# miha-stopar/Plonky3-mobile

Measured on AMD Instinct MI355X. Metric: fib_air proofs/sec, higher is better.
Workload: dtype u32 (BabyBear Montgomery, 31-bit modular)

## Files before the change

include/p3hip.h:

```cpp
#ifndef P3HIP_H
#define P3HIP_H
#include <stddef.h>
#include <stdint.h>

#ifdef __cplusplus
extern "C" {
#endif

#define P3HIP_OK 0
#define P3HIP_ERR_BAD_ARG (-1)
#define P3HIP_ERR_HIP (-2)
#define P3HIP_ERR_BACKEND (-3)
#define P3HIP_ERR_INTERNAL (-4)

#define P3HIP_BACKEND_CPU 0
#define P3HIP_BACKEND_VULKAN 1
#define P3HIP_BACKEND_METAL 2
#define P3HIP_BACKEND_WEBGPU 3
#define P3HIP_BACKEND_HIP 4

int p3hip_set_backend(const char *name);
int p3hip_get_backend(void);
int p3hip_is_available(char *msg, size_t cap);
const char *p3hip_take_last_error(void);

int p3hip_malloc(void **dev_ptr, size_t bytes);
int p3hip_free(void *dev_ptr);
int p3hip_upload(void *dev_dst, const void *host_src, size_t bytes);
int p3hip_download(void *host_dst, const void *dev_src, size_t bytes);
int p3hip_sync(void *stream);
void p3hip_release_thread_context(void);

int p3hip_dft_batch_bb31(const uint32_t *in, uint32_t *out, size_t height, size_t width);
int p3hip_idft_batch_bb31(const uint32_t *in, uint32_t *out, size_t height, size_t width);
int p3hip_coset_dft_batch_bb31(const uint32_t *in, uint32_t *out, size_t height, size_t width,
                               uint32_t shift_monty);
int p3hip_coset_lde_batch_bb31(const uint32_t *in, uint32_t *out, size_t height, size_t width,
                               unsigned added_bits, uint32_t shift_monty, int bit_reversed_out);
const char *p3hip_last_timing_line(void);
int p3hip_dft_batch_bb31_dev(const uint32_t *d_in, uint32_t *d_out, size_t height, size_t width, void *stream);
int p3hip_idft_batch_bb31_dev(const uint32_t *d_in, uint32_t *d_out, size_t height, size_t width, void *stream);
int p3hip_coset_dft_batch_bb31_dev(const uint32_t *d_in, uint32_t *d_out, size_t height, size_t width,
                                   uint32_t shift_monty, void *stream);
int p3hip_coset_lde_batch_bb31_dev(const uint32_t *d_in, uint32_t *d_out, size_t height, size_t width,
                                   unsigned added_bits, uint32_t shift_monty, int bit_reversed_out,
                                   void *stream);
int p3hip_coset_lde_from_coeffs_bb31_dev(const uint32_t *d_coeffs, uint32_t *d_out, size_t height, size_t width,
                                         unsigned added_bits, uint32_t shift_monty, void *stream);
int p3hip_dft_plan_bb31(size_t height, size_t width, uint32_t *stages_per_pass, size_t cap, size_t *n_passes);
int p3hip_bit_reverse_rows_dev(const uint32_t *d_in, uint32_t *d_out, size_t height, size_t width, void *stream);

int p3hip_fib_trace_dev(uint64_t a, uint64_t b, size_t n, uint32_t *d_out, void *stream);

int p3hip_poseidon2_permute_dev(uint32_t *d_states, size_t n, void *stream);
int p3hip_poseidon2_permute(uint32_t *states, size_t n);
int p3hip_poseidon2_permute_variant_dev(uint32_t *d_states, size_t n, int variant, void *stream);
int p3hip_poseidon2_f64_probe_dev(const double *d_in, uint32_t *d_out, size_t n, int mode, void *stream);

typedef struct p3hip_tree p3hip_tree_t;
int p3hip_mmcs_commit_dev(const uint32_t *const *d_mats, const size_t *heights, const size_t *widths,
                          size_t n_mats, uint32_t root_out[8], p3hip_tree_t **tree_out, void *stream);
int p3hip_mmcs_commit_async_dev(const uint32_t *const *d_mats, const size_t *heights, const size_t *widths,
                                size_t n_mats, p3hip_tree_t **tree_out, void *stream);
int p3hip_mmcs_root(const p3hip_tree_t *tree, uint32_t root_out[8], void *stream);
size_t p3hip_mmcs_log_max_height(const p3hip_tree_t *tree);
size_t p3hip_mmcs_num_layers(const p3hip_tree_t *tree);
const uint32_t *p3hip_mmcs_layer_dev(const p3hip_tree_t *tree, size_t layer, size_t *len_out);
int p3hip_mmcs_open_batch(const p3hip_tree_t *tree, size_t index, uint32_t *rows_out, uint32_t *path_out,
                          void *stream);
void p3hip_mmcs_free(p3hip_tree_t *tree);
#define P3HIP_MMCS_ROOT_MISMATCH 1
#define P3HIP_MMCS_WRONG_HEIGHT  2
#define P3HIP_MMCS_NOT_CANONICAL 3
#define P3HIP_MMCS_BAD_INDEX     4
int p3hip_mmcs_verify_batch(int hash, const uint32_t root[8], const size_t *heights, const size_t *widths, size_t n_mats,
                            size_t index, const uint32_t *rows, const uint32_t *path, size_t path_len);
size_t p3hip_mmcs_row_words(const p3hip_tree_t *tree);
int p3hip_mmcs_open_batch_many_dev(const p3hip_tree_t *tree, const uint32_t *d_indices, size_t n,
                                   uint32_t *d_rows , uint32_t *d_paths , void *stream);
int p3hip_mmcs_verify_batch_many_dev(int hash, const uint32_t root[8] ,
                                     const size_t *heights, const size_t *widths, size_t n_mats,
                                     const uint32_t *d_indices, size_t n, const uint32_t *d_rows, const uint32_t *d_paths,
                                     uint32_t *d_status , uint32_t *d_rejected ,
                                     void *stream);
int p3hip_mmcs_verify_batch_many_form_dev(int form, int hash, const uint32_t root[8], const size_t *heights, const size_t *widths,
                                          size_t n_mats, const uint32_t *d_indices, size_t n, const uint32_t *d_rows,
                                          const uint32_t *d_paths, uint32_t *d_status, uint32_t *d_rejected, void *stream);
size_t p3hip_mmcs_verify_coop_max(int hash, int profile);
int p3hip_mmcs_commit(const uint32_t *const *mats, const size_t *heights, const size_t *widths,
                      size_t n_mats, uint32_t root_out[8], p3hip_tree_t **tree_out);

#define P3HIP_HASH_POSEIDON2 0
#define P3HIP_HASH_KECCAK 1
int p3hip_mmcs_commit_hash_dev(int hash, const uint32_t *const *d_mats, const size_t *heights, const size_t *widths,
                               size_t n_mats, uint32_t root_out[8], p3hip_tree_t **tree_out, void *stream);
int p3hip_mmcs_commit_hash(int hash, const uint32_t *const *mats, const size_t *heights, const size_t *widths,
                           size_t n_mats, uint32_t root_out[8], p3hip_tree_t **tree_out);
size_t p3hip_mmcs_layer_words(size_t max_height);
int p3hip_mmcs_commit_into_dev(int hash, const uint32_t *const *d_mats, const size_t *heights, const size_t *widths,
                               size_t n_mats, uint32_t *d_layers, p3hip_tree_t **tree_out, void *stream);
int p3hip_keccak_f_dev(uint64_t *d_states, size_t n, void *stream);

typedef struct {
    uint32_t log_blowup;
    uint32_t log_final_poly_len;
    uint32_t num_queries;
    uint32_t proof_of_work_bits;
} p3hip_fri_params_t;
typedef struct p3hip_fib_prover p3hip_fib_prover_t;
#define P3HIP_PROFILE_THROUGHPUT 1
#define P3HIP_PROFILE_LATENCY 2
int p3hip_set_thread_profile(int profile);
int p3hip_get_thread_profile(void);
int p3hip_fib_prover_create_profile(int profile, int hash, int hiding, uint64_t seed, unsigned log_n, const p3hip_fri_params_t *params,
                                    void *stream, int own_stream, p3hip_fib_prover_t **out);
int p3hip_fib_prover_create(unsigned log_n, const p3hip_fri_params_t *params, void *stream, int own_stream,
                            p3hip_fib_prover_t **out);
int p3hip_fib_prover_prove(p3hip_fib_prover_t *prover, uint64_t a, uint64_t b, const uint8_t **proof_out,
                           size_t *proof_len);
int p3hip_fib_prover_prove_into(p3hip_fib_prover_t *prover, uint64_t a, uint64_t b, uint8_t *out, size_t cap, size_t *proof_len);
int p3hip_fib_prover_enqueue(p3hip_fib_prover_t *prover, uint64_t a, uint64_t b);
int p3hip_fib_prover_finish(p3hip_fib_prover_t *prover, const uint8_t **proof_out, size_t *proof_len);
int p3hip_fib_prover_stage_times(p3hip_fib_prover_t *prover, double out_ms[6], uint64_t *proofs, int reset);
int p3hip_fib_prover_grind_miss_probe(p3hip_fib_prover_t *prover, uint64_t *misses, uint32_t *indices_out, size_t cap,
                                      size_t *n_out);
void p3hip_fib_prover_destroy(p3hip_fib_prover_t *prover);
int p3hip_verify_fib_air(const uint8_t *proof, size_t len, uint64_t a, uint64_t b, uint64_t x, unsigned log_n,
                         const p3hip_fri_params_t *params);

int p3hip_fib_prover_create_hash(int hash, unsigned log_n, const p3hip_fri_params_t *params, void *stream, int own_stream,
                                 p3hip_fib_prover_t **out);
int p3hip_verify_fib_air_hash(int hash, const uint8_t *proof, size_t len, uint64_t a, uint64_t b, uint64_t x,
                              unsigned log_n, const p3hip_fri_params_t *params);

int p3hip_fib_prover_create_hiding(int hash, unsigned log_n, const p3hip_fri_params_t *params, uint64_t seed, void *stream,
                                   int own_stream, p3hip_fib_prover_t **out);
int p3hip_verify_fib_air_hiding(int hash, const uint8_t *proof, size_t len, uint64_t a, uint64_t b, uint64_t x,
                                unsigned log_n, const p3hip_fri_params_t *params);
typedef struct p3hip_rng p3hip_rng_t;
int p3hip_rng_create(uint64_t seed, p3hip_rng_t **out);
int p3hip_rng_fill_field_dev(p3hip_rng_t *rng, uint32_t *d_out, size_t n, void *stream);
int p3hip_rng_state(p3hip_rng_t *rng, uint64_t state_out[4], void *stream);
void p3hip_rng_destroy(p3hip_rng_t *rng);
int p3hip_mmcs_commit_hiding_dev(int hash, const uint32_t *const *d_mats, const size_t *heights, const size_t *widths,
                                 size_t n_mats, p3hip_rng_t *rng, uint32_t root_out[8], p3hip_tree_t **tree_out, void *stream);

typedef struct p3hip_fib_batch p3hip_fib_batch_t;
int p3hip_fib_batch_create(unsigned log_n, const p3hip_fri_params_t *params, unsigned n_provers,
                           p3hip_fib_batch_t **out);
int p3hip_fib_batch_create_hash(int hash, unsigned log_n, const p3hip_fri_params_t *params, unsigned n_provers,
                                p3hip_fib_batch_t **out);
int p3hip_fib_batch_create_hiding(int hash, unsigned log_n, const p3hip_fri_params_t *params, uint64_t seed, unsigned n_provers,
                                  p3hip_fib_batch_t **out);
int p3hip_fib_batch_prove(p3hip_fib_batch_t *batch, size_t n, const uint64_t *a, const uint64_t *b,
                          const uint8_t **proofs_out, size_t *lens_out);
int p3hip_fib_batch_submit(p3hip_fib_batch_t *batch, size_t n, const uint64_t *a, const uint64_t *b, uint64_t *ticket_out);
int p3hip_fib_batch_collect(p3hip_fib_batch_t *batch, uint64_t ticket, const uint8_t **proofs_out, size_t *lens_out);
void p3hip_fib_batch_destroy(p3hip_fib_batch_t *batch);

#define P3HIP_PROVE_CHECK_TRACE 1u
#define P3HIP_TRACE_BAD_FIRST_LEFT 1u
#define P3HIP_TRACE_BAD_FIRST_RIGHT 2u
#define P3HIP_TRACE_BAD_NEXT_LEFT 4u
#define P3HIP_TRACE_BAD_NEXT_RIGHT 8u
#define P3HIP_TRACE_BAD_LAST_RIGHT 16u
#define P3HIP_TRACE_BAD_RANGE 32u
typedef struct {
    int64_t first_bad_row;
    uint32_t mask;
    uint64_t bad_rows;
} p3hip_trace_check_t;
int p3hip_fib_check_trace_dev(const uint32_t *d_trace, size_t n, const uint32_t pis[3], p3hip_trace_check_t *out, void *stream);
int p3hip_fib_prover_prove_trace_dev(p3hip_fib_prover_t *prover, const uint32_t *d_trace, const uint32_t pis[3], unsigned flags,
                                     const uint8_t **proof_out, size_t *proof_len);
int p3hip_fib_prover_prove_trace(p3hip_fib_prover_t *prover, const uint32_t *host_trace, size_t n, const uint32_t pis[3], unsigned flags,
                                 const uint8_t **proof_out, size_t *proof_len);
int p3hip_fib_prover_enqueue_trace_dev(p3hip_fib_prover_t *prover, const uint32_t *d_trace, const uint32_t pis[3]);
int p3hip_fib_batch_prove_traces_dev(p3hip_fib_batch_t *batch, size_t n, const uint32_t *const *d_traces, const uint32_t *pis,
                                     unsigned flags, const uint8_t **proofs_out, size_t *lens_out);

typedef struct p3hip_fib_verifier p3hip_fib_verifier_t;
#define P3HIP_VERIFY_MALFORMED 16
int p3hip_fib_proof_len(int hash, int hiding, unsigned log_n, const p3hip_fri_params_t *params, size_t *len_out);
int p3hip_fib_verifier_create(int hash, int hiding, unsigned log_n, const p3hip_fri_params_t *params, size_t max_proofs,
                              p3hip_fib_verifier_t **out);
int p3hip_fib_verifier_verify_dev(p3hip_fib_verifier_t *v, const uint8_t *d_proofs, size_t stride_bytes, const uint32_t *d_lens,
                                  const uint32_t *d_pis, size_t n, uint32_t *d_status, uint32_t *d_rejected, void *stream);
int p3hip_fib_verifier_verify(p3hip_fib_verifier_t *v, size_t n, const uint8_t *const *proofs, const size_t *lens,
                              const uint64_t *a, const uint64_t *b, const uint64_t *x, uint32_t *status_out);
void p3hip_fib_verifier_destroy(p3hip_fib_verifier_t *v);

int p3hip_run_fib_air_zk(char *out, size_t cap);

typedef struct p3hip_challenger p3hip_challenger_t;
int p3hip_challenger_create(int hash, p3hip_challenger_t **out);
int p3hip_challenger_observe(p3hip_challenger_t *c, const uint32_t *monty_words, size_t n);
int p3hip_challenger_observe_digest(p3hip_challenger_t *c, const uint32_t digest[8]);
int p3hip_challenger_sample_ext(p3hip_challenger_t *c, uint32_t out[4]);
int p3hip_challenger_sample_bits(p3hip_challenger_t *c, unsigned bits, uint32_t *out);
int p3hip_challenger_clone(const p3hip_challenger_t *c, p3hip_challenger_t **out);
void p3hip_challenger_destroy(p3hip_challenger_t *c);
#define P3HIP_CHALLENGER_STATE_WORDS 128
int p3hip_challenger_export(const p3hip_challenger_t *c, uint32_t words[P3HIP_CHALLENGER_STATE_WORDS]);
int p3hip_challenger_import(p3hip_challenger_t *c, const uint32_t words[P3HIP_CHALLENGER_STATE_WORDS]);

typedef struct p3hip_pcs p3hip_pcs_t;
typedef struct p3hip_pcs_data p3hip_pcs_data_t;
int p3hip_pcs_create(int profile, int hash, const p3hip_fri_params_t *params, void *stream, int own_stream, p3hip_pcs_t **out);
int p3hip_pcs_commit_dev(p3hip_pcs_t *pcs, const uint32_t *const *d_evals, const size_t *heights, const size_t *widths,
                         const uint32_t *domain_shifts , size_t n_mats,
                         uint32_t root_out[8], p3hip_pcs_data_t **data_out);
int p3hip_pcs_lde_dev(const p3hip_pcs_data_t *data, size_t mat, const uint32_t **d_lde, size_t *height, size_t *width);
int p3hip_pcs_open(p3hip_pcs_t *pcs, const p3hip_pcs_data_t *const *rounds, size_t n_rounds,
                   const size_t *points_per_mat, const uint32_t *points ,
                   p3hip_challenger_t *challenger ,
                   uint32_t *opened_out, size_t opened_cap_words, const uint8_t **proof_out, size_t *proof_len);
int p3hip_pcs_verify(int hash, const p3hip_fri_params_t *params, unsigned log_h, const uint32_t *roots ,
                     const size_t *mats_per_round, const size_t *widths, size_t n_rounds, const size_t *points_per_mat,
                     const uint32_t *points, const uint32_t *opened, const uint8_t *proof, size_t len,
                     p3hip_challenger_t *challenger, int *reject_code);
void p3hip_pcs_data_free(p3hip_pcs_data_t *d);
void p3hip_pcs_destroy(p3hip_pcs_t *pcs);

int p3hip_pcs_create_hiding(int profile, int hash, const p3hip_fri_params_t *params, unsigned num_random_codewords, uint64_t mmcs_seed,
                            uint64_t pcs_seed, void *stream, int own_stream, p3hip_pcs_t **out);
int p3hip_pcs_commit_quotient_dev(p3hip_pcs_t *pcs, const uint32_t *const *d_chunks, size_t h, size_t width, size_t n_chunks,
                                  uint32_t root_out[8], p3hip_pcs_data_t **data_out);
int p3hip_pcs_commit_randomization(p3hip_pcs_t *pcs, unsigned log_h, uint32_t root_out[8], p3hip_pcs_data_t **data_out);
int p3hip_pcs_verify_hiding(int hash, const p3hip_fri_params_t *params, unsigned log_h, const uint32_t *roots ,
                            const size_t *mats_per_round, const size_t *widths, size_t n_rounds, const size_t *points_per_mat,
                            const uint32_t *points, const uint32_t *opened, const uint8_t *proof, size_t len,
                            p3hip_challenger_t *challenger, int *reject_code);

typedef struct p3hip_pcs_verifier p3hip_pcs_verifier_t;
typedef struct {
    unsigned log_h;
    size_t n_rounds;
    const size_t *mats_per_round;
    const size_t *widths;
    const size_t *points_per_mat;
    size_t n_slots;
    const uint32_t *slots;
} p3hip_pcs_shape_t;
int p3hip_pcs_proof_len(int hash, int hiding, const p3hip_fri_params_t *params, const p3hip_pcs_shape_t *shape, size_t *len_out);
int p3hip_pcs_verifier_create(int hash, int hiding, const p3hip_fri_params_t *params, const p3hip_pcs_shape_t *shape, size_t max_proofs,
                              p3hip_pcs_verifier_t **out);
int p3hip_pcs_verifier_verify_dev(p3hip_pcs_verifier_t *v, const uint8_t *d_proofs, size_t stride_bytes, const uint32_t *d_lens,
                                  const uint32_t *d_roots, const uint32_t *d_points, const uint32_t *d_opened, const uint32_t *d_chal_in,
                                  size_t n, uint32_t *d_status, uint32_t *d_rejected, uint32_t *d_chal_out, void *stream);
int p3hip_pcs_verifier_verify(p3hip_pcs_verifier_t *v, size_t n, const uint8_t *const *proofs, const size_t *lens, const uint32_t *roots,
                              const uint32_t *points, const uint32_t *opened, p3hip_challenger_t *const *challengers, uint32_t *status_out);
int p3hip_pcs_verifier_wave_form(const p3hip_pcs_verifier_t *v);
void p3hip_pcs_verifier_destroy(p3hip_pcs_verifier_t *v);

typedef int (*p3hip_cpu_dft_fn)(void *user, const uint32_t *in, uint32_t *out, size_t height, size_t width);
int p3hip_run_dft_benchmark(p3hip_cpu_dft_fn cpu_dft, void *user, char *out, size_t cap);

#ifdef __cplusplus
}
#endif
#endif
```

plonky3-mobile_amd/_lib.py:

```python
import ctypes as C
import os
import subprocess

_HERE = os.path.dirname(os.path.abspath(__file__))
LIB_PATH = os.environ.get("P3HIP_LIB") or os.path.join(_HERE, "libp3hip.so")
ROOT = os.path.dirname(_HERE)

u32p = C.POINTER(C.c_uint32)
_SIGS = {
    "p3hip_set_backend": (C.c_int, [C.c_char_p]),
    "p3hip_get_backend": (C.c_int, []),
    "p3hip_is_available": (C.c_int, [C.c_char_p, C.c_size_t]),
    "p3hip_take_last_error": (C.c_char_p, []),
    "p3hip_malloc": (C.c_int, [C.POINTER(C.c_void_p), C.c_size_t]),
    "p3hip_free": (C.c_int, [C.c_void_p]),
    "p3hip_upload": (C.c_int, [C.c_void_p, C.c_void_p, C.c_size_t]),
    "p3hip_download": (C.c_int, [C.c_void_p, C.c_void_p, C.c_size_t]),
    "p3hip_sync": (C.c_int, [C.c_void_p]),
    "p3hip_last_timing_line": (C.c_char_p, []),
    "p3hip_release_thread_context": (None, []),
    "p3hip_dft_batch_bb31": (C.c_int, [C.c_void_p, C.c_void_p, C.c_size_t, C.c_size_t]),
    "p3hip_idft_batch_bb31": (C.c_int, [C.c_void_p, C.c_void_p, C.c_size_t, C.c_size_t]),
    "p3hip_coset_dft_batch_bb31": (C.c_int, [C.c_void_p, C.c_void_p, C.c_size_t, C.c_size_t, C.c_uint32]),
    "p3hip_coset_lde_batch_bb31": (C.c_int, [C.c_void_p, C.c_void_p, C.c_size_t, C.c_size_t, C.c_uint,
                                             C.c_uint32, C.c_int]),
    "p3hip_dft_batch_bb31_dev": (C.c_int, [C.c_void_p, C.c_void_p, C.c_size_t, C.c_size_t, C.c_void_p]),
    "p3hip_idft_batch_bb31_dev": (C.c_int, [C.c_void_p, C.c_void_p, C.c_size_t, C.c_size_t, C.c_void_p]),
    "p3hip_coset_dft_batch_bb31_dev": (C.c_int, [C.c_void_p, C.c_void_p, C.c_size_t, C.c_size_t, C.c_uint32,
                                                 C.c_void_p]),
    "p3hip_coset_lde_batch_bb31_dev": (C.c_int, [C.c_void_p, C.c_void_p, C.c_size_t, C.c_size_t, C.c_uint,
                                                 C.c_uint32, C.c_int, C.c_void_p]),
    "p3hip_coset_lde_from_coeffs_bb31_dev": (C.c_int, [C.c_void_p, C.c_void_p, C.c_size_t, C.c_size_t, C.c_uint, C.c_uint32,
                                                       C.c_void_p]),
    "p3hip_bit_reverse_rows_dev": (C.c_int, [C.c_void_p, C.c_void_p, C.c_size_t, C.c_size_t, C.c_void_p]),
    "p3hip_dft_plan_bb31": (C.c_int, [C.c_size_t, C.c_size_t, C.POINTER(C.c_uint32), C.c_size_t, C.POINTER(C.c_size_t)]),
    "p3hip_fib_trace_dev": (C.c_int, [C.c_uint64, C.c_uint64, C.c_size_t, C.c_void_p, C.c_void_p]),
    "p3hip_poseidon2_permute_dev": (C.c_int, [C.c_void_p, C.c_size_t, C.c_void_p]),
    "p3hip_poseidon2_permute": (C.c_int, [C.c_void_p, C.c_size_t]),
    "p3hip_poseidon2_permute_variant_dev": (C.c_int, [C.c_void_p, C.c_size_t, C.c_int, C.c_void_p]),
    "p3hip_poseidon2_f64_probe_dev": (C.c_int, [C.c_void_p, C.c_void_p, C.c_size_t, C.c_int, C.c_void_p]),
    "p3hip_mmcs_commit_dev": (C.c_int, [C.POINTER(C.c_void_p), C.POINTER(C.c_size_t), C.POINTER(C.c_size_t),
                                        C.c_size_t, C.c_void_p, C.POINTER(C.c_void_p), C.c_void_p]),
    "p3hip_mmcs_commit_async_dev": (C.c_int, [C.POINTER(C.c_void_p), C.POINTER(C.c_size_t),
                                              C.POINTER(C.c_size_t), C.c_size_t, C.POINTER(C.c_void_p),
                                              C.c_void_p]),
    "p3hip_mmcs_commit_hash_dev": (C.c_int, [C.c_int, C.POINTER(C.c_void_p), C.POINTER(C.c_size_t), C.POINTER(C.c_size_t),
                                             C.c_size_t, C.c_void_p, C.POINTER(C.c_void_p), C.c_void_p]),
    "p3hip_mmcs_commit_hash": (C.c_int, [C.c_int, C.POINTER(C.c_void_p), C.POINTER(C.c_size_t), C.POINTER(C.c_size_t),
                                         C.c_size_t, C.c_void_p, C.POINTER(C.c_void_p)]),
    "p3hip_mmcs_layer_words": (C.c_size_t, [C.c_size_t]),
    "p3hip_mmcs_commit_into_dev": (C.c_int, [C.c_int, C.POINTER(C.c_void_p), C.POINTER(C.c_size_t), C.POINTER(C.c_size_t),
                                             C.c_size_t, C.c_void_p, C.POINTER(C.c_void_p), C.c_void_p]),
    "p3hip_keccak_f_dev": (C.c_int, [C.c_void_p, C.c_size_t, C.c_void_p]),
    "p3hip_mmcs_root": (C.c_int, [C.c_void_p, C.c_void_p, C.c_void_p]),
    "p3hip_mmcs_log_max_height": (C.c_size_t, [C.c_void_p]),
    "p3hip_mmcs_num_layers": (C.c_size_t, [C.c_void_p]),
    "p3hip_mmcs_layer_dev": (C.c_void_p, [C.c_void_p, C.c_size_t, C.POINTER(C.c_size_t)]),
    "p3hip_mmcs_open_batch": (C.c_int, [C.c_void_p, C.c_size_t, C.c_void_p, C.c_void_p, C.c_void_p]),
    "p3hip_mmcs_free": (None, [C.c_void_p]),
    "p3hip_mmcs_verify_batch": (C.c_int, [C.c_int, C.c_void_p, C.POINTER(C.c_size_t), C.POINTER(C.c_size_t), C.c_size_t, C.c_size_t,
                                          C.c_void_p, C.c_void_p, C.c_size_t]),
    "p3hip_mmcs_row_words": (C.c_size_t, [C.c_void_p]),
    "p3hip_mmcs_verify_coop_max": (C.c_size_t, [C.c_int, C.c_int]),
    "p3hip_mmcs_open_batch_many_dev": (C.c_int, [C.c_void_p, C.c_void_p, C.c_size_t, C.c_void_p, C.c_void_p, C.c_void_p]),
    "p3hip_mmcs_verify_batch_many_dev": (C.c_int, [C.c_int, C.c_void_p, C.POINTER(C.c_size_t), C.POINTER(C.c_size_t), C.c_size_t, C.c_void_p,
                                                   C.c_size_t, C.c_void_p, C.c_void_p, C.c_void_p, C.c_void_p, C.c_void_p]),
    "p3hip_mmcs_verify_batch_many_form_dev": (C.c_int, [C.c_int, C.c_int, C.c_void_p, C.POINTER(C.c_size_t), C.POINTER(C.c_size_t), C.c_size_t,
                                                        C.c_void_p, C.c_size_t, C.c_void_p, C.c_void_p, C.c_void_p, C.c_void_p, C.c_void_p]),
    "p3hip_set_thread_profile": (C.c_int, [C.c_int]),
    "p3hip_get_thread_profile": (C.c_int, []),
    "p3hip_fib_prover_create_profile": (C.c_int, [C.c_int, C.c_int, C.c_int, C.c_uint64, C.c_uint, C.c_void_p, C.c_void_p, C.c_int,
                                                  C.POINTER(C.c_void_p)]),
    "p3hip_fib_prover_create": (C.c_int, [C.c_uint, C.c_void_p, C.c_void_p, C.c_int, C.POINTER(C.c_void_p)]),
    "p3hip_fib_prover_create_hash": (C.c_int, [C.c_int, C.c_uint, C.c_void_p, C.c_void_p, C.c_int, C.POINTER(C.c_void_p)]),
    "p3hip_verify_fib_air_hash": (C.c_int, [C.c_int, C.c_void_p, C.c_size_t, C.c_uint64, C.c_uint64, C.c_uint64, C.c_uint,
                                            C.c_void_p]),
    "p3hip_fib_prover_prove": (C.c_int, [C.c_void_p, C.c_uint64, C.c_uint64, C.POINTER(C.POINTER(C.c_uint8)),
                                         C.POINTER(C.c_size_t)]),
    "p3hip_fib_prover_prove_into": (C.c_int, [C.c_void_p, C.c_uint64, C.c_uint64, C.c_void_p, C.c_size_t, C.POINTER(C.c_size_t)]),
    "p3hip_fib_prover_stage_times": (C.c_int, [C.c_void_p, C.POINTER(C.c_double), C.POINTER(C.c_uint64), C.c_int]),
    "p3hip_fib_prover_enqueue": (C.c_int, [C.c_void_p, C.c_uint64, C.c_uint64]),
    "p3hip_fib_prover_finish": (C.c_int, [C.c_void_p, C.POINTER(C.POINTER(C.c_uint8)), C.POINTER(C.c_size_t)]),
    "p3hip_fib_prover_destroy": (None, [C.c_void_p]),
    "p3hip_run_fib_air_zk": (C.c_int, [C.c_char_p, C.c_size_t]),
    "p3hip_run_dft_benchmark": (C.c_int, [C.c_void_p, C.c_void_p, C.c_char_p, C.c_size_t]),
    "p3hip_fib_prover_grind_miss_probe": (C.c_int, [C.c_void_p, C.POINTER(C.c_uint64), C.POINTER(C.c_uint32), C.c_size_t,
                                                    C.POINTER(C.c_size_t)]),
    "p3hip_fib_prover_create_hiding": (C.c_int, [C.c_int, C.c_uint, C.c_void_p, C.c_uint64, C.c_void_p, C.c_int, C.POINTER(C.c_void_p)]),
    "p3hip_verify_fib_air_hiding": (C.c_int, [C.c_int, C.c_void_p, C.c_size_t, C.c_uint64, C.c_uint64, C.c_uint64, C.c_uint,
                                              C.c_void_p]),
    "p3hip_rng_create": (C.c_int, [C.c_uint64, C.POINTER(C.c_void_p)]),
    "p3hip_rng_fill_field_dev": (C.c_int, [C.c_void_p, C.c_void_p, C.c_size_t, C.c_void_p]),
    "p3hip_rng_state": (C.c_int, [C.c_void_p, C.POINTER(C.c_uint64), C.c_void_p]),
    "p3hip_rng_destroy": (None, [C.c_void_p]),
    "p3hip_mmcs_commit_hiding_dev": (C.c_int, [C.c_int, C.POINTER(C.c_void_p), C.POINTER(C.c_size_t), C.POINTER(C.c_size_t),
                                               C.c_size_t, C.c_void_p, C.c_void_p, C.POINTER(C.c_void_p), C.c_void_p]),
    "p3hip_fib_batch_create": (C.c_int, [C.c_uint, C.c_void_p, C.c_uint, C.POINTER(C.c_void_p)]),
    "p3hip_fib_batch_create_hash": (C.c_int, [C.c_int, C.c_uint, C.c_void_p, C.c_uint, C.POINTER(C.c_void_p)]),
    "p3hip_fib_batch_create_hiding": (C.c_int, [C.c_int, C.c_uint, C.c_void_p, C.c_uint64, C.c_uint, C.POINTER(C.c_void_p)]),
    "p3hip_fib_batch_prove": (C.c_int, [C.c_void_p, C.c_size_t, C.POINTER(C.c_uint64), C.POINTER(C.c_uint64),
                                        C.POINTER(C.POINTER(C.c_uint8)), C.POINTER(C.c_size_t)]),
    "p3hip_fib_batch_submit": (C.c_int, [C.c_void_p, C.c_size_t, C.POINTER(C.c_uint64), C.POINTER(C.c_uint64), C.POINTER(C.c_uint64)]),
    "p3hip_fib_batch_collect": (C.c_int, [C.c_void_p, C.c_uint64, C.POINTER(C.POINTER(C.c_uint8)), C.POINTER(C.c_size_t)]),
    "p3hip_fib_batch_destroy": (None, [C.c_void_p]),
    "p3hip_verify_fib_air": (C.c_int, [C.c_void_p, C.c_size_t, C.c_uint64, C.c_uint64, C.c_uint64, C.c_uint, C.c_void_p]),
    "p3hip_fib_check_trace_dev": (C.c_int, [C.c_void_p, C.c_size_t, u32p, C.c_void_p, C.c_void_p]),
    "p3hip_fib_prover_prove_trace_dev": (C.c_int, [C.c_void_p, C.c_void_p, u32p, C.c_uint, C.POINTER(C.POINTER(C.c_uint8)),
                                                   C.POINTER(C.c_size_t)]),
    "p3hip_fib_prover_prove_trace": (C.c_int, [C.c_void_p, C.c_void_p, C.c_size_t, u32p, C.c_uint, C.POINTER(C.POINTER(C.c_uint8)),
                                               C.POINTER(C.c_size_t)]),
    "p3hip_fib_prover_enqueue_trace_dev": (C.c_int, [C.c_void_p, C.c_void_p, u32p]),
    "p3hip_fib_batch_prove_traces_dev": (C.c_int, [C.c_void_p, C.c_size_t, C.POINTER(C.c_void_p), u32p, C.c_uint,
                                                   C.POINTER(C.POINTER(C.c_uint8)), C.POINTER(C.c_size_t)]),
    "p3hip_fib_proof_len": (C.c_int, [C.c_int, C.c_int, C.c_uint, C.c_void_p, C.POINTER(C.c_size_t)]),
    "p3hip_fib_verifier_create": (C.c_int, [C.c_int, C.c_int, C.c_uint, C.c_void_p, C.c_size_t, C.POINTER(C.c_void_p)]),
    "p3hip_fib_verifier_verify_dev": (C.c_int, [C.c_void_p, C.c_void_p, C.c_size_t, C.c_void_p, C.c_void_p, C.c_size_t, C.c_void_p, C.c_void_p,
                                                C.c_void_p]),
    "p3hip_fib_verifier_verify": (C.c_int, [C.c_void_p, C.c_size_t, C.POINTER(C.c_char_p), C.POINTER(C.c_size_t), C.POINTER(C.c_uint64),
                                            C.POINTER(C.c_uint64), C.POINTER(C.c_uint64), u32p]),
    "p3hip_fib_verifier_destroy": (None, [C.c_void_p]),
    "p3hip_mmcs_commit": (C.c_int, [C.POINTER(C.c_void_p), C.POINTER(C.c_size_t), C.POINTER(C.c_size_t),
                                    C.c_size_t, C.c_void_p, C.POINTER(C.c_void_p)]),
    "p3hip_challenger_create": (C.c_int, [C.c_int, C.POINTER(C.c_void_p)]),
    "p3hip_challenger_observe": (C.c_int, [C.c_void_p, C.c_void_p, C.c_size_t]),
    "p3hip_challenger_observe_digest": (C.c_int, [C.c_void_p, C.c_void_p]),
    "p3hip_challenger_sample_ext": (C.c_int, [C.c_void_p, C.c_void_p]),
    "p3hip_challenger_sample_bits": (C.c_int, [C.c_void_p, C.c_uint, u32p]),
    "p3hip_challenger_clone": (C.c_int, [C.c_void_p, C.POINTER(C.c_void_p)]),
    "p3hip_challenger_destroy": (None, [C.c_void_p]),
    "p3hip_pcs_create": (C.c_int, [C.c_int, C.c_int, C.c_void_p, C.c_void_p, C.c_int, C.POINTER(C.c_void_p)]),
    "p3hip_pcs_commit_dev": (C.c_int, [C.c_void_p, C.POINTER(C.c_void_p), C.POINTER(C.c_size_t), C.POINTER(C.c_size_t), C.c_void_p, C.c_size_t,
                                       C.c_void_p, C.POINTER(C.c_void_p)]),
    "p3hip_pcs_lde_dev": (C.c_int, [C.c_void_p, C.c_size_t, C.POINTER(C.c_void_p), C.POINTER(C.c_size_t), C.POINTER(C.c_size_t)]),
    "p3hip_pcs_open": (C.c_int, [C.c_void_p, C.POINTER(C.c_void_p), C.c_size_t, C.POINTER(C.c_size_t), C.c_void_p, C.c_void_p, C.c_void_p,
                                 C.c_size_t, C.POINTER(C.POINTER(C.c_uint8)), C.POINTER(C.c_size_t)]),
    "p3hip_pcs_verify": (C.c_int, [C.c_int, C.c_void_p, C.c_uint, C.c_void_p, C.POINTER(C.c_size_t), C.POINTER(C.c_size_t), C.c_size_t,
                                   C.POINTER(C.c_size_t), C.c_void_p, C.c_void_p, C.c_void_p, C.c_size_t, C.c_void_p, C.POINTER(C.c_int)]),
    "p3hip_pcs_create_hiding": (C.c_int, [C.c_int, C.c_int, C.c_void_p, C.c_uint, C.c_uint64, C.c_uint64, C.c_void_p, C.c_int,
                                          C.POINTER(C.c_void_p)]),
    "p3hip_pcs_commit_quotient_dev": (C.c_int, [C.c_void_p, C.POINTER(C.c_void_p), C.c_size_t, C.c_size_t, C.c_size_t, C.c_void_p,
                                                C.POINTER(C.c_void_p)]),
    "p3hip_pcs_commit_randomization": (C.c_int, [C.c_void_p, C.c_uint, C.c_void_p, C.POINTER(C.c_void_p)]),
    "p3hip_pcs_verify_hiding": (C.c_int, [C.c_int, C.c_void_p, C.c_uint, C.c_void_p, C.POINTER(C.c_size_t), C.POINTER(C.c_size_t), C.c_size_t,
                                          C.POINTER(C.c_size_t), C.c_void_p, C.c_void_p, C.c_void_p, C.c_size_t, C.c_void_p,
                                          C.POINTER(C.c_int)]),
    "p3hip_challenger_export": (C.c_int, [C.c_void_p, C.c_void_p]),
    "p3hip_challenger_import": (C.c_int, [C.c_void_p, C.c_void_p]),
    "p3hip_pcs_proof_len": (C.c_int, [C.c_int, C.c_int, C.c_void_p, C.c_void_p, C.POINTER(C.c_size_t)]),
    "p3hip_pcs_verifier_create": (C.c_int, [C.c_int, C.c_int, C.c_void_p, C.c_void_p, C.c_size_t, C.POINTER(C.c_void_p)]),
    "p3hip_pcs_verifier_verify_dev": (C.c_int, [C.c_void_p, C.c_void_p, C.c_size_t, C.c_void_p, C.c_void_p, C.c_void_p, C.c_void_p, C.c_void_p,
                                                C.c_size_t, C.c_void_p, C.c_void_p, C.c_void_p, C.c_void_p]),
    "p3hip_pcs_verifier_verify": (C.c_int, [C.c_void_p, C.c_size_t, C.POINTER(C.c_char_p), C.POINTER(C.c_size_t), C.c_void_p, C.c_void_p,
                                            C.c_void_p, C.POINTER(C.c_void_p), u32p]),
    "p3hip_pcs_verifier_wave_form": (C.c_int, [C.c_void_p]),
    "p3hip_pcs_verifier_destroy": (None, [C.c_void_p]),
    "p3hip_pcs_data_free": (None, [C.c_void_p]),
    "p3hip_pcs_destroy": (None, [C.c_void_p]),
}


class P3HipError(RuntimeError):
    def __init__(self, code, msg):
        super().__init__("libp3hip error %d: %s" % (code, msg))
        self.code = code
        self.message = msg


def build(force=False):
    csrc = os.path.join(_HERE, "csrc")
    if force:
        subprocess.check_call(["make", "-s", "-C", csrc, "clean"])
    subprocess.check_call(["make", "-s", "-j4", "-C", csrc])
    return LIB_PATH


_lib = None


def lib():
    global _lib
    if _lib is None:
        if not os.path.exists(LIB_PATH):
            raise ImportError("libp3hip.so is not built (run __graft_entry__.build()); "
                              "there is no CPU fallback in this package")
        import torch
        L = C.CDLL(LIB_PATH)
        for name, (res, args) in _SIGS.items():
            fn = getattr(L, name)
            fn.restype = res
            fn.argtypes = args
        _lib = L
    return _lib


_sha = None


def lib_sha256():
    global _sha
    if _sha is None:
        import hashlib
        with open(LIB_PATH, "rb") as f:
            _sha = hashlib.sha256(f.read()).hexdigest()
    return _sha


_src_sha = None


def src_sha256():
    global _src_sha
    if _src_sha is None:
        import glob
        import hashlib
        csrc = os.path.join(_HERE, "csrc")
        files = sorted(glob.glob(os.path.join(csrc, "*.hip")) + glob.glob(os.path.join(csrc, "*.h")) + glob.glob(os.path.join(csrc, "*.inc")) +
                       [os.path.join(csrc, "Makefile"), os.path.join(ROOT, "include", "p3hip.h")])
        h = hashlib.sha256()
        for f in files:
            h.update(os.path.relpath(f, ROOT).encode() + b"\0")
            with open(f, "rb") as fh:
                h.update(fh.read())
            h.update(b"\0")
        _src_sha = h.hexdigest()
    return _src_sha


def declared_symbols():
    return sorted(_SIGS)


def take_last_error():
    m = lib().p3hip_take_last_error()
    return m.decode() if m else None


def check(rc):
    if rc != 0:
        raise P3HipError(rc, take_last_error() or "")
```

plonky3-mobile_amd/csrc/c_api.hip:

```cpp
#include "../../include/p3hip.h"

#include <atomic>
#include <chrono>
#include <condition_variable>
#include <mutex>
#include <deque>
#include <thread>
#include <cctype>
#include <cstdio>
#include <cstring>

#include "bb31.hip.h"
#include "challenger.h"
#include "common.h"
#include "mmcs.h"
#include "prover.h"
#include "pcs_verifier_dev.h"
#include "verifier_dev.h"
#include "rng.h"

namespace p3 {
bool take_error(std::string* out);
}
using namespace p3;
// ... 563 lines not shown
            P3_HIP(hipStreamCreateWithFlags(&st, hipStreamNonBlocking));
            own = true;
        }
        std::unique_ptr<p3hip_fib_prover> p(new p3hip_fib_prover());
        FriParams fp{params->log_blowup, params->log_final_poly_len, params->num_queries, params->proof_of_work_bits};
        if (hiding) {
            p->hiding.reset(new FibHidingProver());
            rc = p->hiding->init(log_n, fp, st, own, hash, seed, prof);
        } else {
            p->plain.reset(new FibProver());
            rc = p->plain->init(log_n, fp, st, own, hash, prof);
        }
        if (rc) return rc;
        *out = p.release();
        return OK;
    });
}
int p3hip_fib_prover_create(unsigned log_n, const p3hip_fri_params_t* params, void* stream, int own_stream,
                            p3hip_fib_prover_t** out) {
    return p3hip_fib_prover_create_profile(P3HIP_PROFILE_LATENCY, HASH_POSEIDON2, 0, 0, log_n, params, stream, own_stream, out);
}
int p3hip_fib_prover_create_hash(int hash, unsigned log_n, const p3hip_fri_params_t* params, void* stream, int own_stream,
                                 p3hip_fib_prover_t** out) {
    return p3hip_fib_prover_create_profile(P3HIP_PROFILE_LATENCY, hash, 0, 0, log_n, params, stream, own_stream, out);
}

int p3hip_fib_prover_prove(p3hip_fib_prover_t* prover, uint64_t a, uint64_t b, const uint8_t** proof_out,
                           size_t* proof_len) {
    return guarded([&]() -> int {
        if (!prover || !proof_out || !proof_len) return fail(ERR_BAD_ARG, "fib_prover_prove: null argument");
        int rc = prover->prove(a, b);
        if (rc) return rc;
        *proof_out = prover->last.data();
        *proof_len = prover->last.size();
        return OK;
    });
}

int p3hip_fib_prover_prove_into(p3hip_fib_prover_t* prover, uint64_t a, uint64_t b, uint8_t* out, size_t cap, size_t* proof_len) {
    return guarded([&]() -> int {
        if (!prover || !out || !proof_len) return fail(ERR_BAD_ARG, "fib_prover_prove_into: null argument");
        if (prover->proof_len && prover->proof_len > cap) {
            *proof_len = prover->proof_len;
            return fail(ERR_BAD_ARG, "fib_prover_prove_into: the proof needs " + std::to_string(prover->proof_len) + " bytes");
        }
        int rc = prover->prove(a, b);
        if (rc) return rc;
        *proof_len = prover->last.size();
        if (prover->last.size() > cap) return fail(ERR_BAD_ARG, "fib_prover_prove_into: the proof needs " + std::to_string(prover->last.size()) + " bytes");
        memcpy(out, prover->last.data(), prover->last.size());
        return OK;
    });
}

int p3hip_fib_prover_enqueue(p3hip_fib_prover_t* prover, uint64_t a, uint64_t b) {
    return guarded([&]() -> int {
        if (!prover) return fail(ERR_BAD_ARG, "fib_prover_enqueue: null argument");
        if (!prover->plain) return fail(ERR_BAD_ARG, "fib_prover_enqueue: the hiding prover proves one proof at a time");
        return prover->plain->enqueue(a, b);
    });
}
int p3hip_fib_prover_finish(p3hip_fib_prover_t* prover, const uint8_t** proof_out, size_t* proof_len) {
    return guarded([&]() -> int {
        if (!prover || !proof_out || !proof_len) return fail(ERR_BAD_ARG, "fib_prover_finish: null argument");
        if (!prover->plain) return fail(ERR_BAD_ARG, "fib_prover_finish: the hiding prover proves one proof at a time");
        int rc = prover->plain->finish(&prover->last);
        if (rc) { prover->last.clear(); return rc; }
        prover->proof_len = prover->last.size();
        *proof_out = prover->last.data();
        *proof_len = prover->last.size();
        return OK;
    });
}

int p3hip_fib_check_trace_dev(const uint32_t* d_trace, size_t n, const uint32_t pis[3], p3hip_trace_check_t* out, void* stream) {
    return guarded([&]() -> int {
        if (!out || !pis) return fail(ERR_BAD_ARG, "fib_check_trace: null argument");
        Context* cx;
        int rc = get_context(&cx);
        if (rc) return rc;
        if (!n) { *out = p3hip_trace_check_t{-1, 0, 0}; return OK; }
        if ((rc = check_device_trace(d_trace, n, cx->device, "fib_check_trace"))) return rc;
        if ((rc = check_pis_flags(pis, 0, "fib_check_trace"))) return rc;
        TraceCheck c;
        if ((rc = fib_check_trace(*cx, (hipStream_t)stream, d_trace, n, pis, &c))) return rc;
        *out = p3hip_trace_check_t{c.first_bad_row, c.mask, c.bad_rows};
        return OK;
    });
}

int p3hip_fib_prover_prove_trace_dev(p3hip_fib_prover_t* prover, const uint32_t* d_trace, const uint32_t pis[3], unsigned flags,
                                     const uint8_t** proof_out, size_t* proof_len) {
    return guarded([&]() -> int {
        if (!prover || !proof_out || !proof_len) return fail(ERR_BAD_ARG, "fib_prover_prove_trace_dev: null argument");
        int rc = check_pis_flags(pis, flags, "fib_prover_prove_trace_dev");
        if (rc) return rc;
        if ((rc = check_device_trace(d_trace, 1ull << prover->log_n(), prover->device(), "fib_prover_prove_trace_dev"))) return rc;
        if ((rc = prover->prove_trace(d_trace, pis, flags))) return rc;
        *proof_out = prover->last.data();
        *proof_len = prover->last.size();
        return OK;
    });
}
int p3hip_fib_prover_prove_trace(p3hip_fib_prover_t* prover, const uint32_t* host_trace, size_t n, const uint32_t pis[3], unsigned flags,
                                 const uint8_t** proof_out, size_t* proof_len) {
    return guarded([&]() -> int {
        if (!prover || !host_trace || !proof_out || !proof_len) return fail(ERR_BAD_ARG, "fib_prover_prove_trace: null argument");
        int rc = check_pis_flags(pis, flags, "fib_prover_prove_trace");
        if (rc) return rc;
        if (n != (1ull << prover->log_n()))
            return fail(ERR_BAD_ARG, "fib_prover_prove_trace: n = " + std::to_string(n) + " rows, the prover proves 2^" + std::to_string(prover->log_n()));
        if (prover->plain && prover->plain->has_pending())
            return fail(ERR_BAD_ARG, "fib prover: finish the enqueued proofs before a synchronous prove");
        Context* cx;
        if ((rc = get_context(&cx))) return rc;
        if (cx->device != prover->device())
            return fail(ERR_BAD_ARG, "fib prover: created on device " + std::to_string(prover->device()) + ", current device is " + std::to_string(cx->device));
        P3_HIP(hipMemcpyAsync(prover->arena_trace(), host_trace, (size_t)n * 8, hipMemcpyHostToDevice, prover->stream()));
        if ((rc = prover->prove_trace(prover->arena_trace(), pis, flags))) return rc;
        *proof_out = prover->last.data();
        *proof_len = prover->last.size();
        return OK;
    });
}
int p3hip_fib_prover_enqueue_trace_dev(p3hip_fib_prover_t* prover, const uint32_t* d_trace, const uint32_t pis[3]) {
    return guarded([&]() -> int {
        if (!prover) return fail(ERR_BAD_ARG, "fib_prover_enqueue_trace_dev: null argument");
        if (!prover->plain) return fail(ERR_BAD_ARG, "fib_prover_enqueue_trace_dev: the hiding prover proves one proof at a time");
        int rc = check_pis_flags(pis, 0, "fib_prover_enqueue_trace_dev");
        if (rc) return rc;
        if ((rc = check_device_trace(d_trace, 1ull << prover->log_n(), prover->device(), "fib_prover_enqueue_trace_dev"))) return rc;
        return prover->plain->enqueue_trace(d_trace, pis);
    });
}

int p3hip_fib_prover_stage_times(p3hip_fib_prover_t* prover, double out_ms[6], uint64_t* proofs, int reset) {
    if (!prover || !out_ms) return fail(ERR_BAD_ARG, "fib_prover_stage_times: null argument");
    if (!prover->plain) return fail(ERR_BAD_ARG, "fib_prover_stage_times: not kept by the hiding prover");
    const StageTimes& t = prover->plain->times();
    out_ms[0] = t.trace_commit_ms; out_ms[1] = t.quotient_commit_ms; out_ms[2] = t.open_ms;
    out_ms[3] = t.fri_commit_ms; out_ms[4] = t.grind_ms; out_ms[5] = t.query_ms;
    if (proofs) *proofs = t.proofs;
    if (reset) prover->plain->reset_times();
    return OK;
}

int p3hip_fib_prover_grind_miss_probe(p3hip_fib_prover_t* prover, uint64_t* misses, uint32_t* indices_out, size_t cap, size_t* n_out) {
    if (!prover || !misses) return fail(ERR_BAD_ARG, "fib_prover_grind_miss_probe: null argument");
    if (!prover->plain) return fail(ERR_BAD_ARG, "fib_prover_grind_miss_probe: not kept by the hiding prover");
    std::vector<uint32_t> idx;
    *misses = prover->plain->grind_misses(&idx);
    if (n_out) *n_out = idx.size();
    if (indices_out) for (size_t i = 0; i < idx.size() && i < cap; i++) indices_out[i] = idx[i];
    return OK;
}

void p3hip_fib_prover_destroy(p3hip_fib_prover_t* prover) { delete prover; }

int p3hip_fib_prover_create_hiding(int hash, unsigned log_n, const p3hip_fri_params_t* params, uint64_t seed, void* stream,
                                   int own_stream, p3hip_fib_prover_t** out) {
    return p3hip_fib_prover_create_profile(P3HIP_PROFILE_LATENCY, hash, 1, seed, log_n, params, stream, own_stream, out);
}
int p3hip_verify_fib_air_hiding(int hash, const uint8_t* proof, size_t len, uint64_t a, uint64_t b, uint64_t x, unsigned log_n,
                                const p3hip_fri_params_t* params) {
    return guarded([&]() -> int {
        if (!proof || !params) return fail(ERR_BAD_ARG, "verify_fib_air_hiding: null argument");
        FriParams fp{params->log_blowup, params->log_final_poly_len, params->num_queries, params->proof_of_work_bits};
        std::string why;
        int rc = verify_fib_air_hiding(proof, len, a, b, x, log_n, fp, &why, hash);
        if (rc != 0) set_error("fib_air verification failed: " + why);
        return rc;
    });
}

}
struct p3hip_rng {
    DevRng* d = nullptr;
    uint32_t* err = nullptr;
    DevBuf ws;
    ~p3hip_rng() { if (d) (void)hipFree(d); }
};
extern "C" {
int p3hip_rng_create(uint64_t seed, p3hip_rng_t** out) {
    return guarded([&]() -> int {
        if (!out) return fail(ERR_BAD_ARG, "rng_create: null argument");
        Context* cx;
        int rc = get_context(&cx);
        if (rc) return rc;
        std::unique_ptr<p3hip_rng> r(new p3hip_rng());
        P3_HIP(hipMalloc(reinterpret_cast<void**>(&r->d), sizeof(DevRng) + 16));
        r->err = reinterpret_cast<uint32_t*>(r->d + 1);
        uint64_t s[6] = {0, 0, 0, 0, 0, 0};
        rng_seed_from_u64(s, seed);
        P3_HIP(hipMemcpy(r->d, s, sizeof(DevRng) + 16, hipMemcpyHostToDevice));
        *out = r.release();
        return OK;
    });
}
int p3hip_rng_fill_field_dev(p3hip_rng_t* rng, uint32_t* d_out, size_t n, void* stream) {
    return guarded([&]() -> int {
        if (!rng || (n && !d_out)) return fail(ERR_BAD_ARG, "rng_fill_field: null argument");
        Context* cx;
        int rc = get_context(&cx);
        if (rc) return rc;
        size_t words = 0;
        if ((rc = rng_workspace_words(n, &words))) return rc;
        if ((rc = rng->ws.reserve(words * 4))) return rc;
        return rng_fill_field(*cx, (hipStream_t)stream, rng->d, d_out, n, rng->ws.as<uint32_t>(), rng->err);
    });
}
int p3hip_rng_state(p3hip_rng_t* rng, uint64_t state_out[4], void* stream) {
    return guarded([&]() -> int {
        if (!rng || !state_out) return fail(ERR_BAD_ARG, "rng_state: null argument");
        uint64_t s[6];
        P3_HIP(hipMemcpyAsync(s, rng->d, sizeof(DevRng) + 16, hipMemcpyDeviceToHost, (hipStream_t)stream));
        P3_HIP(hipStreamSynchronize((hipStream_t)stream));
        memcpy(state_out, s, 32);
        if ((uint32_t)s[4] != 0) return fail(ERR_INTERNAL, "rng: a fill ran out of raw draws");
        return OK;
    });
}
void p3hip_rng_destroy(p3hip_rng_t* rng) { delete rng; }

int p3hip_mmcs_commit_hiding_dev(int hash, const uint32_t* const* d_mats, const size_t* heights, const size_t* widths, size_t n_mats,
                                 p3hip_rng_t* rng, uint32_t root_out[8], p3hip_tree_t** tree_out, void* stream) {
    return guarded([&]() -> int {
        if (!d_mats || !heights || !widths || !n_mats || !rng || !root_out || !tree_out) return fail(ERR_BAD_ARG, "mmcs_commit_hiding: null/empty argument");
        if (n_mats > 32) return fail(ERR_BAD_ARG, "mmcs_commit_hiding: at most 32 matrices per commitment");
        constexpr size_t SALT = 4;
        std::vector<void*> owned;
        auto cleanup = [&]() { for (void* p : owned) (void)hipFree(p); };
        std::vector<const uint32_t*> mp;
        std::vector<size_t> hh, ww;
        for (size_t i = 0; i < n_mats; i++) {
            void* salt = nullptr;
            if (hipMalloc(&salt, heights[i] * SALT * 4 + 16) != hipSuccess) { cleanup(); return fail(ERR_HIP, "hipMalloc failed"); }
            owned.push_back(salt);
            int rc = p3hip_rng_fill_field_dev(rng, (uint32_t*)salt, heights[i] * SALT, stream);
            if (rc) { cleanup(); return rc; }
            mp.push_back(d_mats[i]); hh.push_back(heights[i]); ww.push_back(widths[i]);
            mp.push_back((const uint32_t*)salt); hh.push_back(heights[i]); ww.push_back(SALT);
        }
        int rc = p3hip_mmcs_commit_hash_dev(hash, mp.data(), hh.data(), ww.data(), mp.size(), root_out, tree_out, stream);
        if (rc) { cleanup(); return rc; }
        (*tree_out)->t->owned = owned;
        return OK;
    });
}

int p3hip_verify_fib_air(const uint8_t* proof, size_t len, uint64_t a, uint64_t b, uint64_t x, unsigned log_n,
                         const p3hip_fri_params_t* params) {
    return p3hip_verify_fib_air_hash(HASH_POSEIDON2, proof, len, a, b, x, log_n, params);
}
int p3hip_verify_fib_air_hash(int hash, const uint8_t* proof, size_t len, uint64_t a, uint64_t b, uint64_t x, unsigned log_n,
                              const p3hip_fri_params_t* params) {
    return guarded([&]() -> int {
        if (!proof || !params) return fail(ERR_BAD_ARG, "verify_fib_air: null argument");
        FriParams fp{params->log_blowup, params->log_final_poly_len, params->num_queries, params->proof_of_work_bits};
        std::string why;
        int rc = verify_fib_air(proof, len, a, b, x, log_n, fp, &why, hash);
        if (rc != 0) set_error("fib_air verification failed: " + why);
        return rc;
    });
}

}

struct p3hip_fib_batch {
    unsigned log_n = 0;
    int hash = HASH_POSEIDON2;
    int device = 0;
    FriParams fp{};
    std::vector<std::thread> workers;
    std::mutex mu;
    std::condition_variable cv_work, cv_done;
    struct Job {
        uint64_t ticket = 0;
        std::vector<uint64_t> a, b;
        std::vector<const uint32_t*> traces;
        std::vector<uint32_t> pis;
        unsigned flags = 0;
        size_t next = 0, done = 0;
        std::vector<std::vector<uint8_t>> proofs;
        int first_error = 0;
        std::string error_text;
    };
    std::deque<std::shared_ptr<Job>> jobs;
    std::shared_ptr<Job> collected;
    uint64_t next_ticket = 1;
    bool stop = false;
    size_t ready = 0;
    int first_error = 0;
    std::string error_text;
    static constexpr size_t MAX_INFLIGHT = 8;

    bool hiding = false;
    uint64_t seed = 1;
    int profile = PROFILE_THROUGHPUT;
    void worker_main() {
        if (hiding) {
            FibHidingProver prover;
            worker_loop(prover, [&](hipStream_t st) { return prover.init(log_n, fp, st, true, hash, seed, profile); });
        } else {
            FibProver prover;
            worker_loop(prover, [&](hipStream_t st) { return prover.init(log_n, fp, st, true, hash, profile); });
        }
// ... 507 lines not shown
```

plonky3-mobile_amd/csrc/common.h:

```cpp
#pragma once
#include <hip/hip_runtime.h>
#include <stdint.h>

#include <map>
#include <set>
#include <string>
#include <tuple>
#include <vector>

namespace p3 {

#ifndef P3_NO_SETPRIO
#define P3_LATENCY_BOUND_KERNEL() __builtin_amdgcn_s_setprio(3)
#else
#define P3_LATENCY_BOUND_KERNEL() ((void)0)
#endif

enum Profile : int { PROFILE_THROUGHPUT = 0, PROFILE_LATENCY = 1 };

enum Status : int {
    OK = 0,
    ERR_BAD_ARG = -1,
    ERR_HIP = -2,
    ERR_BACKEND = -3,
    ERR_INTERNAL = -4,
};

void set_error(const std::string& msg);
int fail(int code, const std::string& msg);

#define P3_HIP(call)                                                                       \
    do {                                                                                   \
        hipError_t e__ = (call);                                                           \
        if (e__ != hipSuccess)                                                             \
            return p3::fail(p3::ERR_HIP, std::string(#call) + ": " + hipGetErrorString(e__)); \
    } while (0)

struct DevBuf {
    void* ptr = nullptr;
    size_t cap = 0;
    int reserve(size_t bytes);
    template <class T>
    T* as() const { return reinterpret_cast<T*>(ptr); }
    ~DevBuf();
};

struct TwoLevelTable {
    uint32_t* lo = nullptr;
    uint32_t* hi = nullptr;
    uint32_t T = 0;
};

struct CachedTable {
    TwoLevelTable t;
    hipEvent_t ready = nullptr;
    hipStream_t built_on = nullptr;
    bool complete = false;
};

struct Context {
    int device = -1;
    int profile = PROFILE_LATENCY;
    uint32_t* tile_tw[2] = {nullptr, nullptr};
    double2* tile_twd[2] = {nullptr, nullptr};
    std::map<std::pair<uint32_t, int>, CachedTable> root_tables;
    std::map<std::tuple<uint32_t, uint32_t, uint32_t>, CachedTable> scale_tables;
    std::map<std::pair<hipStream_t, int>, DevBuf> scratch;
    std::set<const void*> attr_done;
    uint64_t* rng_jump = nullptr;
    std::map<uint32_t, CachedTable> selector_tables;
    int init(int dev);
    DevBuf& ws(hipStream_t stream, int slot);
    int get_root_table(hipStream_t stream, uint32_t q, bool inverse, TwoLevelTable* out);
    int get_scale_table(hipStream_t stream, uint32_t base, uint32_t log_n, uint32_t mult, TwoLevelTable* out);
    int reserve_scale_slots(size_t k);
    int mark_built(hipStream_t stream, CachedTable& e);
    int wait_ready(hipStream_t stream, CachedTable& e);
    int ensure_dynamic_lds(const void* kernel, int bytes);
    ~Context();
};

int get_context(Context** out);
void release_thread_contexts();

int ntt_dft(Context& cx, hipStream_t stream, const uint32_t* src, uint32_t* dst, uint64_t height,
            uint32_t width, bool inverse);
std::vector<uint32_t> ntt_dft_plan(uint32_t n);
int ntt_coset_lde(Context& cx, hipStream_t stream, const uint32_t* src, uint32_t* dst, uint64_t height,
                  uint32_t width, uint32_t added_bits, uint32_t shift_monty, bool bit_reversed_out);
int ntt_coset_lde_from_coeffs(Context& cx, hipStream_t stream, const uint32_t* coeffs, uint32_t* dst, uint32_t* scratch,
                              uint64_t height, uint32_t width, uint32_t added_bits, uint32_t shift_monty);
int ntt_coset_dft(Context& cx, hipStream_t stream, const uint32_t* src, uint32_t* dst, uint64_t height,
                  uint32_t width, uint32_t shift_monty);
int bit_reverse_rows(hipStream_t stream, const uint32_t* src, uint32_t* dst, uint64_t height, uint32_t width);

int fib_trace(hipStream_t stream, uint64_t a, uint64_t b, uint64_t n, uint32_t* d_out);
enum : uint32_t {
    TRACE_BAD_FIRST_LEFT = 1, TRACE_BAD_FIRST_RIGHT = 2, TRACE_BAD_NEXT_LEFT = 4, TRACE_BAD_NEXT_RIGHT = 8, TRACE_BAD_LAST_RIGHT = 16,
    TRACE_BAD_RANGE = 32,
};
struct TraceCheck {
    int64_t first_bad_row;
    uint32_t mask;
    uint64_t bad_rows;
};
int fib_check_trace(Context& cx, hipStream_t stream, const uint32_t* d_trace, uint64_t n, const uint32_t pis[3], TraceCheck* out);

inline bool is_pow2(uint64_t v) { return v && !(v & (v - 1)); }
inline uint32_t log2u(uint64_t v) {
    uint32_t l = 0;
    while ((1ull << l) < v) l++;
    return l;
}

}
```

plonky3-mobile_amd/csrc/fib_air.hip:

```cpp
#include "bb31.hip.h"
#include "common.h"

#include <algorithm>

namespace p3 {

constexpr uint32_t FIB_CHUNK = 16;

struct M2 { uint32_t a, b, c, d; };
__device__ __forceinline__ M2 m2mul(const M2& x, const M2& y) {
    return M2{bb::add(bb::mul(x.a, y.a), bb::mul(x.b, y.c)), bb::add(bb::mul(x.a, y.b), bb::mul(x.b, y.d)),
              bb::add(bb::mul(x.c, y.a), bb::mul(x.d, y.c)), bb::add(bb::mul(x.c, y.b), bb::mul(x.d, y.d))};
}

__global__ void fib_trace_kernel(uint32_t a0, uint32_t b0, uint64_t n, uint32_t* out) {
    uint64_t t = (uint64_t)blockIdx.x * blockDim.x + threadIdx.x;
    uint64_t start = t * FIB_CHUNK;
    if (start >= n) return;
    M2 acc{bb::ONE, 0, 0, bb::ONE}, base{0, bb::ONE, bb::ONE, bb::ONE};
    for (uint64_t e = start; e; e >>= 1) {
        if (e & 1) acc = m2mul(acc, base);
        base = m2mul(base, base);
    }
    uint32_t l = bb::add(bb::mul(acc.a, a0), bb::mul(acc.b, b0));
    uint32_t r = bb::add(bb::mul(acc.c, a0), bb::mul(acc.d, b0));
    uint2* rows = reinterpret_cast<uint2*>(out);
    for (uint32_t i = 0; i < FIB_CHUNK && start + i < n; i++) {
        rows[start + i] = make_uint2(l, r);
        uint32_t nr = bb::add(l, r);
        l = r;
        r = nr;
    }
}

int fib_trace(hipStream_t stream, uint64_t a, uint64_t b, uint64_t n, uint32_t* d_out) {
    if (!n) return OK;
    if (!is_pow2(n)) return fail(ERR_BAD_ARG, "generate_trace_rows: n must be a power of two");
    uint64_t threads = (n + FIB_CHUNK - 1) / FIB_CHUNK;
    uint32_t a0 = bb::to_monty((uint32_t)(a % bb::P)), b0 = bb::to_monty((uint32_t)(b % bb::P));
    hipLaunchKernelGGL(fib_trace_kernel, dim3((uint32_t)((threads + 255) / 256)), dim3(256), 0, stream, a0, b0, n, d_out);
    P3_HIP(hipGetLastError());
    return OK;
}

constexpr uint32_t CHECK_BLOCK = 256, CHECK_UNROLL = 4, CHECK_MAX_BLOCKS = 256 * 8;

struct CheckPis { uint32_t p0, p1, p2; };

__device__ __forceinline__ uint32_t check_row(uint64_t i, uint64_t n, uint32_t l, uint32_t r, uint32_t nl, uint32_t nr, const CheckPis& p) {
    uint32_t m = (l >= bb::P || r >= bb::P) ? TRACE_BAD_RANGE : 0u;
    if (i == 0) m |= (l != p.p0 ? TRACE_BAD_FIRST_LEFT : 0u) | (r != p.p1 ? TRACE_BAD_FIRST_RIGHT : 0u);
    if (i + 1 < n) {
        m |= nl != r ? TRACE_BAD_NEXT_LEFT : 0u;
        m |= nr != (uint32_t)(((uint64_t)l + r) % bb::P) ? TRACE_BAD_NEXT_RIGHT : 0u;
    } else {
        m |= r != p.p2 ? TRACE_BAD_LAST_RIGHT : 0u;
    }
    return m;
}

template <bool WIDE>
__global__ void __launch_bounds__(CHECK_BLOCK) fib_check_trace_kernel(const uint32_t* trace, uint64_t n, CheckPis pis,
                                                                     unsigned long long* res ) {
    const uint32_t lane = threadIdx.x & 63;
    const uint64_t pairs = (n + 1) / 2;
    const uint64_t wave = ((uint64_t)blockIdx.x * CHECK_BLOCK + threadIdx.x) >> 6, n_waves = ((uint64_t)gridDim.x * CHECK_BLOCK) >> 6;
    const uint2* rows = reinterpret_cast<const uint2*>(trace);
    unsigned long long best = ~0ull;
    uint32_t bad = 0;
    for (uint64_t base = wave * 64 * CHECK_UNROLL; base < pairs; base += n_waves * 64 * CHECK_UNROLL) {
        uint4 v[CHECK_UNROLL];
#pragma unroll
        for (uint32_t k = 0; k < CHECK_UNROLL; k++) {
            const uint64_t q = base + k * 64 + lane;
            v[k] = make_uint4(0, 0, 0, 0);
            if (2 * q + 2 <= n) {
                if (WIDE) {
                    v[k] = reinterpret_cast<const uint4*>(trace)[q];
                } else {
                    const uint2 x = rows[2 * q], y = rows[2 * q + 1];
                    v[k] = make_uint4(x.x, x.y, y.x, y.y);
                }
            } else if (2 * q < n) {
                const uint2 x = rows[2 * q];
                v[k].x = x.x; v[k].y = x.y;
            }
        }
        uint2 tail = make_uint2(0, 0);
        const uint64_t tail_row = 2 * (base + CHECK_UNROLL * 64);
        if (lane == 63 && tail_row < n) tail = rows[tail_row];
#pragma unroll
        for (uint32_t k = 0; k < CHECK_UNROLL; k++) {
            const uint64_t q = base + k * 64 + lane;
            uint32_t nl = __shfl_down(v[k].x, 1), nr = __shfl_down(v[k].y, 1);
            if (k + 1 < CHECK_UNROLL) {
                const uint32_t fl = __shfl(v[k + 1].x, 0), fr = __shfl(v[k + 1].y, 0);
                if (lane == 63) { nl = fl; nr = fr; }
            } else if (lane == 63) {
                nl = tail.x; nr = tail.y;
            }
            if (2 * q < n) {
                const uint32_t m0 = check_row(2 * q, n, v[k].x, v[k].y, v[k].z, v[k].w, pis);
                if (m0) { best = min(best, ((unsigned long long)(2 * q) << 6) | m0); bad++; }
                if (2 * q + 1 < n) {
                    const uint32_t m1 = check_row(2 * q + 1, n, v[k].z, v[k].w, nl, nr, pis);
                    if (m1) { best = min(best, ((unsigned long long)(2 * q + 1) << 6) | m1); bad++; }
                }
            }
        }
    }
    if (__ballot(bad != 0) == 0) return;
    unsigned long long total = bad;
#pragma unroll
    for (int off = 32; off > 0; off >>= 1) {
        best = min(best, __shfl_xor(best, off));
        total += __shfl_xor(total, off);
    }
    if (lane == 0) {
        atomicMax(&res[0], ~best);
        atomicAdd(&res[1], total);
    }
}

int fib_check_trace(Context& cx, hipStream_t stream, const uint32_t* d_trace, uint64_t n, const uint32_t pis[3], TraceCheck* out) {
    *out = TraceCheck{-1, 0, 0};
    if (!n) return OK;
    if (reinterpret_cast<uintptr_t>(d_trace) % 8) return fail(ERR_BAD_ARG, "check_trace: the trace must be 8-byte aligned (rows of two words)");
    if (n > (1ull << 57)) return fail(ERR_BAD_ARG, "check_trace: too many rows");
    DevBuf& buf = cx.ws(stream, 4);
    int rc = buf.reserve(16);
    if (rc) return rc;
    unsigned long long* res = buf.as<unsigned long long>();
    P3_HIP(hipMemsetAsync(res, 0, 16, stream));
    const uint64_t pairs = (n + 1) / 2, per_block = (uint64_t)CHECK_BLOCK * CHECK_UNROLL;
    const uint32_t blocks = (uint32_t)std::min<uint64_t>((pairs + per_block - 1) / per_block, CHECK_MAX_BLOCKS);
    const CheckPis p{pis[0], pis[1], pis[2]};
    if (reinterpret_cast<uintptr_t>(d_trace) % 16 == 0)
        hipLaunchKernelGGL(fib_check_trace_kernel<true>, dim3(blocks), dim3(CHECK_BLOCK), 0, stream, d_trace, n, p, res);
    else
        hipLaunchKernelGGL(fib_check_trace_kernel<false>, dim3(blocks), dim3(CHECK_BLOCK), 0, stream, d_trace, n, p, res);
    P3_HIP(hipGetLastError());
    unsigned long long h[2] = {0, 0};
    P3_HIP(hipMemcpyAsync(h, res, 16, hipMemcpyDeviceToHost, stream));
    P3_HIP(hipStreamSynchronize(stream));
    if (h[1]) {
        const unsigned long long key = ~h[0];
        out->first_bad_row = (int64_t)(key >> 6);
        out->mask = (uint32_t)(key & 63);
        out->bad_rows = h[1];
    }
    return OK;
}

}
```

plonky3-mobile_amd/csrc/poseidon2_f64.hip.h:

```cpp
#pragma once
#include "poseidon2.hip.h"

namespace p2f {

constexpr double PD = 2013265921.0;
constexpr double PINV = 1.0 / 2013265921.0;

__device__ __forceinline__ double mulmod(double a, double b) {
    double h = a * b;
    double l = __fma_rn(a, b, -h);
    double q = __builtin_rint(h * PINV);
    double r = __fma_rn(-q, PD, h);
    return r + l;
}
constexpr double PM1 = 2013265920.0;
__device__ __forceinline__ double mulmod_p(double a, double b, double aP) {
    double q = __builtin_rint(b * aP);
    double t = __fma_rn(a, b, -(q * PM1));
    return t - q;
}
__device__ __forceinline__ double reduce(double x) {
    return __fma_rn(-__builtin_rint(x * PINV), PD, x);
}
__device__ __forceinline__ double add_scaled_pow2(double tot, double x, double inv) {
    double xt = __fma_rn(x, inv, tot);
    double fr = __builtin_amdgcn_fract(xt);
    return __fma_rn(fr, -PD, xt);
}
constexpr double MAGIC = 6755399441055744.0;
constexpr double MAGIC_P = 6755399441055744.0 * 2013265921.0;
struct MagicRegs { double m, mp; };
__device__ __forceinline__ MagicRegs magic_regs() {
    MagicRegs r{MAGIC, MAGIC_P};
    asm volatile("" : "+v"(r.m), "+v"(r.mp));
    return r;
}
__device__ __forceinline__ double mulmod_m(double a, double b, double aP, const MagicRegs& k, double neg_pm1) {
    const double qb = __fma_rn(b, aP, k.m);
    const double c = __fma_rn(qb, neg_pm1, k.mp);
    const double t = __fma_rn(a, b, c);
    return t - qb;
}
__device__ __forceinline__ double sbox7(double x, const MagicRegs& k, double neg_pm1, double pinv) {
    const double xP = x * pinv;
    const double x2 = mulmod_m(x, x, xP, k, neg_pm1), x3 = mulmod_m(x, x2, xP, k, neg_pm1), x4 = mulmod_m(x, x3, xP, k, neg_pm1);
    return mulmod_m(x3, x4, x3 * pinv, k, neg_pm1);
}

struct ConstsF64 {
    double ext[8][16];
    double in[13];
    double k3, k15, i4, i8, i16, i256;
    double neg_pm1, pinv;
};
constexpr uint32_t c_from_monty(uint32_t m) {
    uint32_t t = m * bb::MU;
    uint64_t u = (uint64_t)t * bb::P;
    uint32_t uh = (uint32_t)(u >> 32);
    return uh ? bb::P - uh : 0;
}
constexpr uint64_t c_powmod(uint64_t b, uint64_t e) { uint64_t r = 1; b %= bb::P; while (e) { if (e & 1) r = r * b % bb::P; b = b * b % bb::P; e >>= 1; } return r; }
constexpr ConstsF64 make_consts() {
    ConstsF64 c{};
    for (int r = 0; r < 4; r++)
        for (int i = 0; i < 16; i++) {
            c.ext[r][i] = (double)c_from_monty(P3_RC16_EXT_INIT_MONTY[r][i]);
            c.ext[4 + r][i] = (double)c_from_monty(P3_RC16_EXT_FINAL_MONTY[r][i]);
        }
    for (int r = 0; r < 13; r++) c.in[r] = (double)c_from_monty(P3_RC16_INTERNAL_MONTY[r]);
    c.k3 = 3.0; c.k15 = 15.0; c.i4 = 0.25; c.i8 = 0.125; c.i16 = 0.0625; c.i256 = 0.00390625;
    c.neg_pm1 = -2013265920.0; c.pinv = 1.0 / 2013265921.0;
    return c;
}
static __device__ __constant__ ConstsF64 d_c = make_consts();

__device__ __forceinline__ void mat4(double& a, double& b, double& c, double& d) {
    double t01 = a + b, t23 = c + d, t0123 = t01 + t23;
    double t01123 = t0123 + b, t01233 = t0123 + d;
    double nd = __fma_rn(a, 2.0, t01233), nb = __fma_rn(c, 2.0, t01123);
    double na = t01123 + t01, nc = t01233 + t23;
    a = na; b = nb; c = nc; d = nd;
}
__device__ __forceinline__ void external_linear(double (&s)[16]) {
#pragma unroll
    for (int i = 0; i < 16; i += 4) mat4(s[i], s[i + 1], s[i + 2], s[i + 3]);
    double t[4];
#pragma unroll
    for (int k = 0; k < 4; k++) t[k] = (s[k] + s[k + 4]) + (s[k + 8] + s[k + 12]);
#pragma unroll
    for (int i = 0; i < 16; i++) s[i] += t[i & 3];
}

__device__ __forceinline__ void internal_rounds(double (&s)[16], const MagicRegs& mk) {
    const double npm1 = d_c.neg_pm1, pinv = d_c.pinv;
    const double k3 = d_c.k3, k15 = d_c.k15, i4 = d_c.i4, i8 = d_c.i8, i16 = d_c.i16, i256 = d_c.i256;
    auto internal_round = [&](int r) {
        s[0] = sbox7(s[0] + d_c.in[r], mk, npm1, pinv);
        double tot = ((s[0] + s[1]) + (s[2] + s[3])) + ((s[4] + s[5]) + (s[6] + s[7])) +
                     (((s[8] + s[9]) + (s[10] + s[11])) + ((s[12] + s[13]) + (s[14] + s[15])));
        tot = reduce(tot);
        s[0] = __fma_rn(s[0], -2.0, tot);
        s[1] = tot + s[1];
        s[2] = __fma_rn(s[2], 2.0, tot);
        s[3] = add_scaled_pow2(tot, s[3], 0.5);
        s[4] = __fma_rn(s[4], k3, tot);
        s[5] = __fma_rn(s[5], 4.0, tot);
        s[6] = add_scaled_pow2(tot, s[6], -0.5);
        s[7] = __fma_rn(s[7], -k3, tot);
        s[8] = __fma_rn(s[8], -4.0, tot);
        s[9] = add_scaled_pow2(tot, s[9], i256);
        s[10] = add_scaled_pow2(tot, s[10], i4);
        s[11] = add_scaled_pow2(tot, s[11], i8);
        s[12] = __fma_rn(s[12], -k15, tot);
        s[13] = add_scaled_pow2(tot, s[13], -i256);
        s[14] = add_scaled_pow2(tot, s[14], -i16);
        s[15] = __fma_rn(s[15], k15, tot);
    };
    auto fold_integer_lanes = [&]() {
        s[1] = reduce(s[1]); s[2] = reduce(s[2]); s[4] = reduce(s[4]); s[5] = reduce(s[5]);
        s[7] = reduce(s[7]); s[8] = reduce(s[8]); s[12] = reduce(s[12]); s[15] = reduce(s[15]);
    };
    _Pragma("clang loop unroll(disable)")
    for (int blk = 0; blk < 3; blk++) {
        _Pragma("clang loop unroll(disable)")
        for (int r = 0; r < 4; r++) internal_round(4 * blk + r);
        fold_integer_lanes();
    }
    internal_round(12);
    fold_integer_lanes();
}

__device__ __forceinline__ void permute(double (&s)[16]) {
    const MagicRegs mk = magic_regs();
    const double npm1 = d_c.neg_pm1, pinv = d_c.pinv;
    external_linear(s);
    _Pragma("clang loop unroll(disable)")
    for (int r = 0; r < 4; r++) {
#pragma unroll
        for (int i = 0; i < 16; i++) s[i] = sbox7(s[i] + d_c.ext[r][i], mk, npm1, pinv);
        external_linear(s);
    }
    internal_rounds(s, mk);
    _Pragma("clang loop unroll(disable)")
    for (int r = 4; r < 8; r++) {
#pragma unroll
        for (int i = 0; i < 16; i++) s[i] = sbox7(s[i] + d_c.ext[r][i], mk, npm1, pinv);
        external_linear(s);
    }
}

__device__ __forceinline__ double load_elem(uint32_t monty) { return (double)bb::from_monty(monty); }
constexpr double R_MOD_P = 268435454.0;
constexpr double R_MOD_P_OVER_P = 268435454.0 / 2013265921.0;
__device__ __forceinline__ uint32_t store_elem(double v, const MagicRegs& k) {
    const double r = mulmod_m(R_MOD_P, v, R_MOD_P_OVER_P, k, d_c.neg_pm1);
    const uint32_t w = (uint32_t)(int32_t)r;
    return min(w, w + bb::P);
}
__device__ __forceinline__ uint32_t store_elem(double v) { return store_elem(v, magic_regs()); }

}
```

plonky3-mobile_amd/csrc/prover.h:

```cpp
#pragma once
#include <chrono>
#include <string>
#include <vector>

#include "common.h"

namespace p3 {

struct Tree;
struct Challenger;

struct FriParams {
    uint32_t log_blowup, log_final_poly_len, num_queries, proof_of_work_bits;
};

constexpr uint32_t MAX_LOG_DOMAIN = 26;
constexpr uint32_t MAX_LOG_DOMAIN_HIDING = 24;

struct StageTimes {
    double trace_commit_ms = 0, quotient_commit_ms = 0, open_ms = 0, fri_commit_ms = 0, grind_ms = 0, query_ms = 0;
    uint64_t proofs = 0;
};

class FibProver {
  public:
    FibProver();
    ~FibProver();
    FibProver(const FibProver&) = delete;
    int init(uint32_t log_n, const FriParams& fp, hipStream_t stream, bool own_stream, int hash = 0, int profile = PROFILE_LATENCY);
    int prove(uint64_t a, uint64_t b, std::vector<uint8_t>* proof);
    int enqueue(uint64_t a, uint64_t b);
    int finish(std::vector<uint8_t>* proof);
    int prove_trace(const uint32_t* d_trace, const uint32_t pis[3], std::vector<uint8_t>* proof);
    int enqueue_trace(const uint32_t* d_trace, const uint32_t pis[3]);
    uint32_t* arena_trace() const;
    bool has_pending() const;
    hipStream_t stream() const;
    uint32_t log_n() const;
    int device() const;
    const StageTimes& times() const;
    void reset_times();
    uint64_t grind_misses(std::vector<uint32_t>* last_indices) const;

  private:
    struct Impl;
    Impl* im;
    int run(uint64_t a, uint64_t b, int slot, int phase, std::vector<uint8_t>* proof, void* pending_rec);
    int enqueue_any(uint64_t a, uint64_t b, const uint32_t* d_trace, const uint32_t* pis);
};

class FibHidingProver {
  public:
    FibHidingProver();
    ~FibHidingProver();
    FibHidingProver(const FibHidingProver&) = delete;
    int init(uint32_t log_n, const FriParams& fp, hipStream_t stream, bool own_stream, int hash, uint64_t seed, int profile = PROFILE_LATENCY);
    int prove(uint64_t a, uint64_t b, std::vector<uint8_t>* proof);
    int prove_trace(const uint32_t* d_trace, const uint32_t pis[3], std::vector<uint8_t>* proof);
    uint32_t* arena_trace() const;
    hipStream_t stream() const;
    uint32_t log_n() const;
    int device() const;

  private:
    struct Impl;
    Impl* im;
    int prove_any(uint64_t a, uint64_t b, const uint32_t* d_trace, const uint32_t* pis, std::vector<uint8_t>* proof);
};

int verify_fib_air(const uint8_t* proof, size_t len, uint64_t a_pub, uint64_t b_pub, uint64_t x_pub, uint32_t log_n,
                   const FriParams& fp, std::string* why, int hash = 0);
int verify_fib_air_hiding(const uint8_t* proof, size_t len, uint64_t a_pub, uint64_t b_pub, uint64_t x_pub, uint32_t log_n,
                          const FriParams& fp, std::string* why, int hash);
int verify_check_parameters(int hash, bool hiding, uint32_t log_n, const FriParams& fp, std::string* why);


constexpr size_t PCS_MAX_MATS = 8;
constexpr size_t PCS_MAX_ROUNDS = 4;
constexpr size_t PCS_MAX_POINTS = 4;
constexpr size_t PCS_MAX_COLS = 8192;

constexpr size_t PCS_HIDING_MAX_MATS = 4;
constexpr uint32_t PCS_SALT = 4;
constexpr uint32_t PCS_MAX_RANDOM_CODEWORDS = 8;
constexpr size_t PCS_MAX_QUOTIENT_WIDTH = 2048;

struct PcsData {
    std::vector<uint32_t*> lde;
    std::vector<size_t> widths;
    uint32_t log_h = 0, log_big = 0;
    int hash = 0, device = -1;
    Tree* tree = nullptr;
    bool hiding = false;
    uint32_t nrc = 0;
    uint32_t* salt_base = nullptr;
    std::vector<uint32_t*> salts;
    PcsData() = default;
    PcsData(const PcsData&) = delete;
    ~PcsData();
};

class Pcs {
  public:
    Pcs();
    ~Pcs();
    Pcs(const Pcs&) = delete;
    int init(const FriParams& fp, hipStream_t stream, bool own_stream, int hash, int profile);
    int init_hiding(const FriParams& fp, hipStream_t stream, bool own_stream, int hash, int profile, uint32_t num_random_codewords,
                    uint64_t mmcs_seed, uint64_t pcs_seed);
    bool hiding() const;
    int commit(const uint32_t* const* d_evals, const size_t* heights, const size_t* widths, const uint32_t* shifts, size_t n_mats,
               uint32_t root_out[8], PcsData** out);
    int commit_quotient(const uint32_t* const* d_chunks, size_t h, size_t width, size_t n_chunks, uint32_t root_out[8], PcsData** out);
    int commit_randomization(uint32_t log_h, uint32_t root_out[8], PcsData** out);
    int open(const PcsData* const* rounds, size_t n_rounds, const size_t* points_per_mat, const uint32_t* points, Challenger* chal,
             std::vector<uint32_t>* opened, std::vector<uint8_t>* proof);
    hipStream_t stream() const;

  private:
    struct Impl;
    Impl* im;
    int commit_hiding(const uint32_t* const* d_evals, const size_t* heights, const size_t* widths, const uint32_t* shifts, size_t n_mats,
                      uint32_t root_out[8], PcsData** out);
    int hiding_finish(PcsData* data, uint32_t root_out[8]);
};

bool pcs_point_on_lde_coset(const uint32_t z[4], uint32_t log_big);
constexpr uint32_t CHALLENGER_STATE_WORDS = 128;
void challenger_export(const Challenger& c, uint32_t* words);
int challenger_import(const uint32_t* words, Challenger* c);
int pcs_verify(int hash, const FriParams& fp, uint32_t log_h, const uint32_t* roots, const size_t* mats_per_round, const size_t* widths,
               size_t n_rounds, const size_t* points_per_mat, const uint32_t* points, const uint32_t* opened, const uint8_t* proof,
               size_t len, Challenger* chal, std::string* why);
int pcs_verify_hiding(int hash, const FriParams& fp, uint32_t log_h, const uint32_t* roots, const size_t* mats_per_round,
                      const size_t* widths, size_t n_rounds, const size_t* points_per_mat, const uint32_t* points, const uint32_t* opened,
                      const uint8_t* proof, size_t len, Challenger* chal, std::string* why);

}
```

plonky3-mobile_amd/csrc/prover.hip:

```cpp
#include <chrono>
#include <cstddef>
#include <deque>
#include <memory>
#include <cstring>

#include "bb31.hip.h"
#include "challenger.h"
#include "common.h"
#include "keccak.hip.h"
#include "mmcs.h"
#include "poseidon2.hip.h"
#include "poseidon2_f64.hip.h"
#include "prover.h"
#include "rng.h"
#include "rng_dev.hip.h"
#include "transcript.hip.h"

namespace p3 {

using bb::Ext;

__device__ __forceinline__ uint32_t tl(const TwoLevelTable& t, uint32_t e) {
    return bb::mul(t.lo[e & ((1u << t.T) - 1u)], t.hi[e >> t.T]);
}
__device__ __forceinline__ uint32_t brev(uint32_t v, uint32_t bits) { return bits ? (__brev(v) >> (32 - bits)) : 0u; }

__device__ __forceinline__ Ext ld_ext(const uint32_t* p) {
    uint4 v = *reinterpret_cast<const uint4*>(p);
    return Ext{{v.x, v.y, v.z, v.w}};
}
__device__ __forceinline__ void st_ext(uint32_t* p, const Ext& e) {
    *reinterpret_cast<uint4*>(p) = make_uint4(e.c[0], e.c[1], e.c[2], e.c[3]);
}

constexpr int SEL_CHUNK = 8;
__global__ void selectors_kernel(TwoLevelTable roots, uint32_t n, uint32_t gen, uint32_t ginv, uint32_t zh, uint2* sel) {
    uint32_t t = blockIdx.x * blockDim.x + threadIdx.x;
    uint32_t i0 = t * SEL_CHUNK;
    if (i0 >= n) return;
    uint32_t v[2 * SEL_CHUNK], pre[2 * SEL_CHUNK];
    uint32_t acc = bb::ONE;
#pragma unroll
    for (int k = 0; k < SEL_CHUNK; k++) {
        uint32_t x = bb::mul(gen, tl(roots, (i0 + k) & (n - 1)));
        v[2 * k] = bb::sub(x, bb::ONE);
        v[2 * k + 1] = bb::sub(x, ginv);
    }
#pragma unroll
    for (int k = 0; k < 2 * SEL_CHUNK; k++) { pre[k] = acc; acc = bb::mul(acc, v[k]); }
    uint32_t inv = bb::mul(bb::inv(acc), zh);
#pragma unroll
    for (int k = 2 * SEL_CHUNK - 1; k >= 0; k--) {
        uint32_t r = bb::mul(inv, pre[k]);
        inv = bb::mul(inv, v[k]);
        v[k] = r;
    }
#pragma unroll
    for (int k = 0; k < SEL_CHUNK; k++)
        if (i0 + k < n) sel[i0 + k] = make_uint2(v[2 * k], v[2 * k + 1]);
}

struct QuotArgs {
    const uint2* lde;
    const uint2* sel;
    uint32_t* out;
    const DevState* ds;
    TwoLevelTable roots;
    uint32_t n, log_n, gen, ginv, zh_inv;
};
__global__ void __launch_bounds__(256) fib_quotient_kernel(QuotArgs a) {
    uint32_t i = blockIdx.x * blockDim.x + threadIdx.x;
    if (i >= a.n) return;
    const DevState* __restrict__ ds = a.ds;
    uint2 loc = a.lde[brev(i, a.log_n)];
    uint2 nxt = a.lde[brev((i + 1) & (a.n - 1), a.log_n)];
    uint2 s = a.sel[i];
    uint32_t x = bb::mul(a.gen, tl(a.roots, i));
    uint32_t trans = bb::sub(x, a.ginv);
    uint32_t c0 = bb::mul(s.x, bb::sub(loc.x, ds->pis[0]));
    uint32_t c1 = bb::mul(s.x, bb::sub(loc.y, ds->pis[1]));
    uint32_t c2 = bb::mul(trans, bb::sub(loc.y, nxt.x));
    uint32_t c3 = bb::mul(trans, bb::sub(bb::add(loc.x, loc.y), nxt.y));
    uint32_t c4 = bb::mul(s.y, bb::sub(loc.y, ds->pis[2]));
    Ext acc;
#pragma unroll
    for (int k = 0; k < 4; k++)
        acc.c[k] = bb::add(bb::add(bb::dot2(ds->apow[4].c[k], c0, ds->apow[3].c[k], c1), bb::dot2(ds->apow[2].c[k], c2, ds->apow[1].c[k], c3)),
                           bb::mul(ds->apow[0].c[k], c4));
    st_ext(a.out + 4 * (size_t)i, bb::scale(acc, a.zh_inv));
}

constexpr int DEN_CHUNK = 4;
__global__ void __launch_bounds__(256) inv_denoms_kernel(TwoLevelTable roots, uint32_t big, uint32_t log_big, uint32_t gen,
                                                         const DevState* __restrict__ ds, uint32_t* d0, uint32_t* d1) {
    const DenConsts k0 = ds->k0, k1 = ds->k1;
    uint32_t t = blockIdx.x * blockDim.x + threadIdx.x;
    uint32_t j0 = t * DEN_CHUNK;
    if (j0 >= big) return;
    uint32_t a0[2 * DEN_CHUNK], e0[2 * DEN_CHUNK], e1[2 * DEN_CHUNK], nrm[2 * DEN_CHUNK], pre[2 * DEN_CHUNK];
#pragma unroll
    for (int k = 0; k < DEN_CHUNK; k++) {
        uint32_t x = bb::mul(gen, tl(roots, brev((j0 + k) & (big - 1), log_big)));
#pragma unroll
        for (int z = 0; z < 2; z++) {
            const DenConsts& c = z ? k1 : k0;
            const uint32_t a = bb::sub(c.z0, x);
            const uint32_t dd0 = bb::add(bb::sqr(a), c.k0), dd1 = bb::sub(bb::mul(c.k1, a), c.c1);
            a0[2 * k + z] = a; e0[2 * k + z] = dd0; e1[2 * k + z] = dd1;
            nrm[2 * k + z] = bb::sub(bb::sqr(dd0), bb::mul(bb::W_MONTY, bb::sqr(dd1)));
        }
    }
    uint32_t acc = bb::ONE;
#pragma unroll
    for (int k = 0; k < 2 * DEN_CHUNK; k++) { pre[k] = acc; acc = bb::mul(acc, nrm[k]); }
    uint32_t inv = bb::inv(acc);
#pragma unroll
    for (int k = 2 * DEN_CHUNK - 1; k >= 0; k--) {
        const uint32_t r = bb::mul(inv, pre[k]);
        inv = bb::mul(inv, nrm[k]);
        nrm[k] = r;
    }
#pragma unroll
    for (int k = 0; k < DEN_CHUNK; k++) {
        if (j0 + k >= big) break;
#pragma unroll
        for (int z = 0; z < 2; z++) {
            const DenConsts& c = z ? k1 : k0;
            const uint32_t i = 2 * k + z;
            const uint32_t f0 = bb::mul(e0[i], nrm[i]), f1 = bb::neg(bb::mul(e1[i], nrm[i]));
            Ext r;
            r.c[0] = bb::add(bb::mul(a0[i], f0), bb::mul(c.z2w, f1));
            r.c[2] = bb::add(bb::mul(a0[i], f1), bb::mul(c.z2, f0));
            r.c[1] = bb::neg(bb::add(bb::mul(c.z1, f0), bb::mul(c.z3w, f1)));
            r.c[3] = bb::neg(bb::add(bb::mul(c.z1, f1), bb::mul(c.z3, f0)));
            st_ext((z ? d1 : d0) + 4 * (size_t)(j0 + k), r);
        }
    }
}

constexpr int BARY_BLOCK = 256;
__global__ void __launch_bounds__(BARY_BLOCK) barycentric_kernel(TwoLevelTable roots, uint32_t n, uint32_t log_big,
                                                                 uint32_t gen, const uint2* lde_t, const uint4* lde_q,
                                                                 const uint32_t* d0, const uint32_t* d1,
                                                                 uint32_t* partials) {
    Ext acc[8];
#pragma unroll
    for (int k = 0; k < 8; k++) acc[k] = bb::ext_zero();
    const uint32_t step = gridDim.x * blockDim.x;
    for (uint32_t j = blockIdx.x * blockDim.x + threadIdx.x; j < n; j += 2 * step) {
        const bool two = j + step < n;
        const uint32_t j2 = two ? j + step : j;
        const uint32_t xa = bb::mul(gen, tl(roots, brev(j, log_big))), xb = two ? bb::mul(gen, tl(roots, brev(j2, log_big))) : 0u;
        const Ext e0a = bb::scale(ld_ext(d0 + 4 * (size_t)j), xa), e1a = bb::scale(ld_ext(d1 + 4 * (size_t)j), xa);
        const Ext e0b = bb::scale(ld_ext(d0 + 4 * (size_t)j2), xb), e1b = bb::scale(ld_ext(d1 + 4 * (size_t)j2), xb);
        const uint2 ta = lde_t[j], tb = lde_t[j2];
        const uint4 qa = lde_q[j], qb = lde_q[j2];
        auto fma2 = [](Ext& s, const Ext& ea, uint32_t va, const Ext& eb, uint32_t vb) {
#pragma unroll
            for (int c = 0; c < 4; c++) s.c[c] = bb::add(s.c[c], bb::dot2(ea.c[c], va, eb.c[c], vb));
        };
        fma2(acc[0], e0a, ta.x, e0b, tb.x);
        fma2(acc[1], e0a, ta.y, e0b, tb.y);
        fma2(acc[2], e1a, ta.x, e1b, tb.x);
        fma2(acc[3], e1a, ta.y, e1b, tb.y);
        fma2(acc[4], e0a, qa.x, e0b, qb.x);
        fma2(acc[5], e0a, qa.y, e0b, qb.y);
        fma2(acc[6], e0a, qa.z, e0b, qb.z);
        fma2(acc[7], e0a, qa.w, e0b, qb.w);
    }
    __shared__ uint32_t red[BARY_BLOCK / 64][32];
    const uint32_t lane = threadIdx.x & 63, wave = threadIdx.x >> 6;
#pragma unroll
    for (int k = 0; k < 8; k++)
#pragma unroll
        for (int c = 0; c < 4; c++) {
            uint32_t v = acc[k].c[c];
#pragma unroll
            for (int off = 32; off > 0; off >>= 1) v = bb::add(v, (uint32_t)__shfl_down((int)v, off, 64));
            if (lane == 0) red[wave][4 * k + c] = v;
        }
    __syncthreads();
    if (threadIdx.x < 32) {
        uint32_t v = 0;
#pragma unroll
        for (int w = 0; w < BARY_BLOCK / 64; w++) v = bb::add(v, red[w][threadIdx.x]);
        partials[blockIdx.x * 32 + threadIdx.x] = v;
    }
}

struct ReducedArgs {
    const uint2* lde_t;
    const uint4* lde_q;
    const uint32_t* d0;
    const uint32_t* d1;
    uint32_t* ro;
    const DevState* ds;
    uint32_t big;
};
__global__ void __launch_bounds__(256) reduced_openings_kernel(ReducedArgs a) {
    uint32_t j = blockIdx.x * blockDim.x + threadIdx.x;
    if (j >= a.big) return;
    const DevState* __restrict__ ds = a.ds;
    uint2 t = a.lde_t[j];
    uint4 q = a.lde_q[j];
    Ext u, w;
#pragma unroll
    for (int c = 0; c < 4; c++) {
        u.c[c] = bb::add(bb::add(bb::dot2(ds->alp[4].c[c], q.x, ds->alp[5].c[c], q.y), bb::dot2(ds->alp[6].c[c], q.z, ds->alp[7].c[c], q.w)),
                         bb::mul(ds->alp[1].c[c], t.y));
        w.c[c] = bb::dot2(ds->alp[2].c[c], t.x, ds->alp[3].c[c], t.y);
    }
    u.c[0] = bb::add(u.c[0], t.x);
    Ext e0 = ld_ext(a.d0 + 4 * (size_t)j), e1 = ld_ext(a.d1 + 4 * (size_t)j);
    Ext r = bb::add(bb::mul(bb::sub(ds->y02, u), e0), bb::mul(bb::sub(ds->y1, w), e1));
    st_ext(a.ro + 4 * (size_t)j, r);
}

__global__ void __launch_bounds__(256) fri_fold_kernel(TwoLevelTable inv_roots , const uint32_t* in,
                                                       uint32_t* out, uint32_t half, uint32_t log_half,
                                                       const DevState* __restrict__ ds, uint32_t round, uint32_t one_half) {
    if (gridDim.x <= 512u) P3_LATENCY_BOUND_KERNEL();
    uint32_t i = blockIdx.x * blockDim.x + threadIdx.x;
    if (i >= half) return;
    const Ext half_beta = ds->half_beta[round];
    Ext lo = ld_ext(in + 8 * (size_t)i), hi = ld_ext(in + 8 * (size_t)i + 4);
    uint32_t p = tl(inv_roots, brev(i, log_half));
    Ext s = bb::scale(bb::add(lo, hi), one_half);
    Ext d = bb::mul(bb::scale(half_beta, p), bb::sub(lo, hi));
    st_ext(out + 4 * (size_t)i, bb::add(s, d));
}

__global__ void __launch_bounds__(256) grind_kernel(DevState* ds, uint32_t mask, uint32_t base) {
    uint32_t w = base + blockIdx.x * blockDim.x + threadIdx.x;
    if (w >= bb::P) return;
    if (base + blockIdx.x * blockDim.x > *(volatile uint32_t*)&ds->grind_result) return;
    const uint32_t pos = ds->n_in;
    double s[16];
#pragma unroll
    for (int i = 0; i < 16; i++) s[i] = p2f::load_elem((i < 8 && (uint32_t)i < pos) ? ds->inb[i & 7] : ds->st[i]);
#pragma unroll
    for (int i = 0; i < 8; i++) s[i] = (i == (int)pos) ? (double)w : s[i];
    p2f::permute(s);
    if ((bb::from_monty(p2f::store_elem(s[7])) & mask) == 0) atomicMin(&ds->grind_result, w);
}

__global__ void __launch_bounds__(256) grind_keccak_kernel(DevState* ds, uint32_t mask, uint32_t base) {
    uint32_t w = base + blockIdx.x * blockDim.x + threadIdx.x;
    if (w >= bb::P) return;
    if (base + blockIdx.x * blockDim.x > *(volatile uint32_t*)&ds->grind_result) return;
    const KeccakGrindArgs& a = ds->kgrind;
    const uint32_t wm = bb::to_monty(w);
    uint64_t st[25];
#pragma unroll
    for (int i = 0; i < 25; i++) st[i] = a.state[i];
    for (uint32_t blk = 0; blk < a.n_blocks; blk++) {
#pragma unroll
        for (int i = 0; i < 17; i++) {
            uint64_t lane = a.block[blk][i];
            const int32_t rel = (int32_t)(a.wpos) - (int32_t)(blk * 136 + i * 8);
            if (rel > -4 && rel < 8) {
                const uint64_t v = (uint64_t)wm;
                lane ^= rel >= 0 ? (v << (8 * rel)) : (v >> (8 * -rel));
            }
            st[i] ^= lane;
        }
        if (blk + 1 == a.n_blocks) kk::permute_digest(st);
        else kk::permute(st);
    }
    bool ok = false;
#pragma unroll
    for (int t = 0; t < 8; t++) {
        const uint64_t lane = st[3 - t / 2];
        const uint32_t hi_or_lo = (t & 1) ? (uint32_t)lane : (uint32_t)(lane >> 32);
        const uint32_t v = __builtin_bswap32(hi_or_lo) & 0x7fffffffu;
        if (v < bb::P) { ok = (v & mask) == 0; break; }
    }
    if (ok) atomicMin(&ds->grind_result, w);
}

constexpr uint32_t QTREE_MAX_MATS = 8;
struct QTree {
    const uint32_t* mat[QTREE_MAX_MATS];
    uint32_t width[QTREE_MAX_MATS];
    uint32_t stride[QTREE_MAX_MATS];
    uint32_t n_mats;
    const uint32_t* layers;
    uint32_t log_height, shift, slot_off;
};
__global__ void query_gather_kernel(const QTree* trees, const uint32_t* indices, uint32_t slot_words, uint32_t* out) {
    P3_LATENCY_BOUND_KERNEL();
    const QTree& t = trees[blockIdx.y];
    const uint64_t index = (indices[blockIdx.x] >> t.shift) & ((1ull << t.log_height) - 1ull);
    uint32_t* dst = out + (size_t)blockIdx.x * slot_words + t.slot_off;
    uint32_t off = 0;
    for (uint32_t m = 0; m < t.n_mats; m++) {
        for (uint32_t c = threadIdx.x; c < t.width[m]; c += blockDim.x) dst[off + c] = t.mat[m][index * t.stride[m] + c];
        off += t.width[m];
    }
    uint64_t base = 0, len = 1ull << t.log_height;
    for (uint32_t i = 0; i < t.log_height; i++) {
        const uint64_t sib = (index >> i) ^ 1;
        if (threadIdx.x < 8) dst[off + i * 8 + threadIdx.x] = t.layers[base + sib * 8 + threadIdx.x];
        base += len * 8;
        len >>= 1;
    }
}

struct StageLayout {
    uint32_t root_t = 0, root_q = 8, opened = 16, froots = 48, fpoly = 0, witness = 0, status = 0, qidx = 0, slots = 0, words = 0;
};
struct TsArgs {
    DevState* ds;
    uint32_t* ps;
    int kind;
    StageLayout lay;
};
struct TsPis {
    uint32_t w[3];
    uint32_t given;
};

__global__ void __launch_bounds__(64) ts_begin_kernel(TsArgs a, const uint32_t* trace, uint32_t n, uint32_t log_n, TsPis given) {
    P3_LATENCY_BOUND_KERNEL();
    __shared__ KState ks;
    DevChal ch;
    ch.begin(a.kind, a.ds, &ks, true);
    uint32_t pis[3];
    if (given.given) {
        for (int k = 0; k < 3; k++) pis[k] = given.w[k];
    } else {
        pis[0] = trace[0]; pis[1] = trace[1]; pis[2] = trace[2 * (size_t)(n - 1) + 1];
    }
    ch.observe(bb::to_monty(log_n));
    ch.observe(bb::to_monty(log_n));
    ch.observe_n(a.ps + a.lay.root_t, 8);
    ch.observe_n(pis, 3);
    const Ext alpha = ch.sample_ext();
    Ext ap[5];
    ap[0] = bb::ext_one();
#pragma unroll
    for (int k = 1; k < 5; k++) ap[k] = bb::mul(ap[k - 1], alpha);
    if (threadIdx.x == 0) {
        for (int k = 0; k < 3; k++) a.ds->pis[k] = pis[k];
        for (int k = 0; k < 5; k++) a.ds->apow[k] = ap[k];
        a.ds->status = 0;
        a.ps[a.lay.status] = 0;
    }
    ch.end();
}
__global__ void __launch_bounds__(64) ts_zeta_kernel(TsArgs a, uint32_t g_n) {
    P3_LATENCY_BOUND_KERNEL();
    __shared__ KState ks;
    DevChal ch;
    ch.begin(a.kind, a.ds, &ks, false);
    ch.observe_n(a.ps + a.lay.root_q, 8);
    const Ext zeta = ch.sample_ext();
    const Ext zeta_next = bb::scale(zeta, g_n);
    if (threadIdx.x == 0) {
        a.ds->zeta = zeta;
        a.ds->zeta_next = zeta_next;
        a.ds->k0 = den_consts(zeta);
        a.ds->k1 = den_consts(zeta_next);
    }
    ch.end();
}
constexpr int TS_OPEN_THREADS = 256;
__global__ void __launch_bounds__(TS_OPEN_THREADS) ts_open_kernel(TsArgs a, const uint32_t* partials, uint32_t n_blocks,
                                                                  uint32_t log_n, uint32_t sn, uint32_t denom) {
    P3_LATENCY_BOUND_KERNEL();
    __shared__ KState ks;
    __shared__ uint32_t red[TS_OPEN_THREADS / 32][32];
    __shared__ uint32_t tot[32];
    {
        const uint32_t col = threadIdx.x & 31u, part = threadIdx.x >> 5;
        uint32_t v = 0;
        constexpr uint32_t STEP = TS_OPEN_THREADS / 32;
        uint32_t b = part;
        for (; b + 3 * STEP < n_blocks; b += 4 * STEP) {
            const uint32_t p0 = partials[b * 32 + col], p1 = partials[(b + STEP) * 32 + col],
                           p2 = partials[(b + 2 * STEP) * 32 + col], p3 = partials[(b + 3 * STEP) * 32 + col];
            v = bb::add(bb::add(v, bb::add(p0, p1)), bb::add(p2, p3));
        }
        for (; b < n_blocks; b += STEP) v = bb::add(v, partials[b * 32 + col]);
        red[part][col] = v;
    }
    __syncthreads();
    if (threadIdx.x < 32) {
        uint32_t v = 0;
#pragma unroll
        for (int p = 0; p < TS_OPEN_THREADS / 32; p++) v = bb::add(v, red[p][threadIdx.x]);
        tot[threadIdx.x] = v;
    }
    __syncthreads();
    if (threadIdx.x >= 64) return;
    DevChal ch;
    ch.begin(a.kind, a.ds, &ks, false);
    Ext opened[8];
#pragma unroll
    for (int k = 0; k < 8; k++)
#pragma unroll
        for (int c = 0; c < 4; c++) opened[k].c[c] = tot[4 * k + c];
    {
        Ext z0 = a.ds->zeta, z1 = a.ds->zeta_next;
        for (uint32_t i = 0; i < log_n; i++) { z0 = bb::sqr(z0); z1 = bb::sqr(z1); }
        const Ext f0 = bb::scale(bb::sub(z0, bb::ext_from_base(sn)), denom);
        const Ext f1 = bb::scale(bb::sub(z1, bb::ext_from_base(sn)), denom);
#pragma unroll
        for (int k = 0; k < 8; k++) opened[k] = bb::mul(opened[k], (k == 2 || k == 3) ? f1 : f0);
    }
#pragma unroll
    for (int k = 0; k < 8; k++) ch.observe_ext(opened[k]);
    const Ext al = ch.sample_ext();
    Ext alp[8];
    alp[0] = bb::ext_one();
#pragma unroll
    for (int k = 1; k < 8; k++) alp[k] = bb::mul(alp[k - 1], al);
    const Ext ry0 = bb::add(opened[0], bb::mul(alp[1], opened[1]));
    const Ext ry1 = bb::add(opened[2], bb::mul(alp[1], opened[3]));
    const Ext ry2 = bb::add(bb::add(opened[4], bb::mul(alp[1], opened[5])),
                            bb::add(bb::mul(alp[2], opened[6]), bb::mul(alp[3], opened[7])));
    if (threadIdx.x == 0) {
        for (int k = 0; k < 8; k++) {
            a.ds->alp[k] = alp[k];
            for (int c = 0; c < 4; c++) a.ps[a.lay.opened + 4 * k + c] = opened[k].c[c];
        }
        a.ds->y02 = bb::add(ry0, bb::mul(alp[4], ry2));
        a.ds->y1 = bb::mul(alp[2], ry1);
    }
    ch.end();
}
__global__ void __launch_bounds__(64) ts_fri_round_kernel(TsArgs a, uint32_t round, uint32_t one_half) {
    P3_LATENCY_BOUND_KERNEL();
    __shared__ KState ks;
    DevChal ch;
    ch.begin(a.kind, a.ds, &ks, false);
    ch.observe_n(a.ps + a.lay.froots + 8 * round, 8);
    const Ext beta = ch.sample_ext();
    if (threadIdx.x == 0) a.ds->half_beta[round] = bb::scale(beta, one_half);
    ch.end();
}
constexpr uint32_t FRI_TAIL_MAX_LOG = 8;
struct FriTailArgs {
    TsArgs ts;
    uint32_t* vec;
    uint32_t* layers;
    uint32_t vec_off[FRI_TAIL_MAX_LOG + 1], layer_off[FRI_TAIL_MAX_LOG];
    TwoLevelTable inv_roots[FRI_TAIL_MAX_LOG];
    uint32_t r0, n_tail, log_len0, one_half;
};
__global__ void __launch_bounds__(1024) fri_tail_kernel(FriTailArgs a) {
    P3_LATENCY_BOUND_KERNEL();
    __shared__ __attribute__((aligned(16))) uint32_t vbuf[2][4 << FRI_TAIL_MAX_LOG];
    __shared__ uint32_t dig[2][8 << (FRI_TAIL_MAX_LOG - 1)];
    __shared__ KState ks;
    __shared__ Ext hb;
    const uint32_t tid = threadIdx.x, lane16 = tid & 15u, grp = tid >> 4, wave_first = (tid >> 6) << 2;
    const p2c::LaneConst lc = p2c::lane_constants(lane16);
    DevChal ch;
    if (tid < 64) ch.begin(HASH_POSEIDON2, a.ts.ds, &ks, false);
    uint32_t len = 1u << a.log_len0;
    for (uint32_t i = tid; i < 4 * len; i += blockDim.x) vbuf[0][i] = a.vec[a.vec_off[0] + i];
    __syncthreads();
    uint32_t cur = 0;
    for (uint32_t k = 0; k < a.n_tail; k++, len >>= 1) {
        const uint32_t half = len >> 1, log_half = a.log_len0 - 1 - k;
        uint32_t* lay = a.layers + a.layer_off[k];
        for (uint32_t base = 0; base < half; base += 64) {
            const uint32_t row = base + grp;
            uint32_t res = 0;
            if (base + wave_first < half) {
                const uint32_t v = (row < half && lane16 < 8) ? vbuf[cur][row * 8 + lane16] : 0u;
                res = p2c::permute(v, lc);
            }
            if (row < half && lane16 < 8) { dig[0][row * 8 + lane16] = res; lay[row * 8 + lane16] = res; }
        }
        __syncthreads();
        uint32_t d = 0;
        size_t off = (size_t)half * 8;
        for (uint32_t n = half; n > 1; n >>= 1) {
            const uint32_t m = n >> 1;
            uint32_t res = 0;
            if (wave_first < m) {
                const uint32_t v = grp < m ? dig[d][grp * 16 + lane16] : 0u;
                res = p2c::permute(v, lc);
            }
            if (grp < m && lane16 < 8) { dig[d ^ 1][grp * 8 + lane16] = res; lay[off + grp * 8 + lane16] = res; }
            __syncthreads();
            d ^= 1;
            off += (size_t)m * 8;
        }
        const uint32_t round = a.r0 + k;
        if (tid < 8) a.ts.ps[a.ts.lay.froots + 8 * round + tid] = dig[d][tid];
        if (tid < 64) {
            for (uint32_t i = 0; i < 8; i++) ch.observe(dig[d][i]);
            const Ext beta = ch.sample_ext();
            if (tid == 0) { hb = bb::scale(beta, a.one_half); a.ts.ds->half_beta[round] = hb; }
        }
        __syncthreads();
        if (tid < half) {
            const Ext half_beta = hb;
            const Ext lo = ld_ext(&vbuf[cur][8 * tid]), hi = ld_ext(&vbuf[cur][8 * tid + 4]);
            const uint32_t p = tl(a.inv_roots[k], brev(tid, log_half));
            const Ext r = bb::add(bb::scale(bb::add(lo, hi), a.one_half), bb::mul(bb::scale(half_beta, p), bb::sub(lo, hi)));
            st_ext(&vbuf[cur ^ 1][4 * tid], r);
            st_ext(a.vec + a.vec_off[k + 1] + 4 * (size_t)tid, r);
        }
        __syncthreads();
        cur ^= 1;
    }
    if (tid < 64) ch.end();
}

__global__ void __launch_bounds__(64) ts_final_kernel(TsArgs a, uint32_t fpl, uint32_t pow_mask) {
    P3_LATENCY_BOUND_KERNEL();
    __shared__ KState ks;
    DevChal ch;
    ch.begin(a.kind, a.ds, &ks, false);
    for (uint32_t i = 0; i < 4 * fpl; i++) ch.observe(a.ps[a.lay.fpoly + i]);
    ch.end();
    if (threadIdx.x == 0) {
        a.ds->grind_result = 0xffffffffu;
        if (a.kind == HASH_KECCAK) {
            KeccakGrindArgs& g = a.ds->kgrind;
            for (int i = 0; i < 25; i++) g.state[i] = ks.st[i];
            uint8_t tmpl[272];
            for (int i = 0; i < 272; i++) tmpl[i] = 0;
            const uint32_t tail = ks.blen;
            for (uint32_t i = 0; i < tail; i++) tmpl[i] = ks.blk[i];
            const uint32_t end = tail + 4;
            g.n_blocks = end < 136 ? 1 : 2;
            tmpl[end] ^= 0x01;
            tmpl[g.n_blocks * 136 - 1] ^= 0x80;
            for (int b = 0; b < 2; b++)
                for (int i = 0; i < 17; i++) {
                    uint64_t w = 0;
                    for (int j = 0; j < 8; j++) w |= (uint64_t)tmpl[b * 136 + 8 * i + j] << (8 * j);
                    g.block[b][i] = w;
                }
            g.wpos = tail;
            g.mask = pow_mask;
            g.base = 0;
        }
    }
}
__global__ void __launch_bounds__(64) ts_queries_kernel(TsArgs a, uint32_t nq, uint32_t log_big, uint32_t pow_bits, uint32_t* qidx) {
    P3_LATENCY_BOUND_KERNEL();
    __shared__ KState ks;
    const uint32_t found = a.ds->grind_result;
    if (found == 0xffffffffu) {
        if (threadIdx.x == 0) { a.ds->status = ST_GRIND_MISS; a.ps[a.lay.status] = ST_GRIND_MISS; }
        for (uint32_t q = threadIdx.x; q < nq; q += 64) qidx[q] = 0;
        return;
    }
    DevChal ch;
    ch.begin(a.kind, a.ds, &ks, false);
    const uint32_t witness = bb::to_monty(found);
    ch.observe(witness);
    const uint32_t zero_bits = ch.sample_bits(pow_bits);
    if (threadIdx.x == 0) {
        a.ps[a.lay.witness] = witness;
        a.ps[a.lay.status] = zero_bits == 0 ? 0u : 2u;
        a.ds->status = 0;
    }
    for (uint32_t q = 0; q < nq; q++) {
        const uint32_t idx = ch.sample_bits(log_big);
        if (threadIdx.x == 0) { qidx[q] = idx; a.ps[a.lay.qidx + q] = idx; }
    }
    ch.end();
}

static void put_u32(std::vector<uint8_t>& b, uint32_t v) {
    size_t o = b.size();
    b.resize(o + 4);
    memcpy(b.data() + o, &v, 4);
}
static void put_words(std::vector<uint8_t>& b, const uint32_t* w, size_t n) {
    size_t o = b.size();
    b.resize(o + 4 * n);
    memcpy(b.data() + o, w, 4 * n);
}
// ... 70 lines not shown
    int layout(const char* who, uint32_t extra_words) {
        for (uint32_t r = 0; r < n_rounds; r++) {
            const uint32_t w = salt_words;
            trees.push_back(QTree{{fri_vec + fri_vec_off[r], w ? fri_salts + fri_salt_off[r] : nullptr}, {8, w}, {8, w}, w ? 2u : 1u,
                                  fri_layers + fri_layer_off[r], log_big - 1 - r, r + 1});
        }
        slot_words = 0;
        for (QTree& t : trees) {
            t.slot_off = (uint32_t)slot_words;
            for (uint32_t m = 0; m < t.n_mats; m++) slot_words += t.width[m];
            slot_words += (size_t)t.log_height * 8;
        }
        const uint32_t nq = fp.num_queries;
        StageLayout& L = lay;
        L.fpoly = L.froots + 8 * n_rounds;
        L.witness = L.fpoly + (4u << fp.log_final_poly_len);
        L.status = L.witness + 1;
        L.qidx = L.status + 1;
        L.slots = (L.qidx + nq + 3u) & ~3u;
        const size_t stage_words = (size_t)L.slots + slot_words * nq;
        if (stage_words > 0xffffffffull) return bad_arg(who, "proof staging buffer too large");
        L.words = (uint32_t)stage_words;
        int rc;
        if ((rc = alloc(&pstage, stage_words + extra_words))) return rc;
        if ((rc = alloc(&qidx, std::max<uint32_t>(nq, 1)))) return rc;
        uint32_t* p = nullptr;
        if ((rc = alloc(&p, (sizeof(QTree) + 3) / 4 * trees.size()))) return rc;
        qtrees = reinterpret_cast<QTree*>(p);
        P3_HIP(hipMemcpy(qtrees, trees.data(), trees.size() * sizeof(QTree), hipMemcpyHostToDevice));
        return OK;
    }

    int commit(size_t n, const uint32_t* const* mats, const size_t* widths, uint32_t* const* salts, size_t height, uint32_t* layers,
               uint32_t root_slot, size_t mat_stride = 0, hipStream_t on = nullptr) {
        hipStream_t cs = on ? on : stream;
        const uint32_t* mp[QTREE_MAX_MATS]; size_t hh[QTREE_MAX_MATS], ww[QTREE_MAX_MATS], ss[QTREE_MAX_MATS];
        size_t k = 0;
        for (size_t i = 0; i < n; i++, k++) {
            mp[k] = mats[i]; hh[k] = height; ww[k] = widths[i]; ss[k] = mat_stride ? mat_stride : widths[i];
            if (salt_words) { k++; mp[k] = salts[i]; hh[k] = height; ww[k] = ss[k] = salt_words; }
        }
        Tree* tp = nullptr;
        int r = mmcs_commit(cs, mp, hh, ww, k, &tp, layers, pstage + root_slot, hash, ss, profile);
        if (r) return r;
        std::unique_ptr<Tree> t(tp);
        if (!t->root_copied) P3_HIP(hipMemcpyAsync(pstage + root_slot, t->layers + t->layer_off.back(), 32, hipMemcpyDeviceToDevice, cs));
        return OK;
    }
    int fri_rounds(Context& cx, const TsArgs& ts, uint32_t r_end) {
        const uint32_t one_half = bb::inv(bb::to_monty(2));
        const size_t row = 8;
        int rc;
        for (uint32_t r = 0; r < r_end; r++) {
            const uint32_t log_half = log_big - 1 - r, half = 1u << log_half;
            uint32_t* vec = fri_vec + fri_vec_off[r];
            uint32_t* salts = salt_words ? fri_salts + fri_salt_off[r] : nullptr;
            if ((rc = commit(1, &vec, &row, &salts, half, fri_layers + fri_layer_off[r], lay.froots + 8 * r))) return rc;
            hipLaunchKernelGGL(ts_fri_round_kernel, dim3(1), dim3(64), 0, stream, ts, r, one_half);
            P3_HIP(hipGetLastError());
            TwoLevelTable inv_roots;
            if ((rc = cx.get_root_table(stream, log_half + 1, true, &inv_roots))) return rc;
            hipLaunchKernelGGL(fri_fold_kernel, dim3((half + 255) / 256), dim3(256), 0, stream, inv_roots, vec, fri_vec + fri_vec_off[r + 1],
                               half, log_half, ts.ds, r, one_half);
            P3_HIP(hipGetLastError());
        }
        return OK;
    }
    int fri_final(Context& cx, const TsArgs& ts) {
        const uint32_t fpl = 1u << fp.log_final_poly_len;
        int rc;
        if ((rc = bit_reverse_rows(stream, fri_vec + fri_vec_off[n_rounds], fp_ev, fpl, 4))) return rc;
        if ((rc = ntt_dft(cx, stream, fp_ev, pstage + lay.fpoly, fpl, 4, true))) return rc;
        hipLaunchKernelGGL(ts_final_kernel, dim3(1), dim3(64), 0, stream, ts, fpl, pow_mask());
        P3_HIP(hipGetLastError());
        return OK;
    }

    uint32_t pow_mask() const { return (1u << fp.proof_of_work_bits) - 1u; }
    uint32_t grind_range(uint32_t first_log) const {
        return 1u << std::min<uint32_t>(std::max<uint32_t>(first_log ? first_log : fp.proof_of_work_bits + 4, 8), 24);
    }
    int grind(const TsArgs& ts, uint64_t base, uint32_t count) {
        if (hash == HASH_KECCAK) hipLaunchKernelGGL(grind_keccak_kernel, dim3(count / 256), dim3(256), 0, stream, ts.ds, pow_mask(), (uint32_t)base);
        else hipLaunchKernelGGL(grind_kernel, dim3(count / 256), dim3(256), 0, stream, ts.ds, pow_mask(), (uint32_t)base);
        P3_HIP(hipGetLastError());
        return OK;
    }
    int grind_start(const TsArgs& ts) {
        const uint32_t first_log = grind_first_log(), batch = grind_range(first_log);
        const uint32_t head = first_log ? batch : std::min<uint32_t>(batch, 1u << std::max<uint32_t>(fp.proof_of_work_bits + 1, 8));
        int rc;
        if ((rc = grind(ts, 0, head))) return rc;
        if (batch > head && (rc = grind(ts, head, batch - head))) return rc;
        return OK;
    }
    int queries(const TsArgs& ts, uint32_t* host, size_t words) {
        const uint32_t nq = fp.num_queries;
        hipLaunchKernelGGL(ts_queries_kernel, dim3(1), dim3(64), 0, stream, ts, nq, log_big, fp.proof_of_work_bits, qidx);
        P3_HIP(hipGetLastError());
        if (nq) {
            hipLaunchKernelGGL(query_gather_kernel, dim3(nq, (uint32_t)trees.size()), dim3(64), 0, stream, qtrees, qidx, (uint32_t)slot_words,
                               pstage + lay.slots);
            P3_HIP(hipGetLastError());
        }
        P3_HIP(hipMemcpyAsync(host, pstage, words * 4, hipMemcpyDeviceToHost, stream));
        return OK;
    }
    int continue_grind(const TsArgs& ts, uint32_t* host, size_t words) {
        uint32_t batch = grind_range(grind_first_log()), found = 0xffffffffu;
        int rc;
        for (uint64_t base = batch; base < bb::P && found == 0xffffffffu; base += batch) {
            batch = std::min<uint32_t>(batch * 4, 1u << 24);
            if ((rc = grind(ts, base, batch))) return rc;
            P3_HIP(hipMemcpyAsync(&found, &ts.ds->grind_result, 4, hipMemcpyDeviceToHost, stream));
            P3_HIP(hipStreamSynchronize(stream));
        }
        if (found == 0xffffffffu) return fail(ERR_INTERNAL, "grind: no proof-of-work witness found");
        if ((rc = queries(ts, host, words))) return rc;
        P3_HIP(hipStreamSynchronize(stream));
        return OK;
    }

    void put_fri(std::vector<uint8_t>& pf, const uint32_t* hp) const {
        const StageLayout& L = lay;
        const uint32_t nq = fp.num_queries, fpl = 1u << fp.log_final_poly_len, n_inputs = (uint32_t)trees.size() - n_rounds;
        put_u32(pf, n_rounds); put_words(pf, hp + L.froots, (size_t)n_rounds * 8);
        put_u32(pf, nq);
        for (uint32_t q = 0; q < nq; q++) {
            const uint32_t* slot = hp + L.slots + (size_t)q * slot_words;
            put_u32(pf, n_inputs);
            for (uint32_t i = 0; i < n_inputs; i++) {
                const QTree& t = trees[i];
                put_opening(pf, slot, salt_words ? t.n_mats / 2 : t.n_mats, t.width, salt_words, t.log_height);
            }
            put_u32(pf, n_rounds);
            for (uint32_t r = 0; r < n_rounds; r++) {
                const uint32_t lh = log_big - 1 - r, idx = hp[L.qidx + q] >> r;
                put_words(pf, slot + 4 * ((idx ^ 1) & 1), 4);
                if (salt_words) { put_u32(pf, salt_words); put_words(pf, slot + 8, salt_words); }
                put_u32(pf, lh); put_words(pf, slot + 8 + salt_words, (size_t)lh * 8);
                slot += 8 + salt_words + (size_t)lh * 8;
            }
        }
        put_u32(pf, fpl);
        put_words(pf, hp + L.fpoly, (size_t)fpl * 4);
        put_u32(pf, hp[L.witness]);
    }
};

constexpr int N_STAGE_EVENTS = 7;

struct FibProver::Impl : ProverCore {
    uint32_t log_n = 0;
    uint32_t *trace = nullptr, *lde_t = nullptr, *qflat = nullptr, *lde_q = nullptr, *d0 = nullptr, *d1 = nullptr;
    uint32_t *layers_t = nullptr, *layers_q = nullptr, *partials = nullptr;
    DevState* ds = nullptr;
    uint32_t* host_stage[2] = {nullptr, nullptr};
    hipEvent_t done[2] = {nullptr, nullptr};
    struct Pending {
        uint64_t a, b; int slot; std::chrono::steady_clock::time_point t_start, t_enq; uint64_t seq;
        const uint32_t* trace;
        TsPis pis;
    };
    std::deque<Pending> pending;
    uint64_t next_seq = 1, arena_owner = 0;
    hipEvent_t ev[2][N_STAGE_EVENTS] = {{nullptr}, {nullptr}};
    uint32_t bary_blocks = 0;
    StageTimes times{};
    uint64_t grind_misses = 0;
    std::vector<uint32_t> miss_qidx;
    ~Impl() {
        for (auto* h : host_stage) if (h) (void)hipHostFree(h);
        for (auto& set : ev) for (auto& e : set) if (e) (void)hipEventDestroy(e);
        for (auto& e : done) if (e) (void)hipEventDestroy(e);
    }
};

FibProver::FibProver() : im(new Impl()) {}
FibProver::~FibProver() { delete im; }

int FibProver::init(uint32_t log_n, const FriParams& fp, hipStream_t stream, bool own_stream, int hash, int profile) {
    Impl& s = *im;
    int rc;
    if ((rc = s.begin("fib prover", stream, own_stream, hash, profile))) return rc;
    if (log_n < 1) return fail(ERR_BAD_ARG, "fib prover: log_n must be >= 1");
    if (log_n + fp.log_blowup > MAX_LOG_DOMAIN)
        return fail(ERR_BAD_ARG, "fib prover: LDE domain above 2^" + std::to_string(MAX_LOG_DOMAIN) + " points (log_n + log_blowup)");
    if (fp.log_blowup < 1) return fail(ERR_BAD_ARG, "fib prover: log_blowup must be >= 1");
    if ((rc = s.set_fri("fib prover", fp, log_n))) return rc;
    s.log_n = log_n;
    const size_t n = (size_t)1 << log_n, big = (size_t)1 << s.log_big;
    if ((rc = s.alloc(&s.trace, n * 2))) return rc;
    if ((rc = s.alloc(&s.lde_t, big * 2))) return rc;
    if ((rc = s.alloc(&s.qflat, n * 4))) return rc;
    if ((rc = s.alloc(&s.lde_q, big * 4))) return rc;
    if ((rc = s.alloc(&s.d0, big * 4))) return rc;
    if ((rc = s.alloc(&s.d1, big * 4))) return rc;
    if ((rc = s.alloc(&s.layers_t, mmcs_layer_words(big)))) return rc;
    if ((rc = s.alloc(&s.layers_q, mmcs_layer_words(big)))) return rc;
    if ((rc = s.alloc_fri())) return rc;
    s.bary_blocks = (uint32_t)std::min<size_t>(256, (n + BARY_BLOCK - 1) / BARY_BLOCK);
    if ((rc = s.alloc(&s.partials, (size_t)s.bary_blocks * 32))) return rc;
    {
        uint32_t* p = nullptr;
        if ((rc = s.alloc(&p, (sizeof(DevState) + 3) / 4))) return rc;
        s.ds = reinterpret_cast<DevState*>(p);
        P3_HIP(hipMemset(s.ds, 0, sizeof(DevState)));
    }
    s.trees.push_back(QTree{{s.lde_t}, {2}, {2}, 1, s.layers_t, s.log_big});
    s.trees.push_back(QTree{{s.lde_q}, {4}, {4}, 1, s.layers_q, s.log_big});
    if ((rc = s.layout("fib prover", 0))) return rc;
    for (auto& h : s.host_stage) P3_HIP(hipHostMalloc(reinterpret_cast<void**>(&h), (size_t)s.lay.words * 4 + 64));
    for (auto& set : s.ev) for (auto& e : set) P3_HIP(hipEventCreate(&e));
    for (auto& e : s.done) P3_HIP(hipEventCreateWithFlags(&e, hipEventDisableTiming));
    return OK;
}

static int get_selectors(Context& cx, hipStream_t stream, uint32_t log_n, const uint2** out) {
    auto it = cx.selector_tables.find(log_n);
    if (it == cx.selector_tables.end()) {
        const uint32_t n = 1u << log_n;
        CachedTable e;
        P3_HIP(hipMalloc(reinterpret_cast<void**>(&e.t.lo), (size_t)n * 8));
        TwoLevelTable roots;
        int rc = cx.get_root_table(stream, log_n, false, &roots);
        if (rc) { (void)hipFree(e.t.lo); return rc; }
        uint32_t gen = bb::to_monty(bb::GEN);
        uint32_t g = bb::two_adic_generator(log_n), ginv = bb::inv(g);
        uint32_t zh = bb::sub(bb::pow(gen, n), bb::ONE);
        uint32_t threads = (n + SEL_CHUNK - 1) / SEL_CHUNK;
        hipLaunchKernelGGL(selectors_kernel, dim3((threads + 255) / 256), dim3(256), 0, stream, roots, n, gen, ginv, zh,
                           reinterpret_cast<uint2*>(e.t.lo));
        P3_HIP(hipGetLastError());
        if ((rc = cx.mark_built(stream, e))) return rc;
        it = cx.selector_tables.emplace(log_n, e).first;
    }
    int rc = cx.wait_ready(stream, it->second);
    if (rc) return rc;
    *out = reinterpret_cast<const uint2*>(it->second.t.lo);
    return OK;
}

int FibProver::prove(uint64_t a, uint64_t b, std::vector<uint8_t>* proof) {
    if (!im->pending.empty()) return fail(ERR_BAD_ARG, "fib prover: finish the enqueued proofs before a synchronous prove");
    int rc = enqueue(a, b);
    if (rc) return rc;
    return finish(proof);
}
int FibProver::enqueue(uint64_t a, uint64_t b) { return enqueue_any(a, b, nullptr, nullptr); }
int FibProver::enqueue_trace(const uint32_t* d_trace, const uint32_t pis[3]) {
    if (!d_trace || !pis) return fail(ERR_BAD_ARG, "fib prover: null trace or public values");
    return enqueue_any(0, 0, d_trace, pis);
}
int FibProver::prove_trace(const uint32_t* d_trace, const uint32_t pis[3], std::vector<uint8_t>* proof) {
    if (!im->pending.empty()) return fail(ERR_BAD_ARG, "fib prover: finish the enqueued proofs before a synchronous prove");
    int rc = enqueue_trace(d_trace, pis);
    if (rc) return rc;
    return finish(proof);
}
uint32_t* FibProver::arena_trace() const { return im->trace; }
bool FibProver::has_pending() const { return !im->pending.empty(); }
hipStream_t FibProver::stream() const { return im->stream; }
uint32_t FibProver::log_n() const { return im->log_n; }
int FibProver::device() const { return im->device; }
int FibProver::enqueue_any(uint64_t a, uint64_t b, const uint32_t* d_trace, const uint32_t* pis) {
    Impl& s = *im;
    if (s.pending.size() >= 2) return fail(ERR_BAD_ARG, "fib prover: two proofs already in flight (finish one first)");
    const int slot = s.pending.empty() ? 0 : 1 - s.pending.back().slot;
    Impl::Pending p{a, b, slot, std::chrono::steady_clock::now(), {}, s.next_seq++, d_trace, TsPis{{0, 0, 0}, 0}};
    if (pis) p.pis = TsPis{{pis[0], pis[1], pis[2]}, 1};
    int rc = run(a, b, slot, 0, nullptr, &p);
    if (rc) return rc;
    s.pending.push_back(p);
    return OK;
}
int FibProver::finish(std::vector<uint8_t>* proof) {
    Impl& s = *im;
    if (s.pending.empty()) return fail(ERR_BAD_ARG, "fib prover: no proof in flight");
    Impl::Pending p = s.pending.front();
    int rc = run(p.a, p.b, p.slot, 1, proof, &p);
    s.pending.pop_front();
    return rc;
}
int FibProver::run(uint64_t a, uint64_t b, int slot, int phase, std::vector<uint8_t>* proof, void* pending_rec) {
    Impl& s = *im;
    Impl::Pending& pend = *static_cast<Impl::Pending*>(pending_rec);
    hipEvent_t* const ev = s.ev[slot];
    Context* cxp;
    int rc = get_context(&cxp);
    if (rc) return rc;
    Context& cx = *cxp;
    if (cx.device != s.device)
        return fail(ERR_BAD_ARG, "fib prover: created on device " + std::to_string(s.device) + ", current device is " + std::to_string(cx.device));
    hipStream_t st = s.stream;
    const uint32_t log_n = s.log_n, log_big = s.log_big;
    const uint32_t n = 1u << log_n, big = 1u << log_big;
    const uint32_t gen = bb::to_monty(bb::GEN);
    const uint32_t g_n = bb::two_adic_generator(log_n), g_n_inv = bb::inv(g_n);
    const StageLayout& L = s.lay;
    const TsArgs ts{s.ds, s.pstage, s.hash, L};
    const size_t w_trace = 2, w_quot = 4;
    const uint32_t nq = s.fp.num_queries;
    auto body = [&]() -> int {
        s.arena_owner = pend.seq;
        P3_HIP(hipEventRecord(ev[0], st));

        const uint32_t* trace = pend.trace ? pend.trace : s.trace;
        if (!pend.trace && (rc = fib_trace(st, a, b, n, s.trace))) return rc;
        if ((rc = ntt_coset_lde(cx, st, trace, s.lde_t, n, 2, s.fp.log_blowup, gen, true))) return rc;
        if ((rc = s.commit(1, &s.lde_t, &w_trace, nullptr, big, s.layers_t, L.root_t))) return rc;
        hipLaunchKernelGGL(ts_begin_kernel, dim3(1), dim3(64), 0, st, ts, trace, n, log_n, pend.pis);
        P3_HIP(hipGetLastError());
        P3_HIP(hipEventRecord(ev[1], st));

        const uint2* sel = nullptr;
        if ((rc = get_selectors(cx, st, log_n, &sel))) return rc;
        {
            QuotArgs qa{};
            qa.lde = reinterpret_cast<const uint2*>(s.lde_t);
            qa.sel = sel;
            qa.out = s.qflat;
            qa.ds = s.ds;
            if ((rc = cx.get_root_table(st, log_n, false, &qa.roots))) return rc;
            qa.n = n; qa.log_n = log_n; qa.gen = gen; qa.ginv = g_n_inv;
            qa.zh_inv = bb::inv(bb::sub(bb::pow(gen, n), bb::ONE));
            hipLaunchKernelGGL(fib_quotient_kernel, dim3((n + 255) / 256), dim3(256), 0, st, qa);
            P3_HIP(hipGetLastError());
        }
        if ((rc = ntt_coset_lde(cx, st, s.qflat, s.lde_q, n, 4, s.fp.log_blowup, bb::ONE, true))) return rc;
        if ((rc = s.commit(1, &s.lde_q, &w_quot, nullptr, big, s.layers_q, L.root_q))) return rc;
        hipLaunchKernelGGL(ts_zeta_kernel, dim3(1), dim3(64), 0, st, ts, g_n);
        P3_HIP(hipGetLastError());
        P3_HIP(hipEventRecord(ev[2], st));

        TwoLevelTable roots_big;
        if ((rc = cx.get_root_table(st, log_big, false, &roots_big))) return rc;
        {
            uint32_t threads = (big + DEN_CHUNK - 1) / DEN_CHUNK;
            hipLaunchKernelGGL(inv_denoms_kernel, dim3((threads + 255) / 256), dim3(256), 0, st, roots_big, big, log_big, gen,
                               s.ds, s.d0, s.d1);
            P3_HIP(hipGetLastError());
            hipLaunchKernelGGL(barycentric_kernel, dim3(s.bary_blocks), dim3(BARY_BLOCK), 0, st, roots_big, n, log_big, gen,
                               reinterpret_cast<const uint2*>(s.lde_t), reinterpret_cast<const uint4*>(s.lde_q), s.d0, s.d1,
                               s.partials);
            P3_HIP(hipGetLastError());
            const uint32_t sn = bb::pow(gen, n);
            const uint32_t denom = bb::inv(bb::mul(bb::to_monty(n), sn));
            hipLaunchKernelGGL(ts_open_kernel, dim3(1), dim3(TS_OPEN_THREADS), 0, st, ts, s.partials, s.bary_blocks, log_n, sn, denom);
            P3_HIP(hipGetLastError());
        }
        P3_HIP(hipEventRecord(ev[3], st));

        {
            ReducedArgs ra{};
            ra.lde_t = reinterpret_cast<const uint2*>(s.lde_t);
            ra.lde_q = reinterpret_cast<const uint4*>(s.lde_q);
            ra.d0 = s.d0; ra.d1 = s.d1; ra.ro = s.fri_vec + s.fri_vec_off[0]; ra.big = big;
            ra.ds = s.ds;
            hipLaunchKernelGGL(reduced_openings_kernel, dim3((big + 255) / 256), dim3(256), 0, st, ra);
            P3_HIP(hipGetLastError());
        }

        uint32_t r_tail = s.n_rounds;
        if (s.profile == PROFILE_LATENCY && s.hash == HASH_POSEIDON2)
            while (r_tail > 0 && (big >> (r_tail - 1)) <= (1u << FRI_TAIL_MAX_LOG)) r_tail--;
        if ((rc = s.fri_rounds(cx, ts, r_tail))) return rc;
        if (r_tail < s.n_rounds) {
            FriTailArgs ta{};
            ta.ts = ts; ta.vec = s.fri_vec; ta.layers = s.fri_layers;
            ta.r0 = r_tail; ta.n_tail = s.n_rounds - r_tail; ta.log_len0 = log_big - r_tail; ta.one_half = bb::inv(bb::to_monty(2));
            for (uint32_t k = 0; k <= ta.n_tail; k++) {
                if (s.fri_vec_off[r_tail + k] > 0xffffffffull) return fail(ERR_INTERNAL, "fri tail: vector offset out of range");
                ta.vec_off[k] = (uint32_t)s.fri_vec_off[r_tail + k];
            }
            for (uint32_t k = 0; k < ta.n_tail; k++) {
                if (s.fri_layer_off[r_tail + k] > 0xffffffffull) return fail(ERR_INTERNAL, "fri tail: layer offset out of range");
                ta.layer_off[k] = (uint32_t)s.fri_layer_off[r_tail + k];
                if ((rc = cx.get_root_table(st, ta.log_len0 - k, true, &ta.inv_roots[k]))) return rc;
            }
            hipLaunchKernelGGL(fri_tail_kernel, dim3(1), dim3(1024), 0, st, ta);
            P3_HIP(hipGetLastError());
        }
        if ((rc = s.fri_final(cx, ts))) return rc;
        P3_HIP(hipEventRecord(ev[4], st));

        if ((rc = s.grind_start(ts))) return rc;
        P3_HIP(hipEventRecord(ev[5], st));

        if ((rc = s.queries(ts, s.host_stage[slot], L.words))) return rc;
        P3_HIP(hipEventRecord(ev[6], st));
        return OK;
    };
    if (phase == 0) {
        if ((rc = body())) return rc;
        P3_HIP(hipEventRecord(s.done[slot], st));
        pend.t_enq = std::chrono::steady_clock::now();
        return OK;
    }
    const auto t_start = pend.t_start, t_enq = pend.t_enq;
    P3_HIP(hipEventSynchronize(s.done[slot]));
    const uint32_t* hp = s.host_stage[slot];
    static const bool trace = getenv("P3HIP_TRACE") != nullptr;
#define TR(...) do { if (trace) { fprintf(stderr, __VA_ARGS__); fflush(stderr); } } while (0)
    TR("prove: enqueued in %.0f us of host time, synced after another %.0f us, status %u\n",
       std::chrono::duration<double, std::micro>(t_enq - t_start).count(),
       std::chrono::duration<double, std::micro>(std::chrono::steady_clock::now() - t_enq).count(), hp[L.status]);
    if (hp[L.status] == ST_GRIND_MISS) {
        if (s.arena_owner != pend.seq) {
            P3_HIP(hipStreamSynchronize(st));
            if ((rc = body())) return rc;
            P3_HIP(hipStreamSynchronize(st));
        }
        s.grind_misses++;
        s.miss_qidx.assign(nq, 0xdeadbeefu);
        if (nq) P3_HIP(hipMemcpyAsync(s.miss_qidx.data(), s.qidx, (size_t)nq * 4, hipMemcpyDeviceToHost, st));
        P3_HIP(hipStreamSynchronize(st));
        TR("prove: first proof-of-work range empty, continuing the search\n");
        if ((rc = s.continue_grind(ts, s.host_stage[slot], L.words))) return rc;
        TR("prove: witness %u, queries redone, status %u\n", hp[L.witness], hp[L.status]);
    }
    if (hp[L.status] != 0) return fail(ERR_INTERNAL, "grind: witness rejected by the device transcript");

    std::vector<uint8_t>& pf = *proof;
    pf.clear();
    pf.reserve(64 + (size_t)nq * s.slot_words * 4 + 4096);
    put_u32(pf, 0x42463350u); put_u32(pf, 1); put_u32(pf, log_n);
    put_words(pf, hp + L.root_t, 8); put_words(pf, hp + L.root_q, 8);
    const uint32_t* op = hp + L.opened;
    put_u32(pf, 2); put_words(pf, op, 8);
    put_u32(pf, 2); put_words(pf, op + 8, 8);
    put_u32(pf, 1); put_u32(pf, 4); put_words(pf, op + 16, 16);
    s.put_fri(pf, hp);
    TR("prove: serialised %zu bytes\n", pf.size());
    float ms[N_STAGE_EVENTS - 1] = {0};
    for (int k = 0; k + 1 < N_STAGE_EVENTS; k++) (void)hipEventElapsedTime(&ms[k], ev[k], ev[k + 1]);
    s.times.trace_commit_ms += ms[0]; s.times.quotient_commit_ms += ms[1]; s.times.open_ms += ms[2];
    s.times.fri_commit_ms += ms[3]; s.times.grind_ms += ms[4]; s.times.query_ms += ms[5]; s.times.proofs += 1;
    return OK;
}

const StageTimes& FibProver::times() const { return im->times; }
void FibProver::reset_times() { im->times = StageTimes{}; }
uint64_t FibProver::grind_misses(std::vector<uint32_t>* last_indices) const {
    if (last_indices) *last_indices = im->miss_qidx;
    return im->grind_misses;
}

}

#include "prover_hiding.hip.inc"
#include "pcs.hip.inc"
```

plonky3-mobile_amd/csrc/prover_hiding.hip.inc:

```

namespace p3 {

constexpr uint32_t HW = 2, HNRC = 4, HSALT = 4, HD = 4, HTW = HW + HNRC, HRW = HNRC + HD, HCH = 4;
constexpr uint32_t HOPEN = HRW + 2 * HTW + HCH * HD;
constexpr uint32_t HQS = HCH * HD;

struct DevStateH {
    DevState base;
    Ext alp[HOPEN];
    Ext y0, y1;
    uint32_t err;
};

__global__ void randomize_trace_kernel(const uint2* trace, const uint32_t* rnd, uint32_t h, uint32_t* out) {
    uint32_t i = blockIdx.x * blockDim.x + threadIdx.x;
    if (i >= h) return;
    const uint2 t = trace[i];
    const uint32_t* d = rnd + (size_t)i * (HW + 2 * HNRC);
    uint32_t* even = out + (size_t)(2 * i) * HTW;
    even[0] = t.x; even[1] = t.y;
#pragma unroll
    for (uint32_t k = 0; k < HNRC; k++) even[HW + k] = d[k];
#pragma unroll
    for (uint32_t k = 0; k < HTW; k++) even[HTW + k] = d[HNRC + k];
// ... 448 lines not shown
}
uint32_t* FibHidingProver::arena_trace() const { return im->trace; }
hipStream_t FibHidingProver::stream() const { return im->stream; }
uint32_t FibHidingProver::log_n() const { return im->log_n; }
int FibHidingProver::device() const { return im->device; }
int FibHidingProver::prove_any(uint64_t a, uint64_t b, const uint32_t* d_trace, const uint32_t* pis, std::vector<uint8_t>* proof) {
    Impl& s = *im;
    const TsPis given = pis ? TsPis{{pis[0], pis[1], pis[2]}, 1} : TsPis{{0, 0, 0}, 0};
    Context* cxp;
    int rc = get_context(&cxp);
    if (rc) return rc;
    Context& cx = *cxp;
    if (cx.device != s.device) return fail(ERR_BAD_ARG, "hiding prover: created on another device");
    hipStream_t st = s.stream;
    const uint32_t log_n = s.log_n, log_ext = s.log_ext, log_big = s.log_big;
    const uint32_t h = 1u << log_n, h2 = 2 * h, big = 1u << log_big, log_q = log_n + 2;
    const uint32_t gen = bb::to_monty(bb::GEN);
    const uint32_t g_h = bb::two_adic_generator(log_n);
    const StageLayout& L = s.lay;
    DevState* ds = &s.hs->base;
    const TsArgs ts{ds, s.pstage, s.hash, L};
    DevRng *rng_mmcs = s.rngs, *rng_fri = s.rngs + 1, *rng_pcs = s.rngs + 2;
    uint32_t* err = s.pstage + L.words;
    const uint32_t nq = s.fp.num_queries;
    const uint32_t* const hp = s.host_stage;
    if (s.tiny) {
        TinyArgs ta{};
        ta.hash = (uint32_t)s.hash; ta.log_n = log_n; ta.log_blowup = s.fp.log_blowup; ta.log_fpl = s.fp.log_final_poly_len;
        ta.nq = nq; ta.pow_bits = s.fp.proof_of_work_bits;
        ta.a_monty = bb::to_monty((uint32_t)(a % bb::P)); ta.b_monty = bb::to_monty((uint32_t)(b % bb::P));
        rng_seed_from_u64(ta.seed, s.seed);
        if ((rc = rng_jump_table(cx, &ta.jump))) return rc;
        ta.n_pcs = (uint32_t)s.pcs_words; ta.n_mmcs = (uint32_t)s.mmcs_words; ta.n_fri = (uint32_t)s.fri_salt_words;
        const bool short_chunks = rng_tiny_chunks(s.pcs_words) && rng_tiny_chunks(s.mmcs_words) && (!s.fri_salt_words || rng_tiny_chunks(s.fri_salt_words));
        ta.chunk_log = short_chunks ? RNG_TINY_CHUNK_LOG : RNG_CHUNK_LOG;
        if (short_chunks) {
            ta.jump += (size_t)RNG_MAX_JUMP * 256 * 4;
            ta.ch_pcs = rng_tiny_chunks(s.pcs_words); ta.ch_mmcs = rng_tiny_chunks(s.mmcs_words);
            ta.ch_fri = s.fri_salt_words ? rng_tiny_chunks(s.fri_salt_words) : 0;
        } else {
            ta.ch_pcs = rng_small_chunks(s.pcs_words); ta.ch_mmcs = rng_small_chunks(s.mmcs_words);
            ta.ch_fri = s.fri_salt_words ? rng_small_chunks(s.fri_salt_words) : 0;
        }
        ta.pcs_draws = s.pcs_draws; ta.mmcs_draws = s.mmcs_draws; ta.fri_salts = s.fri_salts;
        ta.trace = s.trace; ta.in_trace = d_trace; ta.pis = given; ta.rt = s.rt; ta.lde_t = s.lde_t; ta.salt_t = s.salt_t; ta.layers_t = s.layers_t;
        ta.qchunks = s.qchunks; ta.co = s.co; ta.ext = s.ext; ta.lde_qb = s.lde_qb; ta.layers_q = s.layers_q; ta.t012 = s.t012;
        for (uint32_t c = 0; c < HCH; c++) ta.salt_q[c] = s.salt_q[c];
        ta.rm = s.rm; ta.lde_r = s.lde_r; ta.salt_r = s.salt_r; ta.layers_r = s.layers_r;
        ta.d0 = s.d0; ta.d1 = s.d1; ta.fri_vec = s.fri_vec; ta.fri_layers = s.fri_layers; ta.fp_ev = s.fp_ev;
        ta.n_rounds = s.n_rounds;
        for (uint32_t r = 0; r <= s.n_rounds; r++) ta.fri_vec_off[r] = (uint32_t)s.fri_vec_off[r];
        for (uint32_t r = 0; r < s.n_rounds; r++) { ta.fri_salt_off[r] = (uint32_t)s.fri_salt_off[r]; ta.fri_layer_off[r] = (uint32_t)s.fri_layer_off[r]; }
        ta.hs = s.hs; ta.pstage = s.pstage; ta.lay = L; ta.root_r_off = s.root_r_off; ta.slot_words = (uint32_t)s.slot_words;
        ta.qtrees = s.qtrees; ta.n_trees = (uint32_t)s.trees.size(); ta.qidx = s.qidx; ta.err = err;
        const size_t lds = (size_t)3 * RNG_SMALL_CHUNKS * RNG_SMALL_STRIDE * 4 + 4096;
        if ((rc = cx.ensure_dynamic_lds(reinterpret_cast<const void*>(tiny_hiding_prover_kernel), (int)lds))) return rc;
        hipLaunchKernelGGL(tiny_hiding_prover_kernel, dim3(1), dim3(TINY_THREADS), lds, st, ta);
        P3_HIP(hipGetLastError());
        P3_HIP(hipMemcpyAsync(s.host_stage, s.pstage, ((size_t)L.words + 1) * 4, hipMemcpyDeviceToHost, st));
        P3_HIP(hipStreamSynchronize(st));
    } else {
        if (s.side) P3_HIP(hipStreamWaitEvent(st, s.ev_fri, 0));
        if (s.side2) P3_HIP(hipStreamWaitEvent(st, s.ev_r, 0));
        if ((rc = rng_seed(st, s.rngs, s.seed, 3, err))) return rc;
        auto fill = [&](DevRng* r, uint32_t* out, uint64_t n) {
            return s.one_fill ? OK : rng_fill_field(cx, st, r, out, n, s.rng_ws, err);
        };
        if (s.one_fill) {
            hipStream_t fs = s.side ? s.side : st;
            if (s.side) { P3_HIP(hipEventRecord(s.ev_start, st)); P3_HIP(hipStreamWaitEvent(s.side, s.ev_start, 0)); }
            if ((rc = rng_fill_field(cx, fs, rng_pcs, s.pcs_draws, s.pcs_words, s.rng_ws, err))) return rc;
            if (s.side) P3_HIP(hipEventRecord(s.ev_pcs, s.side));
            if ((rc = rng_fill_field(cx, fs, rng_mmcs, s.mmcs_draws, s.mmcs_words, s.rng_ws, err))) return rc;
            if (s.side) P3_HIP(hipEventRecord(s.ev_mmcs, s.side));
            if ((rc = rng_fill_field(cx, fs, rng_fri, s.fri_salts, s.fri_salt_words, s.rng_ws, err))) return rc;
            if (s.side) P3_HIP(hipEventRecord(s.ev_fri, s.side));
        }
        auto wait_fill = [&](hipEvent_t e) -> int { if (s.side) P3_HIP(hipStreamWaitEvent(st, e, 0)); return OK; };
        const size_t w_r = HRW, w_t = HTW, w_q[HCH] = {HD, HD, HD, HD};
        auto commit_random = [&](hipStream_t on) -> int {
            int r = ntt_coset_lde(cx, on, s.rm, s.lde_r, h2, HRW, s.fp.log_blowup, gen, true);
            if (r) return r;
            return s.commit(1, &s.lde_r, &w_r, &s.salt_r, big, s.layers_r, s.root_r_off, 0, on);
        };
        if (s.side2) {
            P3_HIP(hipStreamWaitEvent(s.side2, s.ev_start, 0));
            P3_HIP(hipStreamWaitEvent(s.side2, s.ev_pcs, 0));
            P3_HIP(hipStreamWaitEvent(s.side2, s.ev_mmcs, 0));
            if ((rc = commit_random(s.side2))) return rc;
            P3_HIP(hipEventRecord(s.ev_r, s.side2));
        }

        const uint32_t* trace = d_trace ? d_trace : s.trace;
        if (!d_trace && (rc = fib_trace(st, a, b, h, s.trace))) return rc;
        if ((rc = fill(rng_pcs, s.rnd_t, (uint64_t)h * (HW + 2 * HNRC)))) return rc;
        if ((rc = wait_fill(s.ev_pcs))) return rc;
        hipLaunchKernelGGL(randomize_trace_kernel, dim3((h + 255) / 256), dim3(256), 0, st, reinterpret_cast<const uint2*>(trace), s.rnd_t, h, s.rt);
        P3_HIP(hipGetLastError());
        if ((rc = ntt_coset_lde(cx, st, s.rt, s.lde_t, h2, HTW, s.fp.log_blowup, gen, true))) return rc;
        if ((rc = fill(rng_mmcs, s.salt_t, (uint64_t)big * HSALT))) return rc;
        if ((rc = wait_fill(s.ev_mmcs))) return rc;
        if ((rc = s.commit(1, &s.lde_t, &w_t, &s.salt_t, big, s.layers_t, L.root_t))) return rc;
        hipLaunchKernelGGL(ts_begin_h_kernel, dim3(1), dim3(64), 0, st, ts, trace, h, log_n, given);
        P3_HIP(hipGetLastError());

        {
            QuotHArgs qa{};
            qa.lde = s.lde_t; qa.chunks = s.qchunks; qa.ds = ds; qa.sel_fl = s.sel_fl; qa.sel_tr = s.sel_tr;
            qa.h = h; qa.log_h = log_n;
            const uint32_t gh = bb::pow(gen, h), w4 = bb::two_adic_generator(2);
            uint32_t p = bb::ONE;
            for (int c = 0; c < 4; c++) { qa.zh_inv[c] = bb::inv(bb::sub(bb::mul(gh, p), bb::ONE)); p = bb::mul(p, w4); }
            hipLaunchKernelGGL(fib_quotient_h_kernel, dim3((h + 255) / 256), dim3(256), 0, st, qa);
            P3_HIP(hipGetLastError());
        }
        if ((rc = fill(rng_pcs, s.t012, (uint64_t)(HCH - 1) * h * HD))) return rc;
        if ((rc = ntt_dft(cx, st, s.qchunks, s.co, h, HQS, true))) return rc;
        {
            BlindArgs ba{};
            ba.co = s.co; ba.t012 = s.t012; ba.ext = s.ext; ba.h = h;
            const uint32_t gh = bb::pow(gen, h), w4 = bb::two_adic_generator(2), g4 = bb::two_adic_generator(log_q);
            uint32_t sh[HCH], kc[HCH], p = bb::ONE;
            for (uint32_t c = 0; c < HCH; c++) { sh[c] = bb::mul(gh, p); p = bb::mul(p, w4); }
            if ((rc = cx.reserve_scale_slots(HCH))) return rc;
            for (uint32_t c = 0; c < HCH; c++) {
                uint32_t k = bb::ONE;
                for (uint32_t j = 0; j < HCH; j++) if (j != c) k = bb::mul(k, bb::sub(sh[c], sh[j]));
                kc[c] = k;
                ba.sh[c] = sh[c]; ba.kinv[c] = bb::inv(k);
                if ((rc = cx.get_scale_table(st, bb::inv(bb::mul(gen, bb::pow(g4, c))), log_n, bb::ONE, &ba.sp[c]))) return rc;
            }
            ba.k_last = kc[HCH - 1];
            hipLaunchKernelGGL(blind_chunks_kernel, dim3((h + 255) / 256), dim3(256), 0, st, ba);
            P3_HIP(hipGetLastError());
        }
        if ((rc = ntt_coset_lde_from_coeffs(cx, st, s.ext, s.lde_qb, s.ev2, h2, HQS, s.fp.log_blowup, gen))) return rc;
        for (uint32_t c = 0; c < HCH; c++) if ((rc = fill(rng_mmcs, s.salt_q[c], (uint64_t)big * HSALT))) return rc;
        if ((rc = s.commit(HCH, s.lde_q, w_q, s.salt_q, big, s.layers_q, L.root_q, HQS))) return rc;

        if (s.side2) {
            P3_HIP(hipStreamWaitEvent(st, s.ev_r, 0));
        } else {
            if ((rc = fill(rng_pcs, s.rm, (uint64_t)h2 * HRW))) return rc;
            if ((rc = fill(rng_mmcs, s.salt_r, (uint64_t)big * HSALT))) return rc;
            if ((rc = commit_random(st))) return rc;
        }
        hipLaunchKernelGGL(ts_zeta_h_kernel, dim3(1), dim3(64), 0, st, ts, s.root_r_off, g_h);
        P3_HIP(hipGetLastError());

        TwoLevelTable roots_big;
        if ((rc = cx.get_root_table(st, log_big, false, &roots_big))) return rc;
        {
            uint32_t threads = (big + DEN_CHUNK - 1) / DEN_CHUNK;
            hipLaunchKernelGGL(inv_denoms_kernel, dim3((threads + 255) / 256), dim3(256), 0, st, roots_big, big, log_big, gen, ds, s.d0, s.d1);
            P3_HIP(hipGetLastError());
            const size_t ps = (size_t)s.bary_blocks * 32;
            {
                BaryAllArgs ba{};
                ba.roots = roots_big; ba.n2 = h2; ba.log_big = log_big; ba.gen = gen;
                ba.lde_r = s.lde_r; ba.lde_t = s.lde_t;
                for (uint32_t c = 0; c < HCH; c++) ba.lde_q[c] = s.lde_q[c];
                ba.d0 = s.d0; ba.d1 = s.d1; ba.partials = s.partials; ba.set_stride = (uint32_t)ps;
                hipLaunchKernelGGL(bary_all_kernel, dim3(s.bary_blocks), dim3(BARY_BLOCK), 0, st, ba);
                P3_HIP(hipGetLastError());
            }
            const uint32_t sn = bb::pow(gen, h2);
            const uint32_t denom = bb::inv(bb::mul(bb::to_monty(h2), sn));
            hipLaunchKernelGGL(ts_open_h_kernel, dim3(1), dim3(TS_OPEN_H_THREADS), 0, st, ts, s.hs, s.partials, s.bary_blocks, log_ext, sn, denom);
            P3_HIP(hipGetLastError());
        }
        {
            ReducedHArgs ra{};
            ra.lde_r = s.lde_r; ra.lde_t = s.lde_t;
            for (uint32_t c = 0; c < HCH; c++) ra.lde_q[c] = s.lde_q[c];
            ra.d0 = s.d0; ra.d1 = s.d1; ra.ro = s.fri_vec + s.fri_vec_off[0]; ra.hs = s.hs; ra.big = big;
            hipLaunchKernelGGL(reduced_openings_h_kernel, dim3((big + 255) / 256), dim3(256), 0, st, ra);
            P3_HIP(hipGetLastError());
        }

        if ((rc = wait_fill(s.ev_fri))) return rc;
        for (uint32_t r = 0; r < s.n_rounds; r++)
            if ((rc = fill(rng_fri, s.fri_salts + s.fri_salt_off[r], (uint64_t)(big >> (r + 1)) * HSALT))) return rc;
        if ((rc = s.fri_rounds(cx, ts, s.n_rounds))) return rc;
        if ((rc = s.fri_final(cx, ts))) return rc;
        if ((rc = s.grind_start(ts))) return rc;
        const size_t words = (size_t)L.words + 1;
        if ((rc = s.queries(ts, s.host_stage, words))) return rc;
        P3_HIP(hipStreamSynchronize(st));
        if (hp[L.status] == ST_GRIND_MISS && (rc = s.continue_grind(ts, s.host_stage, words))) return rc;
    }
    if (hp[L.status] != 0) return fail(ERR_INTERNAL, "grind: witness rejected by the device transcript");
    if (hp[L.words] != 0) return fail(ERR_INTERNAL, "rng: a random stream ran out of raw draws");

    std::vector<uint8_t>& pf = *proof;
    pf.clear();
    pf.reserve(64 + (size_t)nq * (s.slot_words + 64) * 4 + 4096);
    put_u32(pf, 0x42463350u); put_u32(pf, 2); put_u32(pf, log_n);
    put_words(pf, hp + L.root_t, 8); put_words(pf, hp + L.root_q, 8); put_words(pf, hp + s.root_r_off, 8);
    const uint32_t* op = hp + L.opened;
    put_u32(pf, HRW); put_words(pf, op, 4 * HRW); op += 4 * HRW;
    put_u32(pf, HTW); put_words(pf, op, 4 * HTW); op += 4 * HTW;
    put_u32(pf, HTW); put_words(pf, op, 4 * HTW); op += 4 * HTW;
    put_u32(pf, HCH);
    for (uint32_t c = 0; c < HCH; c++) { put_u32(pf, HD); put_words(pf, op, 4 * HD); op += 4 * HD; }
    s.put_fri(pf, hp);
    return OK;
}

}
```

plonky3-mobile_amd/fib_air.py:

```python
import ctypes as C

from . import _lib
from .gpu_dft import _stream_ptr

NUM_FIBONACCI_COLS = 2


def _is_numpy(x):
    return type(x).__module__ == "numpy"


def generate_trace_rows(a, b, n, device="cuda"):
    import torch
    if n & (n - 1):
        raise AssertionError("n must be a power of two")
    out = torch.empty((n, NUM_FIBONACCI_COLS), dtype=torch.int32, device=device)
    _lib.check(_lib.lib().p3hip_fib_trace_dev(a, b, n, C.c_void_p(out.data_ptr()), _stream_ptr()))
    return out


PROVE_CHECK_TRACE = 1
_P = 0x78000001


class TraceCheck(C.Structure):
    _fields_ = [("first_bad_row", C.c_int64), ("mask", C.c_uint32), ("bad_rows", C.c_uint64)]


def _monty_pis(pis):
    pis = [int(v) for v in pis]
    if len(pis) != 3:
        raise ValueError("FibonacciAir has three public values")
    return (C.c_uint32 * 3)(*[((v % _P) << 32) % _P for v in pis])


def _device_trace(trace, rows=None):
    import torch
    if not isinstance(trace, torch.Tensor) or not trace.is_cuda:
        raise TypeError("expected a torch device tensor")
    if trace.dtype not in (torch.int32, torch.uint32) or trace.dim() != 2 or trace.shape[1] != NUM_FIBONACCI_COLS:
        raise ValueError("expected an (n, 2) tensor of 32-bit Montgomery words")
    if not trace.is_contiguous():
        raise ValueError("the trace must be contiguous")
    if rows is not None and trace.shape[0] != rows:
        raise ValueError("the trace has %d rows, the prover proves %d" % (trace.shape[0], rows))
    return trace.data_ptr()


def _sync_current_stream():
    import torch
    torch.cuda.current_stream().synchronize()


def check_fib_trace(trace, pis):
    ptr = _device_trace(trace)
    out = TraceCheck()
    _lib.check(_lib.lib().p3hip_fib_check_trace_dev(C.c_void_p(ptr), trace.shape[0], _monty_pis(pis), C.byref(out), _stream_ptr()))
    return (None if out.first_bad_row < 0 else int(out.first_bad_row)), int(out.mask), int(out.bad_rows)


class FriParameters:

    def __init__(self, log_blowup=1, log_final_poly_len=0, num_queries=100, proof_of_work_bits=16):
        self.log_blowup, self.log_final_poly_len = log_blowup, log_final_poly_len
        self.num_queries, self.proof_of_work_bits = num_queries, proof_of_work_bits

    def _c(self):
        arr = (C.c_uint32 * 4)(self.log_blowup, self.log_final_poly_len, self.num_queries, self.proof_of_work_bits)
        return arr


def _hash_kind(hash):
    kinds = {"poseidon2": 0, "keccak": 1}
    if hash not in kinds:
        raise ValueError("unknown hash configuration %r" % (hash,))
    return kinds[hash]


PROFILE_THROUGHPUT, PROFILE_LATENCY = 1, 2


def profile_kind(profile):
    try:
        return {"throughput": PROFILE_THROUGHPUT, "latency": PROFILE_LATENCY, PROFILE_THROUGHPUT: PROFILE_THROUGHPUT,
                PROFILE_LATENCY: PROFILE_LATENCY}[profile]
    except KeyError:
        raise ValueError("unknown profile %r (throughput | latency)" % (profile,)) from None


def set_thread_profile(profile):
    _lib.check(_lib.lib().p3hip_set_thread_profile(profile_kind(profile)))


def get_thread_profile():
    return {PROFILE_THROUGHPUT: "throughput", PROFILE_LATENCY: "latency"}.get(_lib.lib().p3hip_get_thread_profile())


class FibAirProver:

    def __init__(self, log_n, log_blowup=1, params=None, own_stream=True, hash="poseidon2", hiding=False, seed=1, profile="latency"):
        self.params = params or FriParameters(log_blowup=log_blowup)
        self.log_n = log_n
        self.hash = hash
        self.hiding = hiding
        self.profile = profile
        self._h = C.c_void_p()
        stream = None if own_stream else _stream_ptr()
        _lib.check(_lib.lib().p3hip_fib_prover_create_profile(profile_kind(profile), _hash_kind(hash), 1 if hiding else 0, seed if hiding else 0,
                                                              log_n, C.cast(self.params._c(), C.c_void_p), stream, 1 if own_stream else 0,
                                                              C.byref(self._h)))

    def prove(self, a, b):
        out = C.POINTER(C.c_uint8)()
        n = C.c_size_t()
        _lib.check(_lib.lib().p3hip_fib_prover_prove(self._h, a, b, C.byref(out), C.byref(n)))
        return C.string_at(out, n.value)

    def prove_into(self, a, b, address, cap):
        n = C.c_size_t()
        _lib.check(_lib.lib().p3hip_fib_prover_prove_into(self._h, a, b, C.c_void_p(address), cap, C.byref(n)))
        return n.value

    def enqueue(self, a, b):
        _lib.check(_lib.lib().p3hip_fib_prover_enqueue(self._h, a, b))

    def finish(self):
        out = C.POINTER(C.c_uint8)()
        n = C.c_size_t()
        _lib.check(_lib.lib().p3hip_fib_prover_finish(self._h, C.byref(out), C.byref(n)))
        return C.string_at(out, n.value)

    def prove_trace(self, trace, pis, check=False):
        out = C.POINTER(C.c_uint8)()
        n = C.c_size_t()
        flags = PROVE_CHECK_TRACE if check else 0
        if _is_numpy(trace):
            import numpy as np
            host = np.ascontiguousarray(trace, dtype=np.uint32)
            if host.ndim != 2 or host.shape[1] != NUM_FIBONACCI_COLS:
                raise ValueError("expected an (n, 2) array of Montgomery words")
            _lib.check(_lib.lib().p3hip_fib_prover_prove_trace(self._h, C.c_void_p(host.ctypes.data), host.shape[0], _monty_pis(pis), flags,
                                                               C.byref(out), C.byref(n)))
        else:
            ptr = _device_trace(trace, 1 << self.log_n)
            _sync_current_stream()
            _lib.check(_lib.lib().p3hip_fib_prover_prove_trace_dev(self._h, C.c_void_p(ptr), _monty_pis(pis), flags, C.byref(out), C.byref(n)))
        return C.string_at(out, n.value)

    def enqueue_trace(self, trace, pis):
        ptr = _device_trace(trace, 1 << self.log_n)
        _sync_current_stream()
        _lib.check(_lib.lib().p3hip_fib_prover_enqueue_trace_dev(self._h, C.c_void_p(ptr), _monty_pis(pis)))

    @staticmethod
    def proof_bytes(proof):
        return proof

    def stage_times(self, reset=True):
        ms = (C.c_double * 6)()
        cnt = C.c_uint64()
        _lib.check(_lib.lib().p3hip_fib_prover_stage_times(self._h, ms, C.byref(cnt), 1 if reset else 0))
        k = max(cnt.value, 1)
        names = ["trace_commit", "quotient_commit", "open", "fri_commit_phase", "grind", "queries"]
        return {"prover_" + nm: v / k for nm, v in zip(names, ms)}

    def grind_miss_probe(self):
        import numpy as np
        misses, n = C.c_uint64(), C.c_size_t()
        buf = (C.c_uint32 * 4096)()
        _lib.check(_lib.lib().p3hip_fib_prover_grind_miss_probe(self._h, C.byref(misses), buf, 4096, C.byref(n)))
        return int(misses.value), np.frombuffer(buf, dtype=np.uint32, count=min(n.value, 4096)).copy()

    def stage_breakdown(self):
        self.stage_times(reset=True)
        for i in range(3):
            self.prove(i, i + 1)
        return self.stage_times(reset=True)

    def close(self):
        if self._h:
            _lib.lib().p3hip_fib_prover_destroy(self._h)
            self._h = None

    def __del__(self):
        try:
            self.close()
        except Exception:
            pass


_P = 0x78000001
BENCHMARK_CASES = [(256, 8), (1024, 8), (4096, 8), (16384, 8), (4096, 32), (16384, 32), (4096, 64), (4096, 128),
                   (16384, 64), (16384, 128), (256, 16000)]


def benchmark_input(height, width):
    import numpy as np
    i = np.arange(height * width, dtype=np.uint64)
    v = (i * np.uint64(17) + np.uint64(3)) % np.uint64(_P)
    return ((v << np.uint64(32)) % np.uint64(_P)).astype(np.uint32).reshape(height, width)


def percentile_ms(samples, q):
    import math
    if not samples:
        return 0.0
    s = sorted(samples)
    idx = min(max(int(math.ceil(q * len(s))) - 1, 0), len(s) - 1)
    return s[idx]


def run_dft_benchmark(cases=None, warmup=1, repeats=10, e2e_batch_size=4, cpu_dft=None):
    import time

    import numpy as np
    import torch

    from .gpu_dft import BackendKind, GpuDft, dev_u32, host_u32, take_last_error
    dft = GpuDft.with_backend(BackendKind.Hip)
    lines = ["dft benchmark (repeats=%d, warmup=%d, stats=avg/median/p95)" % (repeats, warmup)]
    rows = []

    def stats(v):
        return sum(v) / len(v), percentile_ms(v, 0.50), percentile_ms(v, 0.95)

    for h, w in (cases or BENCHMARK_CASES):
        x = benchmark_input(h, w)
        xd = dev_u32(x)
        take_last_error()
        for _ in range(warmup):
            dft.dft_batch(x)
            dft.dft_batch(xd)
        e2e, out = [], None
        for _ in range(repeats):
            t = time.perf_counter()
            out = dft.dft_batch(x)
            e2e.append((time.perf_counter() - t) * 1e3)
        batched = []
        pinned_in = torch.from_numpy(x.view(np.int32)).pin_memory()
        outs = [torch.empty((h, w), dtype=torch.int32).pin_memory() for _ in range(e2e_batch_size)]
        for _ in range(repeats):
            t = time.perf_counter()
            for k in range(e2e_batch_size):
                d = pinned_in.to("cuda", non_blocking=True)
                outs[k].copy_(dft.dft_batch(d), non_blocking=True)
            torch.cuda.synchronize()
            batched.append((time.perf_counter() - t) * 1e3 / e2e_batch_size)
        kern = []
        for _ in range(repeats):
            s, e = torch.cuda.Event(enable_timing=True), torch.cuda.Event(enable_timing=True)
            s.record()
            yd = dft.dft_batch(xd)
            e.record()
            torch.cuda.synchronize()
            kern.append(s.elapsed_time(e))
        if take_last_error() is not None:
            raise RuntimeError("hip benchmark error at h=%d, w=%d" % (h, w))
        row = {"h": h, "w": w, "hip_e2e": stats(e2e), "hip_e2e_batched": stats(batched), "hip_kernel": stats(kern)}
        line = "h=%d, w=%d:" % (h, w)
        if cpu_dft is not None:
            cpu, cpu_out = [], None
            for _ in range(max(1, min(repeats, 3))):
                t = time.perf_counter()
                cpu_out = cpu_dft(x)
                cpu.append((time.perf_counter() - t) * 1e3)
            if not (np.array_equal(cpu_out, out) and np.array_equal(cpu_out, host_u32(yd))):
                raise RuntimeError("dft benchmark mismatch at h=%d, w=%d" % (h, w))
            row["cpu"] = stats(cpu)
            line += " cpu(avg=%.3f med=%.3f p95=%.3f)ms" % row["cpu"]
        for key in ("hip_e2e", "hip_e2e_batched", "hip_kernel"):
            line += " %s(avg=%.3f med=%.3f p95=%.3f)ms" % ((key,) + row[key])
            if cpu_dft is not None:
                line += " speedup_%s(avg)=%.2fx" % (key[4:], row["cpu"][0] / row[key][0] if row[key][0] > 0 else 0.0)
        lines.append(line)
        rows.append(row)
    return "\n".join(lines), rows


def fib_public_x(a, b, n):
    l, r = a % _P, b % _P
    for _ in range(n - 1):
        l, r = r, (l + r) % _P
    return r


def verify_fib_air(proof, a, b, x, log_n, params=None, hash="poseidon2", hiding=False):
    params = params or FriParameters()
    buf = (C.c_uint8 * len(proof)).from_buffer_copy(proof)
    fn = _lib.lib().p3hip_verify_fib_air_hiding if hiding else _lib.lib().p3hip_verify_fib_air_hash
    _lib.check(fn(_hash_kind(hash), buf, len(proof), a, b, x, log_n, C.cast(params._c(), C.c_void_p)))


def run_fib_air(log_n=3, a=0, b=1, params=None, hash="poseidon2", hiding=False, seed=1):
    params = params or FriParameters()
    n = 1 << log_n
    x = fib_public_x(a, b, n)
    prover = FibAirProver(log_n, params=params, hash=hash, hiding=hiding, seed=seed)
    try:
        proof = prover.prove(a, b)
    finally:
        prover.close()
    verify_fib_air(proof, a, b, x, log_n, params, hash=hash, hiding=hiding)
    return "fib_air %sok (n=%d, x=%d)" % ("zk " if hiding else "", n, x)


def run_fib_air_zk_report():
    buf = C.create_string_buffer(1024)
    _lib.lib().p3hip_run_fib_air_zk(buf, len(buf))
    return buf.value.decode()


CPU_DFT_FN = C.CFUNCTYPE(C.c_int, C.c_void_p, C.POINTER(C.c_uint32), C.POINTER(C.c_uint32), C.c_size_t, C.c_size_t)


def run_dft_benchmark_report(cpu_dft=None):
    import numpy as np
    cb = None
    if cpu_dft is not None:
        def _cb(_user, pin, pout, h, w):
            try:
                x = np.ctypeslib.as_array(pin, shape=(h, w)).copy()
                np.ctypeslib.as_array(pout, shape=(h, w))[:] = cpu_dft(x)
                return 0
            except Exception:
# ... 173 lines not shown
```

Baseline: 553.1.

## Evaluate quotient directly on LDE domain and drop zeta_next denominators

Computes the Fibonacci AIR quotient directly over the extended coset domain from the trace LDE, using precomputed selector inverses and per-coset vanishing inverses. This skips the compact quotient kernel followed by a coset LDE NTT. Openings at zeta*g are now derived from shifted trace rows that reuse the single zeta denominator, which removes the second inverse-denominator set and its memory traffic. A faster fract/fma formulation of load_elem replaces from_monty in the Poseidon2 f64 path. For user-supplied traces, a side-stream trace check decides which quotient path runs, and that decision adds a host sync.

```diff
diff --git a/include/p3hip.h b/include/p3hip.h
--- a/include/p3hip.h
+++ b/include/p3hip.h
@@ -124,6 +124,7 @@
 int p3hip_fib_prover_stage_times(p3hip_fib_prover_t *prover, double out_ms[6], uint64_t *proofs, int reset);
 int p3hip_fib_prover_grind_miss_probe(p3hip_fib_prover_t *prover, uint64_t *misses, uint32_t *indices_out, size_t cap,
                                       size_t *n_out);
+int p3hip_fib_prover_quotient_paths(p3hip_fib_prover_t *prover, uint64_t *direct, uint64_t *fallback);
 void p3hip_fib_prover_destroy(p3hip_fib_prover_t *prover);
 int p3hip_verify_fib_air(const uint8_t *proof, size_t len, uint64_t a, uint64_t b, uint64_t x, unsigned log_n,
                          const p3hip_fri_params_t *params);
diff --git a/plonky3-mobile_amd/_lib.py b/plonky3-mobile_amd/_lib.py
--- a/plonky3-mobile_amd/_lib.py
+++ b/plonky3-mobile_amd/_lib.py
@@ -86,6 +86,7 @@
     "p3hip_run_dft_benchmark": (C.c_int, [C.c_void_p, C.c_void_p, C.c_char_p, C.c_size_t]),
     "p3hip_fib_prover_grind_miss_probe": (C.c_int, [C.c_void_p, C.POINTER(C.c_uint64), C.POINTER(C.c_uint32), C.c_size_t,
                                                     C.POINTER(C.c_size_t)]),
+    "p3hip_fib_prover_quotient_paths": (C.c_int, [C.c_void_p, C.POINTER(C.c_uint64), C.POINTER(C.c_uint64)]),
     "p3hip_fib_prover_create_hiding": (C.c_int, [C.c_int, C.c_uint, C.c_void_p, C.c_uint64, C.c_void_p, C.c_int, C.POINTER(C.c_void_p)]),
     "p3hip_verify_fib_air_hiding": (C.c_int, [C.c_int, C.c_void_p, C.c_size_t, C.c_uint64, C.c_uint64, C.c_uint64, C.c_uint,
                                               C.c_void_p]),
diff --git a/plonky3-mobile_amd/csrc/c_api.hip b/plonky3-mobile_amd/csrc/c_api.hip
--- a/plonky3-mobile_amd/csrc/c_api.hip
+++ b/plonky3-mobile_amd/csrc/c_api.hip
@@ -739,6 +739,13 @@
     *misses = prover->plain->grind_misses(&idx);
     if (n_out) *n_out = idx.size();
     if (indices_out) for (size_t i = 0; i < idx.size() && i < cap; i++) indices_out[i] = idx[i];
+    return OK;
+}
+
+int p3hip_fib_prover_quotient_paths(p3hip_fib_prover_t* prover, uint64_t* direct, uint64_t* fallback) {
+    if (!prover || !direct || !fallback) return fail(ERR_BAD_ARG, "fib_prover_quotient_paths: null argument");
+    if (!prover->plain) return fail(ERR_BAD_ARG, "fib_prover_quotient_paths: not kept by the hiding prover");
+    prover->plain->quotient_paths(direct, fallback);
     return OK;
 }
 
diff --git a/plonky3-mobile_amd/csrc/common.h b/plonky3-mobile_amd/csrc/common.h
--- a/plonky3-mobile_amd/csrc/common.h
+++ b/plonky3-mobile_amd/csrc/common.h
@@ -104,6 +104,7 @@
     uint32_t mask;
     uint64_t bad_rows;
 };
+int fib_check_trace_enqueue(hipStream_t stream, const uint32_t* d_trace, uint64_t n, const uint32_t pis[3], unsigned long long* res);
 int fib_check_trace(Context& cx, hipStream_t stream, const uint32_t* d_trace, uint64_t n, const uint32_t pis[3], TraceCheck* out);
 
 inline bool is_pow2(uint64_t v) { return v && !(v & (v - 1)); }
diff --git a/plonky3-mobile_amd/csrc/fib_air.hip b/plonky3-mobile_amd/csrc/fib_air.hip
--- a/plonky3-mobile_amd/csrc/fib_air.hip
+++ b/plonky3-mobile_amd/csrc/fib_air.hip
@@ -122,6 +122,21 @@
     }
 }
 
+int fib_check_trace_enqueue(hipStream_t stream, const uint32_t* d_trace, uint64_t n, const uint32_t pis[3], unsigned long long* res) {
+    if (reinterpret_cast<uintptr_t>(d_trace) % 8) return fail(ERR_BAD_ARG, "check_trace: the trace must be 8-byte aligned (rows of two words)");
+    if (n > (1ull << 57)) return fail(ERR_BAD_ARG, "check_trace: too many rows");
+    P3_HIP(hipMemsetAsync(res, 0, 16, stream));
+    const uint64_t pairs = (n + 1) / 2, per_block = (uint64_t)CHECK_BLOCK * CHECK_UNROLL;
+    const uint32_t blocks = (uint32_t)std::min<uint64_t>((pairs + per_block - 1) / per_block, CHECK_MAX_BLOCKS);
+    const CheckPis p{pis[0], pis[1], pis[2]};
+    if (reinterpret_cast<uintptr_t>(d_trace) % 16 == 0)
+        hipLaunchKernelGGL(fib_check_trace_kernel<true>, dim3(blocks), dim3(CHECK_BLOCK), 0, stream, d_trace, n, p, res);
+    else
+        hipLaunchKernelGGL(fib_check_trace_kernel<false>, dim3(blocks), dim3(CHECK_BLOCK), 0, stream, d_trace, n, p, res);
+    P3_HIP(hipGetLastError());
+    return OK;
+}
+
 int fib_check_trace(Context& cx, hipStream_t stream, const uint32_t* d_trace, uint64_t n, const uint32_t pis[3], TraceCheck* out) {
     *out = TraceCheck{-1, 0, 0};
     if (!n) return OK;
@@ -131,15 +146,7 @@
     int rc = buf.reserve(16);
     if (rc) return rc;
     unsigned long long* res = buf.as<unsigned long long>();
-    P3_HIP(hipMemsetAsync(res, 0, 16, stream));
-    const uint64_t pairs = (n + 1) / 2, per_block = (uint64_t)CHECK_BLOCK * CHECK_UNROLL;
-    const uint32_t blocks = (uint32_t)std::min<uint64_t>((pairs + per_block - 1) / per_block, CHECK_MAX_BLOCKS);
-    const CheckPis p{pis[0], pis[1], pis[2]};
-    if (reinterpret_cast<uintptr_t>(d_trace) % 16 == 0)
-        hipLaunchKernelGGL(fib_check_trace_kernel<true>, dim3(blocks), dim3(CHECK_BLOCK), 0, stream, d_trace, n, p, res);
-    else
-        hipLaunchKernelGGL(fib_check_trace_kernel<false>, dim3(blocks), dim3(CHECK_BLOCK), 0, stream, d_trace, n, p, res);
-    P3_HIP(hipGetLastError());
+    if ((rc = fib_check_trace_enqueue(stream, d_trace, n, pis, res))) return rc;
     unsigned long long h[2] = {0, 0};
     P3_HIP(hipMemcpyAsync(h, res, 16, hipMemcpyDeviceToHost, stream));
     P3_HIP(hipStreamSynchronize(stream));
diff --git a/plonky3-mobile_amd/csrc/poseidon2_f64.hip.h b/plonky3-mobile_amd/csrc/poseidon2_f64.hip.h
--- a/plonky3-mobile_amd/csrc/poseidon2_f64.hip.h
+++ b/plonky3-mobile_amd/csrc/poseidon2_f64.hip.h
@@ -149,7 +149,12 @@
     }
 }
 
-__device__ __forceinline__ double load_elem(uint32_t monty) { return (double)bb::from_monty(monty); }
+constexpr double M15_32 = -15.0 / 32.0;
+__device__ __forceinline__ double load_elem(uint32_t monty) {
+    const double xt = (double)monty * M15_32;
+    const double fr = __builtin_amdgcn_fract(xt);
+    return __fma_rn(fr, -PD, xt);
+}
 constexpr double R_MOD_P = 268435454.0;
 constexpr double R_MOD_P_OVER_P = 268435454.0 / 2013265921.0;
 __device__ __forceinline__ uint32_t store_elem(double v, const MagicRegs& k) {
diff --git a/plonky3-mobile_amd/csrc/prover.h b/plonky3-mobile_amd/csrc/prover.h
--- a/plonky3-mobile_amd/csrc/prover.h
+++ b/plonky3-mobile_amd/csrc/prover.h
@@ -41,6 +41,7 @@
     const StageTimes& times() const;
     void reset_times();
     uint64_t grind_misses(std::vector<uint32_t>* last_indices) const;
+    void quotient_paths(uint64_t* direct, uint64_t* fallback) const;
 
   private:
     struct Impl;
diff --git a/plonky3-mobile_amd/csrc/prover.hip b/plonky3-mobile_amd/csrc/prover.hip
--- a/plonky3-mobile_amd/csrc/prover.hip
+++ b/plonky3-mobile_amd/csrc/prover.hip
@@ -90,43 +90,107 @@
     st_ext(a.out + 4 * (size_t)i, bb::scale(acc, a.zh_inv));
 }
 
-constexpr int DEN_CHUNK = 4;
+constexpr uint32_t QDOM_MAX_LOG_BLOWUP = 2;
+struct CosetConsts { uint32_t v[1u << QDOM_MAX_LOG_BLOWUP]; };
+__device__ __forceinline__ uint32_t coset_const(const CosetConsts& c, uint32_t k) {
+    return k == 0 ? c.v[0] : k == 1 ? c.v[1] : k == 2 ? c.v[2] : c.v[3];
+}
+__global__ void selectors_domain_kernel(TwoLevelTable roots_big, uint32_t big, uint32_t log_big, uint32_t gen, uint32_t ginv, uint2* sel) {
+    uint32_t t = blockIdx.x * blockDim.x + threadIdx.x;
+    uint32_t j0 = t * SEL_CHUNK;
+    if (j0 >= big) return;
+    uint32_t v[2 * SEL_CHUNK], pre[2 * SEL_CHUNK];
+    uint32_t acc = bb::ONE;
+#pragma unroll
+    for (int k = 0; k < SEL_CHUNK; k++) {
+        uint32_t x = bb::mul(gen, tl(roots_big, brev((j0 + k) & (big - 1), log_big)));
+        v[2 * k] = bb::sub(x, bb::ONE);
+        v[2 * k + 1] = bb::sub(x, ginv);
+    }
+#pragma unroll
+    for (int k = 0; k < 2 * SEL_CHUNK; k++) { pre[k] = acc; acc = bb::mul(acc, v[k]); }
+    uint32_t inv = bb::inv(acc);
+#pragma unroll
+    for (int k = 2 * SEL_CHUNK - 1; k >= 0; k--) {
+        uint32_t r = bb::mul(inv, pre[k]);
+        inv = bb::mul(inv, v[k]);
+        v[k] = r;
+    }
+#pragma unroll
+    for (int k = 0; k < SEL_CHUNK; k++)
+        if (j0 + k < big) sel[j0 + k] = make_uint2(v[2 * k], v[2 * k + 1]);
+}
+struct QuotDomArgs {
+    const uint2* lde;
+    const uint2* sel;
+    uint32_t* out;
+    const DevState* ds;
+    TwoLevelTable roots;
+    uint32_t big, log_big, log_n, gen, ginv;
+    CosetConsts zh_inv;
+};
+__global__ void __launch_bounds__(256) fib_quotient_domain_kernel(QuotDomArgs a) {
+    uint32_t j = blockIdx.x * blockDim.x + threadIdx.x;
+    if (j >= a.big) return;
+    const DevState* __restrict__ ds = a.ds;
+    const uint32_t mask = (1u << a.log_n) - 1u, i = j & mask;
+    uint2 loc = a.lde[j];
+    uint2 nxt = a.lde[(j - i) + brev((brev(i, a.log_n) + 1) & mask, a.log_n)];
+    uint2 s = a.sel[j];
+    uint32_t x = bb::mul(a.gen, tl(a.roots, brev(j, a.log_big)));
+    uint32_t trans = bb::mul(bb::sub(x, a.ginv), coset_const(a.zh_inv, j >> a.log_n));
+    uint32_t c0 = bb::mul(s.x, bb::sub(loc.x, ds->pis[0]));
+    uint32_t c1 = bb::mul(s.x, bb::sub(loc.y, ds->pis[1]));
+    uint32_t c2 = bb::mul(trans, bb::sub(loc.y, nxt.x));
+    uint32_t c3 = bb::mul(trans, bb::sub(bb::add(loc.x, loc.y), nxt.y));
+    uint32_t c4 = bb::mul(s.y, bb::sub(loc.y, ds->pis[2]));
+    Ext acc;
+#pragma unroll
+    for (int k = 0; k < 4; k++)
+        acc.c[k] = bb::add(bb::add(bb::dot2(ds->apow[4].c[k], c0, ds->apow[3].c[k], c1), bb::dot2(ds->apow[2].c[k], c2, ds->apow[1].c[k], c3)),
+                           bb::mul(ds->apow[0].c[k], c4));
+    st_ext(a.out + 4 * (size_t)j, acc);
+}
+
+constexpr int DEN_CHUNK = 4, DEN_INVS = 2 * DEN_CHUNK;
+template <int NZ>
 __global__ void __launch_bounds__(256) inv_denoms_kernel(TwoLevelTable roots, uint32_t big, uint32_t log_big, uint32_t gen,
                                                          const DevState* __restrict__ ds, uint32_t* d0, uint32_t* d1) {
-    const DenConsts k0 = ds->k0, k1 = ds->k1;
+    constexpr int ROWS = DEN_INVS / NZ;
+    const DenConsts k0 = ds->k0, k1 = NZ > 1 ? ds->k1 : k0;
     uint32_t t = blockIdx.x * blockDim.x + threadIdx.x;
-    uint32_t j0 = t * DEN_CHUNK;
+    uint32_t j0 = t * ROWS;
     if (j0 >= big) return;
-    uint32_t a0[2 * DEN_CHUNK], e0[2 * DEN_CHUNK], e1[2 * DEN_CHUNK], nrm[2 * DEN_CHUNK], pre[2 * DEN_CHUNK];
-#pragma unroll
-    for (int k = 0; k < DEN_CHUNK; k++) {
+    uint32_t a0[DEN_INVS], e0[DEN_INVS], e1[DEN_INVS], nrm[DEN_INVS], pre[DEN_INVS];
+#pragma unroll
+    for (int k = 0; k < ROWS; k++) {
         uint32_t x = bb::mul(gen, tl(roots, brev((j0 + k) & (big - 1), log_big)));
 #pragma unroll
-        for (int z = 0; z < 2; z++) {
+        for (int z = 0; z < NZ; z++) {
             const DenConsts& c = z ? k1 : k0;
             const uint32_t a = bb::sub(c.z0, x);
             const uint32_t dd0 = bb::add(bb::sqr(a), c.k0), dd1 = bb::sub(bb::mul(c.k1, a), c.c1);
-            a0[2 * k + z] = a; e0[2 * k + z] = dd0; e1[2 * k + z] = dd1;
-            nrm[2 * k + z] = bb::sub(bb::sqr(dd0), bb::mul(bb::W_MONTY, bb::sqr(dd1)));
+            a0[NZ * k + z] = a; e0[NZ * k + z] = dd0; e1[NZ * k + z] = dd1;
+            nrm[NZ * k + z] = bb::sub(bb::sqr(dd0), bb::mul(bb::W_MONTY, bb::sqr(dd1)));
         }
     }
     uint32_t acc = bb::ONE;
 #pragma unroll
-    for (int k = 0; k < 2 * DEN_CHUNK; k++) { pre[k] = acc; acc = bb::mul(acc, nrm[k]); }
+    for (int k = 0; k < DEN_INVS; k++) { pre[k] = acc; acc = bb::mul(acc, nrm[k]); }
     uint32_t inv = bb::inv(acc);
 #pragma unroll
-    for (int k = 2 * DEN_CHUNK - 1; k >= 0; k--) {
+    for (int k = DEN_INVS - 1; k >= 0; k--) {
         const uint32_t r = bb::mul(inv, pre[k]);
         inv = bb::mul(inv, nrm[k]);
         nrm[k] = r;
     }
 #pragma unroll
-    for (int k = 0; k < DEN_CHUNK; k++) {
+    for (int k = 0; k < ROWS; k++) {
         if (j0 + k >= big) break;
 #pragma unroll
-        for (int z = 0; z < 2; z++) {
+        for (int z = 0; z < NZ; z++) {
             const DenConsts& c = z ? k1 : k0;
-            const uint32_t i = 2 * k + z;
+            const uint32_t i = NZ * k + z;
             const uint32_t f0 = bb::mul(e0[i], nrm[i]), f1 = bb::neg(bb::mul(e1[i], nrm[i]));
             Ext r;
             r.c[0] = bb::add(bb::mul(a0[i], f0), bb::mul(c.z2w, f1));
@@ -141,19 +205,18 @@
 constexpr int BARY_BLOCK = 256;
 __global__ void __launch_bounds__(BARY_BLOCK) barycentric_kernel(TwoLevelTable roots, uint32_t n, uint32_t log_big,
                                                                  uint32_t gen, const uint2* lde_t, const uint4* lde_q,
-                                                                 const uint32_t* d0, const uint32_t* d1,
-                                                                 uint32_t* partials) {
+                                                                 const uint32_t* d0, uint32_t* partials) {
     Ext acc[8];
 #pragma unroll
     for (int k = 0; k < 8; k++) acc[k] = bb::ext_zero();
-    const uint32_t step = gridDim.x * blockDim.x;
+    const uint32_t step = gridDim.x * blockDim.x, log_n = 31u - (uint32_t)__clz((int)n);
+    auto next = [&](uint32_t j) { return brev((brev(j, log_n) + 1) & (n - 1), log_n); };
     for (uint32_t j = blockIdx.x * blockDim.x + threadIdx.x; j < n; j += 2 * step) {
         const bool two = j + step < n;
         const uint32_t j2 = two ? j + step : j;
         const uint32_t xa = bb::mul(gen, tl(roots, brev(j, log_big))), xb = two ? bb::mul(gen, tl(roots, brev(j2, log_big))) : 0u;
-        const Ext e0a = bb::scale(ld_ext(d0 + 4 * (size_t)j), xa), e1a = bb::scale(ld_ext(d1 + 4 * (size_t)j), xa);
-        const Ext e0b = bb::scale(ld_ext(d0 + 4 * (size_t)j2), xb), e1b = bb::scale(ld_ext(d1 + 4 * (size_t)j2), xb);
-        const uint2 ta = lde_t[j], tb = lde_t[j2];
+        const Ext e0a = bb::scale(ld_ext(d0 + 4 * (size_t)j), xa), e0b = bb::scale(ld_ext(d0 + 4 * (size_t)j2), xb);
+        const uint2 ta = lde_t[j], tb = lde_t[j2], na = lde_t[next(j)], nb = lde_t[next(j2)];
         const uint4 qa = lde_q[j], qb = lde_q[j2];
         auto fma2 = [](Ext& s, const Ext& ea, uint32_t va, const Ext& eb, uint32_t vb) {
 #pragma unroll
@@ -161,8 +224,8 @@
         };
         fma2(acc[0], e0a, ta.x, e0b, tb.x);
         fma2(acc[1], e0a, ta.y, e0b, tb.y);
-        fma2(acc[2], e1a, ta.x, e1b, tb.x);
-        fma2(acc[3], e1a, ta.y, e1b, tb.y);
+        fma2(acc[2], e0a, na.x, e0b, nb.x);
+        fma2(acc[3], e0a, na.y, e0b, nb.y);
         fma2(acc[4], e0a, qa.x, e0b, qb.x);
         fma2(acc[5], e0a, qa.y, e0b, qb.y);
         fma2(acc[6], e0a, qa.z, e0b, qb.z);
@@ -192,10 +255,9 @@
     const uint2* lde_t;
     const uint4* lde_q;
     const uint32_t* d0;
-    const uint32_t* d1;
     uint32_t* ro;
     const DevState* ds;
-    uint32_t big;
+    uint32_t big, log_n;
 };
 __global__ void __launch_bounds__(256) reduced_openings_kernel(ReducedArgs a) {
     uint32_t j = blockIdx.x * blockDim.x + threadIdx.x;
@@ -211,7 +273,9 @@
         w.c[c] = bb::dot2(ds->alp[2].c[c], t.x, ds->alp[3].c[c], t.y);
     }
     u.c[0] = bb::add(u.c[0], t.x);
-    Ext e0 = ld_ext(a.d0 + 4 * (size_t)j), e1 = ld_ext(a.d1 + 4 * (size_t)j);
+    const uint32_t mask = (1u << a.log_n) - 1u, i = j & mask;
+    const uint32_t jp = (j - i) + brev((brev(i, a.log_n) - 1) & mask, a.log_n);
+    Ext e0 = ld_ext(a.d0 + 4 * (size_t)j), e1 = ld_ext(a.d0 + 4 * (size_t)jp);
     Ext r = bb::add(bb::mul(bb::sub(ds->y02, u), e0), bb::mul(bb::sub(ds->y1, w), e1));
     st_ext(a.ro + 4 * (size_t)j, r);
 }
@@ -360,13 +424,12 @@
         a.ds->zeta = zeta;
         a.ds->zeta_next = zeta_next;
         a.ds->k0 = den_consts(zeta);
-        a.ds->k1 = den_consts(zeta_next);
     }
     ch.end();
 }
 constexpr int TS_OPEN_THREADS = 256;
 __global__ void __launch_bounds__(TS_OPEN_THREADS) ts_open_kernel(TsArgs a, const uint32_t* partials, uint32_t n_blocks,
-                                                                  uint32_t log_n, uint32_t sn, uint32_t denom) {
+                                                                  uint32_t log_n, uint32_t sn, uint32_t denom, uint32_t g_n_inv) {
     P3_LATENCY_BOUND_KERNEL();
     __shared__ KState ks;
     __shared__ uint32_t red[TS_OPEN_THREADS / 32][32];
@@ -401,12 +464,11 @@
 #pragma unroll
         for (int c = 0; c < 4; c++) opened[k].c[c] = tot[4 * k + c];
     {
-        Ext z0 = a.ds->zeta, z1 = a.ds->zeta_next;
-        for (uint32_t i = 0; i < log_n; i++) { z0 = bb::sqr(z0); z1 = bb::sqr(z1); }
+        Ext z0 = a.ds->zeta;
+        for (uint32_t i = 0; i < log_n; i++) z0 = bb::sqr(z0);
         const Ext f0 = bb::scale(bb::sub(z0, bb::ext_from_base(sn)), denom);
-        const Ext f1 = bb::scale(bb::sub(z1, bb::ext_from_base(sn)), denom);
-#pragma unroll
-        for (int k = 0; k < 8; k++) opened[k] = bb::mul(opened[k], (k == 2 || k == 3) ? f1 : f0);
+#pragma unroll
+        for (int k = 0; k < 8; k++) opened[k] = bb::mul(opened[k], f0);
     }
 #pragma unroll
     for (int k = 0; k < 8; k++) ch.observe_ext(opened[k]);
@@ -421,11 +483,11 @@
                             bb::add(bb::mul(alp[2], opened[6]), bb::mul(alp[3], opened[7])));
     if (threadIdx.x == 0) {
         for (int k = 0; k < 8; k++) {
-            a.ds->alp[k] = alp[k];
+            a.ds->alp[k] = (k == 2 || k == 3) ? bb::scale(alp[k], g_n_inv) : alp[k];
             for (int c = 0; c < 4; c++) a.ps[a.lay.opened + 4 * k + c] = opened[k].c[c];
         }
         a.ds->y02 = bb::add(ry0, bb::mul(alp[4], ry2));
-        a.ds->y1 = bb::mul(alp[2], ry1);
+        a.ds->y1 = bb::scale(bb::mul(alp[2], ry1), g_n_inv);
     }
     ch.end();
 }
@@ -802,7 +864,7 @@
 
 struct FibProver::Impl : ProverCore {
     uint32_t log_n = 0;
-    uint32_t *trace = nullptr, *lde_t = nullptr, *qflat = nullptr, *lde_q = nullptr, *d0 = nullptr, *d1 = nullptr;
+    uint32_t *trace = nullptr, *lde_t = nullptr, *qflat = nullptr, *lde_q = nullptr, *d0 = nullptr;
     uint32_t *layers_t = nullptr, *layers_q = nullptr, *partials = nullptr;
     DevState* ds = nullptr;
     uint32_t* host_stage[2] = {nullptr, nullptr};
@@ -811,6 +873,7 @@
         uint64_t a, b; int slot; std::chrono::steady_clock::time_point t_start, t_enq; uint64_t seq;
         const uint32_t* trace;
         TsPis pis;
+        int direct;
     };
     std::deque<Pending> pending;
     uint64_t next_seq = 1, arena_owner = 0;
@@ -819,7 +882,28 @@
     StageTimes times{};
     uint64_t grind_misses = 0;
     std::vector<uint32_t> miss_qidx;
+    hipStream_t check_stream = nullptr;
+    unsigned long long *check_res = nullptr, *check_host = nullptr;
+    hipEvent_t check_fork[2] = {nullptr, nullptr}, check_done[2] = {nullptr, nullptr};
+    uint64_t quotient_paths[2] = {0, 0};
+    int ensure_check() {
+        if (!check_res) {
+            uint32_t* p = nullptr;
+            int rc = alloc(&p, 8);
+            if (rc) return rc;
+            check_res = reinterpret_cast<unsigned long long*>(p);
+        }
+        if (!check_host) P3_HIP(hipHostMalloc(reinterpret_cast<void**>(&check_host), 32));
+        for (auto& e : check_fork) if (!e) P3_HIP(hipEventCreateWithFlags(&e, hipEventDisableTiming));
+        for (auto& e : check_done) if (!e) P3_HIP(hipEventCreateWithFlags(&e, hipEventDisableTiming));
+        if (!check_stream) P3_HIP(hipStreamCreateWithFlags(&check_stream, hipStreamNonBlocking));
+        return OK;
+    }
     ~Impl() {
+        if (check_stream) (void)hipStreamDestroy(check_stream);
+        if (check_host) (void)hipHostFree(check_host);
+        for (auto& e : check_fork) if (e) (void)hipEventDestroy(e);
+        for (auto& e : check_done) if (e) (void)hipEventDestroy(e);
         for (auto* h : host_stage) if (h) (void)hipHostFree(h);
         for (auto& set : ev) for (auto& e : set) if (e) (void)hipEventDestroy(e);
         for (auto& e : done) if (e) (void)hipEventDestroy(e);
@@ -845,7 +929,6 @@
     if ((rc = s.alloc(&s.qflat, n * 4))) return rc;
     if ((rc = s.alloc(&s.lde_q, big * 4))) return rc;
     if ((rc = s.alloc(&s.d0, big * 4))) return rc;
-    if ((rc = s.alloc(&s.d1, big * 4))) return rc;
     if ((rc = s.alloc(&s.layers_t, mmcs_layer_words(big)))) return rc;
     if ((rc = s.alloc(&s.layers_q, mmcs_layer_words(big)))) return rc;
     if ((rc = s.alloc_fri())) return rc;
@@ -891,6 +974,29 @@
     return OK;
 }
 
+static int get_domain_selectors(Context& cx, hipStream_t stream, uint32_t log_n, uint32_t log_blowup, const uint2** out) {
+    const uint32_t key = log_n | (log_blowup << 8), log_big = log_n + log_blowup;
+    auto it = cx.selector_tables.find(key);
+    if (it == cx.selector_tables.end()) {
+        const uint32_t big = 1u << log_big;
+        CachedTable e;
+        P3_HIP(hipMalloc(reinterpret_cast<void**>(&e.t.lo), (size_t)big * 8));
+        TwoLevelTable roots;
+        int rc = cx.get_root_table(stream, log_big, false, &roots);
+        if (rc) { (void)hipFree(e.t.lo); return rc; }
+        uint32_t threads = (big + SEL_CHUNK - 1) / SEL_CHUNK;
+        hipLaunchKernelGGL(selectors_domain_kernel, dim3((threads + 255) / 256), dim3(256), 0, stream, roots, big, log_big,
+                           bb::to_monty(bb::GEN), bb::inv(bb::two_adic_generator(log_n)), reinterpret_cast<uint2*>(e.t.lo));
+        P3_HIP(hipGetLastError());
+        if ((rc = cx.mark_built(stream, e))) return rc;
+        it = cx.selector_tables.emplace(key, e).first;
+    }
+    int rc = cx.wait_ready(stream, it->second);
+    if (rc) return rc;
+    *out = reinterpret_cast<const uint2*>(it->second.t.lo);
+    return OK;
+}
+
 int FibProver::prove(uint64_t a, uint64_t b, std::vector<uint8_t>* proof) {
     if (!im->pending.empty()) return fail(ERR_BAD_ARG, "fib prover: finish the enqueued proofs before a synchronous prove");
     int rc = enqueue(a, b);
@@ -917,10 +1023,12 @@
     Impl& s = *im;
     if (s.pending.size() >= 2) return fail(ERR_BAD_ARG, "fib prover: two proofs already in flight (finish one first)");
     const int slot = s.pending.empty() ? 0 : 1 - s.pending.back().slot;
-    Impl::Pending p{a, b, slot, std::chrono::steady_clock::now(), {}, s.next_seq++, d_trace, TsPis{{0, 0, 0}, 0}};
+    Impl::Pending p{a, b, slot, std::chrono::steady_clock::now(), {}, s.next_seq++, d_trace, TsPis{{0, 0, 0}, 0}, 0};
     if (pis) p.pis = TsPis{{pis[0], pis[1], pis[2]}, 1};
+    if (s.fp.log_blowup <= QDOM_MAX_LOG_BLOWUP) p.direct = d_trace ? -1 : 1;
     int rc = run(a, b, slot, 0, nullptr, &p);
     if (rc) return rc;
+    s.quotient_paths[p.direct == 1 ? 0 : 1]++;
     s.pending.push_back(p);
     return OK;
 }
@@ -957,15 +1065,43 @@
 
         const uint32_t* trace = pend.trace ? pend.trace : s.trace;
         if (!pend.trace && (rc = fib_trace(st, a, b, n, s.trace))) return rc;
+        if (pend.direct < 0) {
+            if ((rc = s.ensure_check())) return rc;
+            P3_HIP(hipEventRecord(s.check_fork[slot], st));
+            P3_HIP(hipStreamWaitEvent(s.check_stream, s.check_fork[slot], 0));
+            if ((rc = fib_check_trace_enqueue(s.check_stream, trace, n, pend.pis.w, s.check_res + 2 * slot))) return rc;
+            P3_HIP(hipMemcpyAsync(s.check_host + 2 * slot, s.check_res + 2 * slot, 16, hipMemcpyDeviceToHost, s.check_stream));
+            P3_HIP(hipEventRecord(s.check_done[slot], s.check_stream));
+        }
         if ((rc = ntt_coset_lde(cx, st, trace, s.lde_t, n, 2, s.fp.log_blowup, gen, true))) return rc;
         if ((rc = s.commit(1, &s.lde_t, &w_trace, nullptr, big, s.layers_t, L.root_t))) return rc;
         hipLaunchKernelGGL(ts_begin_kernel, dim3(1), dim3(64), 0, st, ts, trace, n, log_n, pend.pis);
         P3_HIP(hipGetLastError());
         P3_HIP(hipEventRecord(ev[1], st));
 
-        const uint2* sel = nullptr;
-        if ((rc = get_selectors(cx, st, log_n, &sel))) return rc;
-        {
+        if (pend.direct < 0) {
+            P3_HIP(hipEventSynchronize(s.check_done[slot]));
+            pend.direct = s.check_host[2 * slot + 1] == 0 ? 1 : 0;
+        }
+        if (pend.direct) {
+            QuotDomArgs qa{};
+            qa.lde = reinterpret_cast<const uint2*>(s.lde_t);
+            if ((rc = get_domain_selectors(cx, st, log_n, s.fp.log_blowup, &qa.sel))) return rc;
+            qa.out = s.lde_q;
+            qa.ds = s.ds;
+            if ((rc = cx.get_root_table(st, log_big, false, &qa.roots))) return rc;
+            qa.big = big; qa.log_big = log_big; qa.log_n = log_n; qa.gen = gen; qa.ginv = g_n_inv;
+            const uint32_t gen_n = bb::pow(gen, n), h = bb::pow(bb::two_adic_generator(log_big), n);
+            for (uint32_t c = 0; c < (1u << s.fp.log_blowup); c++) {
+                uint32_t r = 0;
+                for (uint32_t k = 0; k < s.fp.log_blowup; k++) r |= ((c >> k) & 1u) << (s.fp.log_blowup - 1 - k);
+                qa.zh_inv.v[c] = bb::inv(bb::sub(bb::mul(gen_n, bb::pow(h, r)), bb::ONE));
+            }
+            hipLaunchKernelGGL(fib_quotient_domain_kernel, dim3((big + 255) / 256), dim3(256), 0, st, qa);
+            P3_HIP(hipGetLastError());
+        } else {
+            const uint2* sel = nullptr;
+            if ((rc = get_selectors(cx, st, log_n, &sel))) return rc;
             QuotArgs qa{};
             qa.lde = reinterpret_cast<const uint2*>(s.lde_t);
             qa.sel = sel;
@@ -976,8 +1112,8 @@
             qa.zh_inv = bb::inv(bb::sub(bb::pow(gen, n), bb::ONE));
             hipLaunchKernelGGL(fib_quotient_kernel, dim3((n + 255) / 256), dim3(256), 0, st, qa);
             P3_HIP(hipGetLastError());
-        }
-        if ((rc = ntt_coset_lde(cx, st, s.qflat, s.lde_q, n, 4, s.fp.log_blowup, bb::ONE, true))) return rc;
+            if ((rc = ntt_coset_lde(cx, st, s.qflat, s.lde_q, n, 4, s.fp.log_blowup, bb::ONE, true))) return rc;
+        }
         if ((rc = s.commit(1, &s.lde_q, &w_quot, nullptr, big, s.layers_q, L.root_q))) return rc;
         hipLaunchKernelGGL(ts_zeta_kernel, dim3(1), dim3(64), 0, st, ts, g_n);
         P3_HIP(hipGetLastError());
@@ -986,17 +1122,17 @@
         TwoLevelTable roots_big;
         if ((rc = cx.get_root_table(st, log_big, false, &roots_big))) return rc;
         {
-            uint32_t threads = (big + DEN_CHUNK - 1) / DEN_CHUNK;
-            hipLaunchKernelGGL(inv_denoms_kernel, dim3((threads + 255) / 256), dim3(256), 0, st, roots_big, big, log_big, gen,
-                               s.ds, s.d0, s.d1);
+            uint32_t threads = (big + DEN_INVS - 1) / DEN_INVS;
+            hipLaunchKernelGGL(inv_denoms_kernel<1>, dim3((threads + 255) / 256), dim3(256), 0, st, roots_big, big, log_big, gen,
+                               s.ds, s.d0, nullptr);
             P3_HIP(hipGetLastError());
             hipLaunchKernelGGL(barycentric_kernel, dim3(s.bary_blocks), dim3(BARY_BLOCK), 0, st, roots_big, n, log_big, gen,
-                               reinterpret_cast<const uint2*>(s.lde_t), reinterpret_cast<const uint4*>(s.lde_q), s.d0, s.d1,
-                               s.partials);
+                               reinterpret_cast<const uint2*>(s.lde_t), reinterpret_cast<const uint4*>(s.lde_q), s.d0, s.partials);
             P3_HIP(hipGetLastError());
             const uint32_t sn = bb::pow(gen, n);
             const uint32_t denom = bb::inv(bb::mul(bb::to_monty(n), sn));
-            hipLaunchKernelGGL(ts_open_kernel, dim3(1), dim3(TS_OPEN_THREADS), 0, st, ts, s.partials, s.bary_blocks, log_n, sn, denom);
+            hipLaunchKernelGGL(ts_open_kernel, dim3(1), dim3(TS_OPEN_THREADS), 0, st, ts, s.partials, s.bary_blocks, log_n, sn, denom,
+                               g_n_inv);
             P3_HIP(hipGetLastError());
         }
         P3_HIP(hipEventRecord(ev[3], st));
@@ -1005,7 +1141,7 @@
             ReducedArgs ra{};
             ra.lde_t = reinterpret_cast<const uint2*>(s.lde_t);
             ra.lde_q = reinterpret_cast<const uint4*>(s.lde_q);
-            ra.d0 = s.d0; ra.d1 = s.d1; ra.ro = s.fri_vec + s.fri_vec_off[0]; ra.big = big;
+            ra.d0 = s.d0; ra.ro = s.fri_vec + s.fri_vec_off[0]; ra.big = big; ra.log_n = log_n;
             ra.ds = s.ds;
             hipLaunchKernelGGL(reduced_openings_kernel, dim3((big + 255) / 256), dim3(256), 0, st, ra);
             P3_HIP(hipGetLastError());
@@ -1091,6 +1227,10 @@
 
 const StageTimes& FibProver::times() const { return im->times; }
 void FibProver::reset_times() { im->times = StageTimes{}; }
+void FibProver::quotient_paths(uint64_t* direct, uint64_t* fallback) const {
+    *direct = im->quotient_paths[0];
+    *fallback = im->quotient_paths[1];
+}
 uint64_t FibProver::grind_misses(std::vector<uint32_t>* last_indices) const {
     if (last_indices) *last_indices = im->miss_qidx;
     return im->grind_misses;
diff --git a/plonky3-mobile_amd/csrc/prover_hiding.hip.inc b/plonky3-mobile_amd/csrc/prover_hiding.hip.inc
--- a/plonky3-mobile_amd/csrc/prover_hiding.hip.inc
+++ b/plonky3-mobile_amd/csrc/prover_hiding.hip.inc
@@ -624,7 +624,7 @@
         if ((rc = cx.get_root_table(st, log_big, false, &roots_big))) return rc;
         {
             uint32_t threads = (big + DEN_CHUNK - 1) / DEN_CHUNK;
-            hipLaunchKernelGGL(inv_denoms_kernel, dim3((threads + 255) / 256), dim3(256), 0, st, roots_big, big, log_big, gen, ds, s.d0, s.d1);
+            hipLaunchKernelGGL(inv_denoms_kernel<2>, dim3((threads + 255) / 256), dim3(256), 0, st, roots_big, big, log_big, gen, ds, s.d0, s.d1);
             P3_HIP(hipGetLastError());
             const size_t ps = (size_t)s.bary_blocks * 32;
             {
diff --git a/plonky3-mobile_amd/fib_air.py b/plonky3-mobile_amd/fib_air.py
--- a/plonky3-mobile_amd/fib_air.py
+++ b/plonky3-mobile_amd/fib_air.py
@@ -170,6 +170,11 @@
         buf = (C.c_uint32 * 4096)()
         _lib.check(_lib.lib().p3hip_fib_prover_grind_miss_probe(self._h, C.byref(misses), buf, 4096, C.byref(n)))
         return int(misses.value), np.frombuffer(buf, dtype=np.uint32, count=min(n.value, 4096)).copy()
+
+    def quotient_paths(self):
+        direct, fallback = C.c_uint64(), C.c_uint64()
+        _lib.check(_lib.lib().p3hip_fib_prover_quotient_paths(self._h, C.byref(direct), C.byref(fallback)))
+        return int(direct.value), int(fallback.value)
 
     def stage_breakdown(self):
         self.stage_times(reset=True)
```

Result: no change. 566.3 (median of 6 runs) (+2.4%).
